# Future-Power-Networks/MAPDN

Hardware: AMD Instinct MI355X
Metric: env-steps/sec (whole node), case141 batch=4096, at 1/2/4/8 MI355X (higher is better)
Workload: dtype f64

## Files before the change

### include/mapdn.h

```cpp
#ifndef MAPDN_H
#define MAPDN_H

#include <stdint.h>

#ifdef __cplusplus
extern "C" {
#endif

#define MAPDN_OK 0
#define MAPDN_E_INVALID (-1)
#define MAPDN_E_TOPOLOGY (-2)
#define MAPDN_E_HIP (-3)
#define MAPDN_E_STATE (-4)
#define MAPDN_E_NOMEM (-5)
#define MAPDN_E_INTERNAL (-6)

#define MAPDN_N_INFO 11

enum { MAPDN_BARRIER_L1 = 0, MAPDN_BARRIER_L2 = 1, MAPDN_BARRIER_COURANT_BELTRAMI = 2,
       MAPDN_BARRIER_BOWL = 3, MAPDN_BARRIER_BUMP = 4 };

enum { MAPDN_SS_PV = 1, MAPDN_SS_DEMAND = 2, MAPDN_SS_REACTIVE = 4, MAPDN_SS_VM_PU = 8,
       MAPDN_SS_VA_DEGREE = 16, MAPDN_SS_ALL = 31 };

enum { MAPDN_F32 = 0, MAPDN_F64 = 1 };

typedef struct mapdn_netspec {
  int32_t n_bus;
  const double* bus_vn_kv;
  const int32_t* bus_zone;
  int32_t n_line;
  const int32_t* line_from_bus;
  const int32_t* line_to_bus;
  const double* line_r_ohm_per_km;
  const double* line_x_ohm_per_km;
  const double* line_c_nf_per_km;
  const double* line_g_us_per_km;
  const double* line_length_km;
  const int32_t* line_parallel;
  const uint8_t* line_in_service;
  int32_t n_branch_pu;
  const int32_t* br_from_bus;
  const int32_t* br_to_bus;
  const double* br_r_pu;
  const double* br_x_pu;
  const double* br_b_pu;
  const double* br_ratio;
  const double* br_shift_deg;
  int32_t n_shunt;
  const int32_t* shunt_bus;
  const double* shunt_p_mw;
  const double* shunt_q_mvar;
  int32_t n_load;
  const int32_t* load_bus;
  int32_t n_sgen;
  const int32_t* sgen_bus;
  const int32_t* sgen_zone;
  int32_t ext_grid_bus;
  double ext_grid_vm_pu;
  double sn_mva;
  double f_hz;
  const double* br_g_pu;
  const double* load_scaling;
  const double* sgen_scaling;
  const int32_t* bus_alias;
  const double* load_const_z;
  const double* load_const_i;
} mapdn_netspec;

typedef struct mapdn_env_config {
  int32_t barrier_type;
  double voltage_weight;
  double q_weight;
  double line_weight;
  int32_t use_line_weight;
  int32_t use_q_weight;
  double v_lower, v_upper;
  int32_t episode_limit;
  double action_low, action_high;
  int32_t reset_action;
  int32_t state_space;
  uint64_t seed;
  int64_t env_id_offset;
  int32_t auto_reset;
  int32_t nr_solver;
  int32_t nr_waves;
  int32_t nr_lanes;
  int32_t nr_lean;
  int32_t nr_h_lds, nr_g_lds, nr_rec_lds, nr_flat_lds, nr_line_lds;
  int32_t nr_mm_pass;
  int32_t sp_lanes;
  int32_t inject_full;
  double nr_check_dx;
  double nr_check_quad;
  int32_t debug_geometry;
  double tolerance_mva;
  int32_t tolerance_is_pu;
  int32_t nr_init;
  int32_t fuse_inject;
  int32_t overlap_advance;
  int32_t xcd_map;
} mapdn_env_config;

typedef struct mapdn_dims_t {
  int32_t n_envs, n_bus, n_line, n_load, n_sgen, n_agents, n_actions, obs_size, state_size, n_info;
  int32_t is_radial;
  int32_t max_zone_size;
} mapdn_dims_t;

typedef struct mapdn_handle mapdn_handle;

const char* mapdn_last_error(const mapdn_handle* h);

int mapdn_create(const mapdn_netspec* net, const mapdn_env_config* cfg, int32_t n_envs,
                 int32_t device, mapdn_handle** out);
void mapdn_destroy(mapdn_handle* h);
int mapdn_dims(const mapdn_handle* h, mapdn_dims_t* out);

int mapdn_set_profiles(mapdn_handle* h, const double* pv, const double* load_p, const double* load_q,
                       int64_t n_rows, int32_t time_delta_min, int32_t days);

int mapdn_get_profile_stats(const mapdn_handle* h, double* stdv, double* smax);

int mapdn_reset(mapdn_handle* h, const int64_t* start_rows, int32_t add_noise, int32_t max_tries,
                void* stream);

int mapdn_step(mapdn_handle* h, const void* actions, int32_t actions_dtype, int32_t add_noise,
               double* reward, uint8_t* terminated, double* info, void* stream);

int mapdn_step_obs(mapdn_handle* h, const void* actions, int32_t actions_dtype, int32_t add_noise,
                   double* reward, uint8_t* terminated, double* info, void* obs, int32_t obs_dtype, void* stream);

int mapdn_get_obs(mapdn_handle* h, void* obs, int32_t dtype, void* stream);
int mapdn_get_state(mapdn_handle* h, void* state, int32_t dtype, void* stream);

int mapdn_get_results(mapdn_handle* h, double* vm_pu, double* va_degree, double* p_mw, double* q_mvar,
                      double* pl_mw, double* sgen_p, double* sgen_q, void* stream);
int mapdn_get_loads(mapdn_handle* h, double* load_p, double* load_q, void* stream);

int mapdn_get_start_rows(mapdn_handle* h, int64_t* start_rows, void* stream);

int mapdn_get_auto_reset_mask(mapdn_handle* h, uint8_t* mask, void* stream);

int mapdn_get_returns(mapdn_handle* h, double* returns, void* stream);

int mapdn_solve_only(mapdn_handle* h, const double* p_load, const double* q_load, const double* p_sgen,
                     const double* q_sgen, double* vm_pu, double* va_degree, int32_t* iterations,
                     uint8_t* converged, void* stream);

int mapdn_get_ybus_dense(const mapdn_handle* h, double* ybus_re_im);
int mapdn_get_obs_index(const mapdn_handle* h, int32_t* kind, int32_t* index);

int mapdn_get_schedule(const mapdn_handle* h, int32_t n_waves, int32_t* n_rows, int32_t* rows, int32_t* parent);

int mapdn_get_nr_geometry(const mapdn_handle* h, int32_t* out20);

int mapdn_get_dc_angles(const mapdn_handle* h, const double* p_bus_demand_mw, double* va_rad);

int mapdn_get_flat_factors(const mapdn_handle* h, double* factors, int32_t* bus_of_pos);

int mapdn_get_sparse_program(const mapdn_handle* h, int32_t sub_lanes, int32_t* dims, int32_t* ops, int32_t* order, int32_t* slots_ij);

int mapdn_dense_solve(const double* a, const double* b, double* x, int32_t n, int32_t batch, void* stream);

int mapdn_policy_forward(const float* obs, const float* hid_in, const float* w1, const float* b1, const float* ln_g,
                         const float* ln_b, const float* w_ih, const float* w_hh, const float* b_ih, const float* b_hh,
                         const float* w2, const float* b2, float* means, float* hid_out, int32_t rows, int32_t n_agents,
                         int32_t obs_dim, int32_t id_dim, float ln_eps, void* stream);

int mapdn_policy_forward_train(const float* obs, const float* hid_in, const float* w1, const float* b1, const float* ln_g,
                               const float* ln_b, const float* w_ih, const float* w_hh, const float* b_ih, const float* b_hh,
                               const float* w2, const float* b2, float* means, float* hid_out, float* x1_out, int32_t rows,
                               int32_t n_agents, int32_t obs_dim, int32_t id_dim, float ln_eps, void* stream);
int64_t mapdn_policy_backward_scratch_floats(int64_t rows);
int mapdn_policy_backward(const float* dmeans, const float* x1, const float* hid_in, const float* ln_g, const float* ln_b, float ln_eps,
                          const float* w_ih, const float* w_hh, const float* b_ih, const float* b_hh, const float* w2, float* dx1,
                          float* dgates, float* xn, float* small, float* scratch, int64_t rows, void* stream);

int mapdn_policy_forward_fits(int32_t obs_dim, int32_t id_dim);
int mapdn_policy_forward_geometry(int32_t obs_dim, int32_t id_dim, int32_t* threads, int32_t* ids_lds, int32_t* lds_bytes);

int mapdn_layernorm64_forward(const float* x, const float* gamma, const float* beta, float* y, float* mean, float* rstd,
                              int64_t rows, float eps, int32_t relu, void* stream);
int mapdn_layernorm64_backward_blocks(int64_t rows);
int mapdn_layernorm64_backward(const float* dy, const float* x, const float* gamma, const float* beta, const float* mean,
                               const float* rstd, float* dx, float* dgamma, float* dbeta, float* partial, int64_t rows,
                               int32_t relu, void* stream);
int mapdn_layernorm64_bc_forward(const float* base, const float* per_n, int32_t n, const float* gamma, const float* beta, float* y,
                                 float* mean, float* rstd, int64_t rows, float eps, int32_t relu, void* stream);
int mapdn_layernorm64_bc_backward(const float* dy, const float* base, const float* per_n, int32_t n, const float* gamma, const float* beta,
                                  const float* mean, const float* rstd, float* dx, float* dgamma, float* dbeta, float* partial,
                                  int64_t rows, int32_t relu, void* stream);
int mapdn_relu_dot64_forward(const float* pre, const float* w, float bias, float* v, int64_t rows, void* stream);
int mapdn_relu_dot64_backward(const float* dv, const float* pre, const float* w, float* dpre, float* dw, float* db, float* partial,
                              int64_t rows, void* stream);

int mapdn_critic_head_forward(const float* x, const float* per_n, int32_t n, const float* gamma, const float* beta, float eps,
                              const float* w2, const float* b2, const float* w3, const float* b3, float* v, int64_t rows, void* stream);
int64_t mapdn_critic_head_scratch_floats(int64_t rows, int32_t n, int32_t formed);
int mapdn_critic_head_backward_geometry(int64_t rows, int32_t n, int32_t formed, int32_t mode, int32_t cus, int32_t* threads,
                                        int32_t* blocks, int32_t* lds_bytes);
int mapdn_critic_head_backward(const float* dv, const float* x, const float* per_n, int32_t n, const float* gamma, const float* beta,
                               float eps, const float* w2, const float* b2, const float* w3, const float* b3, float* dx, float* grads,
                               float* scratch, int64_t rows, int32_t param_grads, void* stream);
int mapdn_critic_head_mse(const float* ret, const float* wrow, const float* scale, const float* x, const float* per_n, int32_t n,
                          const float* gamma, const float* beta, float eps, const float* w2, const float* b2, const float* w3,
                          const float* b3, float* dx, float* grads, float* scratch, int64_t rows, void* stream);
int mapdn_critic_head_backward_dot(const float* dv, const float* x, const float* per_n, int32_t n, const float* gamma, const float* beta,
                                   float eps, const float* w2, const float* b2, const float* w3, const float* b3, const float* dot_w,
                                   float* dact, int64_t rows, void* stream);

int mapdn_critic_twin_forward(const float* base, const float* per_n, int32_t n, const float* flag_col, const float* gamma, const float* beta,
                              float eps, const float* w2, const float* b2, const float* w3, const float* b3, float* v1, float* v2,
                              float* vmin, int64_t rows, void* stream);
int64_t mapdn_critic_twin_scratch_floats(int64_t rows, int32_t n);
int mapdn_critic_twin_geometry(int64_t rows, int32_t n, int32_t cus, int32_t* threads, int32_t* blocks, int32_t* lds_bytes);
int mapdn_critic_twin_mse(const float* ret, const float* wrow, const float* scale, const float* base, const float* per_n, int32_t n,
                          const float* flag_col, const float* gamma, const float* beta, float eps, const float* w2, const float* b2,
                          const float* w3, const float* b3, float* dbase, float* grads, float* scratch, int64_t rows, void* stream);

int mapdn_explore_actions(const float* mean, const float* eps, const float* avail, float stdv, int32_t tanh_bound, double action_scale,
                          double action_bias, float* action, float* action_pol, float* actual, int64_t n, void* stream);
int mapdn_rollout_stats(const double* info, const double* reward, const uint8_t* alive, const uint8_t* done, uint8_t* alive_out, double* sums,
                        int32_t n_envs, void* stream);
int mapdn_copy_segments(const void* const* src, void* const* dst, const int64_t* nbytes, int32_t n_segments, void* stream);

int mapdn_debug_stream(const double* src, double* dst, int32_t rows, int32_t Bp, int32_t pattern, void* stream);

const char* mapdn_build_info(void);

int mapdn_stats(mapdn_handle* h, int64_t* reset_failures, double* mean_iters, int32_t* max_iters,
                void* stream);

int mapdn_nr_timing(mapdn_handle* h, int32_t enable);
int mapdn_nr_time_ms(mapdn_handle* h, double* total_ms, int64_t* launches);

int mapdn_get_nr_kernel(const mapdn_handle* h, int32_t* out8);

typedef struct mapdn_droop_config {
  double va, vb, vc, vd;
  double damping;
  int32_t max_iter;
  double v_tol;
  double reactive_ratio;
} mapdn_droop_config;

int mapdn_droop_actions(mapdn_handle* h, const mapdn_droop_config* cfg, double* actions, double* vm_pu, int32_t* iterations,
                        uint8_t* status, void* stream);

#ifdef __cplusplus
}
#endif
#endif
```

### mapdn_amd/_lib.py

```python
from __future__ import annotations

import ctypes as C
import os

import numpy as np

from .netspec import NetSpec

_HERE = os.path.dirname(os.path.abspath(__file__))
LIB_PATH = os.path.join(_HERE, "libmapdn_hip.so")

N_INFO = 11
INFO_KEYS = (
    "percentage_of_v_out_of_control", "percentage_of_lower_than_lower_v",
    "percentage_of_higher_than_upper_v", "totally_controllable_ratio",
    "average_voltage_deviation", "average_voltage", "max_voltage_drop_deviation",
    "max_voltage_rise_deviation", "total_line_loss", "q_loss", "destroy",
)
BARRIER_IDS = dict(l1=0, l2=1, courant_beltrami=2, bowl=3, bump=4)
SS_BITS = dict(pv=1, demand=2, reactive=4, vm_pu=8, va_degree=16)
F32, F64 = 0, 1

EXPORTS = (
    "mapdn_last_error", "mapdn_create", "mapdn_destroy", "mapdn_dims", "mapdn_set_profiles", "mapdn_reset",
    "mapdn_step", "mapdn_get_start_rows", "mapdn_get_returns", "mapdn_get_obs", "mapdn_get_state", "mapdn_get_results", "mapdn_get_loads",
    "mapdn_solve_only", "mapdn_get_ybus_dense", "mapdn_get_obs_index", "mapdn_get_schedule", "mapdn_get_flat_factors", "mapdn_stats", "mapdn_nr_timing",
    "mapdn_nr_time_ms", "mapdn_get_auto_reset_mask", "mapdn_dense_solve", "mapdn_step_obs", "mapdn_get_sparse_program", "mapdn_policy_forward",
    "mapdn_policy_forward_fits", "mapdn_layernorm64_forward", "mapdn_layernorm64_backward", "mapdn_layernorm64_backward_blocks",
    "mapdn_get_nr_geometry", "mapdn_debug_stream", "mapdn_build_info", "mapdn_layernorm64_bc_forward", "mapdn_layernorm64_bc_backward", "mapdn_relu_dot64_forward", "mapdn_relu_dot64_backward",
    "mapdn_critic_head_forward", "mapdn_critic_head_scratch_floats", "mapdn_critic_head_backward", "mapdn_critic_head_backward_dot", "mapdn_critic_head_mse", "mapdn_get_profile_stats",
    "mapdn_explore_actions", "mapdn_rollout_stats", "mapdn_copy_segments",
    "mapdn_policy_forward_train", "mapdn_policy_backward", "mapdn_policy_backward_scratch_floats", "mapdn_get_dc_angles",
    "mapdn_get_nr_kernel", "mapdn_droop_actions", "mapdn_policy_forward_geometry", "mapdn_critic_head_backward_geometry",
    "mapdn_critic_twin_forward", "mapdn_critic_twin_scratch_floats", "mapdn_critic_twin_geometry", "mapdn_critic_twin_mse",
)

_pd = C.POINTER(C.c_double)
_pi = C.POINTER(C.c_int32)
_pu8 = C.POINTER(C.c_uint8)


class CNetSpec(C.Structure):
    _fields_ = [
        ("n_bus", C.c_int32), ("bus_vn_kv", _pd), ("bus_zone", _pi),
        ("n_line", C.c_int32), ("line_from_bus", _pi), ("line_to_bus", _pi),
        ("line_r_ohm_per_km", _pd), ("line_x_ohm_per_km", _pd), ("line_c_nf_per_km", _pd),
        ("line_g_us_per_km", _pd), ("line_length_km", _pd), ("line_parallel", _pi), ("line_in_service", _pu8),
        ("n_branch_pu", C.c_int32), ("br_from_bus", _pi), ("br_to_bus", _pi), ("br_r_pu", _pd), ("br_x_pu", _pd),
        ("br_b_pu", _pd), ("br_ratio", _pd), ("br_shift_deg", _pd),
        ("n_shunt", C.c_int32), ("shunt_bus", _pi), ("shunt_p_mw", _pd), ("shunt_q_mvar", _pd),
        ("n_load", C.c_int32), ("load_bus", _pi),
        ("n_sgen", C.c_int32), ("sgen_bus", _pi), ("sgen_zone", _pi),
        ("ext_grid_bus", C.c_int32), ("ext_grid_vm_pu", C.c_double), ("sn_mva", C.c_double), ("f_hz", C.c_double),
        ("br_g_pu", _pd), ("load_scaling", _pd), ("sgen_scaling", _pd), ("bus_alias", _pi),
        ("load_const_z", _pd), ("load_const_i", _pd),
    ]


class CEnvConfig(C.Structure):
    _fields_ = [
        ("barrier_type", C.c_int32), ("voltage_weight", C.c_double), ("q_weight", C.c_double),
        ("line_weight", C.c_double), ("use_line_weight", C.c_int32), ("use_q_weight", C.c_int32),
        ("v_lower", C.c_double), ("v_upper", C.c_double), ("episode_limit", C.c_int32),
        ("action_low", C.c_double), ("action_high", C.c_double), ("reset_action", C.c_int32),
        ("state_space", C.c_int32), ("seed", C.c_uint64), ("env_id_offset", C.c_int64), ("auto_reset", C.c_int32),
        ("nr_solver", C.c_int32), ("nr_waves", C.c_int32), ("nr_lanes", C.c_int32), ("nr_lean", C.c_int32),
        ("nr_h_lds", C.c_int32), ("nr_g_lds", C.c_int32), ("nr_rec_lds", C.c_int32), ("nr_flat_lds", C.c_int32), ("nr_line_lds", C.c_int32),
        ("nr_mm_pass", C.c_int32), ("sp_lanes", C.c_int32), ("inject_full", C.c_int32),
        ("nr_check_dx", C.c_double), ("nr_check_quad", C.c_double), ("debug_geometry", C.c_int32),
        ("tolerance_mva", C.c_double), ("tolerance_is_pu", C.c_int32), ("nr_init", C.c_int32),
        ("fuse_inject", C.c_int32), ("overlap_advance", C.c_int32), ("xcd_map", C.c_int32),
    ]


TUNING_INT = ("nr_solver", "nr_waves", "nr_lanes", "nr_lean", "nr_h_lds", "nr_g_lds", "nr_rec_lds", "nr_flat_lds", "nr_line_lds",
              "nr_mm_pass", "sp_lanes", "inject_full", "debug_geometry", "tolerance_is_pu", "nr_init", "fuse_inject", "overlap_advance", "xcd_map")
TUNING_F64 = ("nr_check_dx", "nr_check_quad", "tolerance_mva")
NR_SOLVERS = dict(auto=0, tree=0, sparse=1, dense=2)
NR_INITS = dict(flat=0, dc=2)
GEOMETRY_KEYS = ("solver", "waves", "lanes", "lean", "rows", "h_lds", "g_lds", "rec_lds", "flat_lds", "line_lds", "mm_pass",
                 "lds_bytes", "workgroups", "resident_per_cu", "rounds", "model_ns", "fuse_inject", "n_fused_buses", "n_nodes", "nr_init")


class CDroopConfig(C.Structure):
    _fields_ = [("va", C.c_double), ("vb", C.c_double), ("vc", C.c_double), ("vd", C.c_double), ("damping", C.c_double),
                ("max_iter", C.c_int32), ("v_tol", C.c_double), ("reactive_ratio", C.c_double)]


DROOP_STATUS = ("converged", "max_iter", "pf_failed", "not_solved")


def make_droop_config(cfg=None) -> CDroopConfig:
    c = CDroopConfig()
    if cfg is None:
        return c
    get = cfg.get if isinstance(cfg, dict) else (lambda k, _d=None: getattr(cfg, k, _d))
    if isinstance(cfg, dict):
        unknown = set(cfg) - {f for f, _ in CDroopConfig._fields_}
        if unknown:
            raise KeyError(f"unknown droop config keys {sorted(unknown)}")
    for name, typ in CDroopConfig._fields_:
        v = get(name, None)
        if v is not None:
            setattr(c, name, int(v) if typ is C.c_int32 else float(v))
    return c


class CDims(C.Structure):
    _fields_ = [(k, C.c_int32) for k in (
        "n_envs", "n_bus", "n_line", "n_load", "n_sgen", "n_agents", "n_actions", "obs_size", "state_size",
        "n_info", "is_radial", "max_zone_size")]


class MapdnError(RuntimeError):
    def __init__(self, code, msg):
        super().__init__(f"libmapdn_hip error {code}: {msg}")
        self.code = code


_lib = None


def _safe_source_hash(b):
    try:
        return b.source_hash()
    except OSError:
        return "sources unreadable"


def load():
    global _lib
    if _lib is not None:
        return _lib
    import torch
    if "MAPDN_LIB_PATH" not in os.environ:
        from . import build as _build
        try:
            is_stale = _build.stale()
        except OSError:
            is_stale = not os.path.exists(LIB_PATH)
            if not is_stale:
                import warnings
                warnings.warn(f"mapdn_amd/csrc is not readable: {LIB_PATH} is loaded without the source-hash check", RuntimeWarning, stacklevel=2)
        if is_stale:
            try:
                _build.build_locked()
            except Exception as exc:
                raise ImportError(
                    f"{LIB_PATH} is missing or was built from other sources than mapdn_amd/csrc (hash {_build.library_hash()} vs "
                    f"{_safe_source_hash(_build)}) and could not be rebuilt ({exc}); build it with `python -m mapdn_amd.build` "
                    "(hipcc --offload-arch=gfx950); there is no CPU fallback") from exc
    lib = C.CDLL(os.environ.get("MAPDN_LIB_PATH", LIB_PATH))
    if "MAPDN_LIB_PATH" in os.environ:
        for name in EXPORTS:
            if not hasattr(lib, name):
                def _missing(*a, _n=name, **k):
                    raise AttributeError(f"{os.environ['MAPDN_LIB_PATH']} does not export {_n}")
                lib.__dict__[name] = _missing
    vp = C.c_void_p
    lib.mapdn_last_error.restype = C.c_char_p
    lib.mapdn_last_error.argtypes = [vp]
    lib.mapdn_build_info.restype = C.c_char_p
    lib.mapdn_build_info.argtypes = []
    lib.mapdn_create.argtypes = [C.POINTER(CNetSpec), C.POINTER(CEnvConfig), C.c_int32, C.c_int32, C.POINTER(vp)]
    lib.mapdn_destroy.argtypes = [vp]
    lib.mapdn_destroy.restype = None
    lib.mapdn_dims.argtypes = [vp, C.POINTER(CDims)]
    lib.mapdn_set_profiles.argtypes = [vp, _pd, _pd, _pd, C.c_int64, C.c_int32, C.c_int32]
    lib.mapdn_get_profile_stats.argtypes = [vp, _pd, _pd]
    lib.mapdn_reset.argtypes = [vp, vp, C.c_int32, C.c_int32, vp]
    lib.mapdn_step.argtypes = [vp, vp, C.c_int32, C.c_int32, vp, vp, vp, vp]
    lib.mapdn_step_obs.argtypes = [vp, vp, C.c_int32, C.c_int32, vp, vp, vp, vp, C.c_int32, vp]
    lib.mapdn_get_start_rows.argtypes = [vp, vp, vp]
    lib.mapdn_get_returns.argtypes = [vp, vp, vp]
    lib.mapdn_get_auto_reset_mask.argtypes = [vp, vp, vp]
    lib.mapdn_get_obs.argtypes = [vp, vp, C.c_int32, vp]
    lib.mapdn_get_state.argtypes = [vp, vp, C.c_int32, vp]
    lib.mapdn_get_results.argtypes = [vp] + [vp] * 7 + [vp]
    lib.mapdn_get_loads.argtypes = [vp, vp, vp, vp]
    lib.mapdn_solve_only.argtypes = [vp] + [vp] * 8 + [vp]
    lib.mapdn_get_ybus_dense.argtypes = [vp, _pd]
    lib.mapdn_get_obs_index.argtypes = [vp, _pi, _pi]
    lib.mapdn_get_schedule.argtypes = [vp, C.c_int32, _pi, _pi, _pi]
    lib.mapdn_get_flat_factors.argtypes = [vp, _pd, _pi]
    lib.mapdn_get_dc_angles.argtypes = [vp, _pd, _pd]
    lib.mapdn_get_nr_geometry.argtypes = [vp, _pi]
    lib.mapdn_get_nr_kernel.argtypes = [vp, _pi]
    lib.mapdn_debug_stream.argtypes = [vp, vp, C.c_int32, C.c_int32, C.c_int32, vp]
    lib.mapdn_get_sparse_program.argtypes = [vp, C.c_int32, _pi, _pi, _pi, _pi]
    lib.mapdn_policy_forward.argtypes = [vp] * 14 + [C.c_int32] * 4 + [C.c_float, vp]
    lib.mapdn_policy_forward_fits.argtypes = [C.c_int32, C.c_int32]
    lib.mapdn_policy_forward_geometry.argtypes = [C.c_int32, C.c_int32, _pi, _pi, _pi]
    lib.mapdn_critic_head_backward_geometry.argtypes = [C.c_int64, C.c_int32, C.c_int32, C.c_int32, C.c_int32, _pi, _pi, _pi]
    lib.mapdn_policy_forward_train.argtypes = [vp] * 15 + [C.c_int32] * 4 + [C.c_float, vp]
    lib.mapdn_policy_backward_scratch_floats.argtypes = [C.c_int64]
    lib.mapdn_policy_backward_scratch_floats.restype = C.c_int64
    lib.mapdn_policy_backward.argtypes = [vp] * 5 + [C.c_float] + [vp] * 10 + [C.c_int64, vp]
    lib.mapdn_layernorm64_forward.argtypes = [vp] * 6 + [C.c_int64, C.c_float, C.c_int32, vp]
    lib.mapdn_layernorm64_backward_blocks.argtypes = [C.c_int64]
    lib.mapdn_layernorm64_backward.argtypes = [vp] * 10 + [C.c_int64, C.c_int32, vp]
    lib.mapdn_layernorm64_bc_forward.argtypes = [vp, vp, C.c_int32] + [vp] * 5 + [C.c_int64, C.c_float, C.c_int32, vp]
    lib.mapdn_layernorm64_bc_backward.argtypes = [vp, vp, vp, C.c_int32] + [vp] * 8 + [C.c_int64, C.c_int32, vp]
    lib.mapdn_relu_dot64_forward.argtypes = [vp, vp, C.c_float, vp, C.c_int64, vp]
    lib.mapdn_relu_dot64_backward.argtypes = [vp] * 7 + [C.c_int64, vp]
    lib.mapdn_critic_head_forward.argtypes = [vp, vp, C.c_int32, vp, vp, C.c_float] + [vp] * 5 + [C.c_int64, vp]
    lib.mapdn_critic_head_scratch_floats.argtypes = [C.c_int64, C.c_int32, C.c_int32]
    lib.mapdn_critic_head_scratch_floats.restype = C.c_int64
    lib.mapdn_critic_head_backward.argtypes = [vp, vp, vp, C.c_int32, vp, vp, C.c_float] + [vp] * 7 + [C.c_int64, C.c_int32, vp]
    lib.mapdn_explore_actions.argtypes = [vp, vp, vp, C.c_float, C.c_int32, C.c_double, C.c_double, vp, vp, vp, C.c_int64, vp]
    lib.mapdn_rollout_stats.argtypes = [vp, vp, vp, vp, vp, vp, C.c_int32, vp]
    lib.mapdn_copy_segments.argtypes = [C.POINTER(vp), C.POINTER(vp), C.POINTER(C.c_int64), C.c_int32, vp]
    lib.mapdn_critic_head_mse.argtypes = [vp] * 5 + [C.c_int32, vp, vp, C.c_float] + [vp] * 7 + [C.c_int64, vp]
    lib.mapdn_critic_twin_forward.argtypes = [vp, vp, C.c_int32, vp, vp, vp, C.c_float] + [vp] * 7 + [C.c_int64, vp]
    lib.mapdn_critic_twin_scratch_floats.argtypes = [C.c_int64, C.c_int32]
    lib.mapdn_critic_twin_scratch_floats.restype = C.c_int64
    lib.mapdn_critic_twin_geometry.argtypes = [C.c_int64, C.c_int32, C.c_int32, _pi, _pi, _pi]
    lib.mapdn_critic_twin_mse.argtypes = [vp] * 5 + [C.c_int32, vp, vp, vp, C.c_float] + [vp] * 7 + [C.c_int64, vp]
    lib.mapdn_critic_head_backward_dot.argtypes = [vp, vp, vp, C.c_int32, vp, vp, C.c_float] + [vp] * 6 + [C.c_int64, vp]
    lib.mapdn_dense_solve.argtypes = [vp, vp, vp, C.c_int32, C.c_int32, vp]
    lib.mapdn_stats.argtypes = [vp, C.POINTER(C.c_int64), C.POINTER(C.c_double), C.POINTER(C.c_int32), vp]
    lib.mapdn_nr_timing.argtypes = [vp, C.c_int32]
    lib.mapdn_nr_time_ms.argtypes = [vp, C.POINTER(C.c_double), C.POINTER(C.c_int64)]
    lib.mapdn_droop_actions.argtypes = [vp, C.POINTER(CDroopConfig), vp, vp, vp, vp, vp]
    for name in EXPORTS:
        if name not in ("mapdn_last_error", "mapdn_destroy", "mapdn_build_info"):
            getattr(lib, name).restype = C.c_int
    _lib = lib
    return lib


def check(rc, handle=None):
    if rc != 0:
        msg = load().mapdn_last_error(handle)
        raise MapdnError(rc, msg.decode() if msg else "?")


def _p(a, typ):
    return a.ctypes.data_as(typ) if a.size else C.cast(None, typ)


def make_cnetspec(net: NetSpec):
    keep = net
    s = CNetSpec()
    s.n_bus = net.n_bus
    s.bus_vn_kv = _p(net.bus_vn_kv, _pd)
    s.bus_zone = _p(net.bus_zone, _pi)
    s.n_line = net.n_line
    s.line_from_bus = _p(net.line_from_bus, _pi)
    s.line_to_bus = _p(net.line_to_bus, _pi)
    s.line_r_ohm_per_km = _p(net.line_r_ohm_per_km, _pd)
    s.line_x_ohm_per_km = _p(net.line_x_ohm_per_km, _pd)
    s.line_c_nf_per_km = _p(net.line_c_nf_per_km, _pd)
    s.line_g_us_per_km = _p(net.line_g_us_per_km, _pd)
    s.line_length_km = _p(net.line_length_km, _pd)
    s.line_parallel = _p(net.line_parallel, _pi)
    s.line_in_service = _p(net.line_in_service, _pu8)
    s.n_branch_pu = net.n_branch_pu
    s.br_from_bus = _p(net.br_from_bus, _pi)
    s.br_to_bus = _p(net.br_to_bus, _pi)
    s.br_r_pu = _p(net.br_r_pu, _pd)
    s.br_x_pu = _p(net.br_x_pu, _pd)
    s.br_b_pu = _p(net.br_b_pu, _pd)
    s.br_ratio = _p(net.br_ratio, _pd)
    s.br_shift_deg = _p(net.br_shift_deg, _pd)
    s.n_shunt = int(net.shunt_bus.shape[0])
    s.shunt_bus = _p(net.shunt_bus, _pi)
    s.shunt_p_mw = _p(net.shunt_p_mw, _pd)
    s.shunt_q_mvar = _p(net.shunt_q_mvar, _pd)
    s.n_load = net.n_load
    s.load_bus = _p(net.load_bus, _pi)
    s.n_sgen = net.n_sgen
    s.sgen_bus = _p(net.sgen_bus, _pi)
    s.sgen_zone = _p(net.sgen_zone, _pi)
    s.ext_grid_bus = int(net.ext_grid_bus)
    s.ext_grid_vm_pu = float(net.ext_grid_vm_pu)
    s.sn_mva = float(net.sn_mva)
    s.f_hz = float(net.f_hz)
    s.br_g_pu = _p(net.br_g_pu, _pd)
    s.load_scaling = _p(net.load_scaling, _pd)
    s.sgen_scaling = _p(net.sgen_scaling, _pd)
    s.bus_alias = _p(net.bus_alias, _pi) if net.has_fused_buses else C.cast(None, _pi)
    zl = net.has_zip_loads
    s.load_const_z = _p(net.load_const_z, _pd) if zl else C.cast(None, _pd)
    s.load_const_i = _p(net.load_const_i, _pd) if zl else C.cast(None, _pd)
    return s, keep


def make_cconfig(args: dict, env_id_offset: int = 0, tuning: dict | None = None) -> CEnvConfig:
    c = CEnvConfig()
    for k, v in (tuning or {}).items():
        if k == "nr_solver" and isinstance(v, str):
            v = NR_SOLVERS[v]
        if k == "nr_init" and isinstance(v, str):
            if v not in NR_INITS:
                raise ValueError(f"nr_init must be one of {sorted(NR_INITS)} (or 0 / 2), got {v!r}")
            v = NR_INITS[v]
        if k in TUNING_INT:
            setattr(c, k, int(v))
        elif k in TUNING_F64:
            setattr(c, k, float(v))
        else:
            raise KeyError(f"unknown tuning key {k!r} (known: {TUNING_INT + TUNING_F64})")
    bt = args.get("voltage_barrier_type", "l1")
    if bt not in BARRIER_IDS:
        raise KeyError(bt)
    c.barrier_type = BARRIER_IDS[bt]
    c.voltage_weight = float(args.get("voltage_weight", 1.0))
    qw, lw = args.get("q_weight", 0.1), args.get("line_weight", None)
    c.q_weight = 0.0 if qw is None else float(qw)
    c.line_weight = 0.0 if lw is None else float(lw)
    c.use_q_weight = int(qw is not None)
    c.use_line_weight = int(lw is not None)
    c.v_lower = float(args.get("v_lower", 0.95))
    c.v_upper = float(args.get("v_upper", 1.05))
    c.episode_limit = int(args["episode_limit"])
    c.action_low = -float(args["action_scale"]) + float(args["action_bias"])
    c.action_high = float(args["action_scale"]) + float(args["action_bias"])
    c.reset_action = int(bool(args.get("reset_action", True)))
    ss = args.get("state_space", ["pv", "demand", "reactive", "vm_pu", "va_degree"])
    c.state_space = sum(SS_BITS[k] for k in set(ss) if k in SS_BITS)
    c.seed = int(args.get("seed", 0)) & 0xFFFFFFFFFFFFFFFF
    c.env_id_offset = int(env_id_offset)
    c.auto_reset = int(bool(args.get("auto_reset", False)))
    return c


def nr_geometry(handle) -> dict:
    out = (C.c_int32 * 20)()
    check(load().mapdn_get_nr_geometry(handle, out), handle)
    return dict(zip(GEOMETRY_KEYS, [int(x) for x in out]))


NR_KERNEL_KEYS = {0: ("W", "L", "HL", "GL", "RES", "DC", "ZIP"), 1: ("L", "DC", "ZIP"), 2: ("W", "GA")}


def nr_kernel(handle) -> dict:
    out = (C.c_int32 * 8)()
    check(load().mapdn_get_nr_kernel(handle, out), handle)
    solver = int(out[0])
    return dict(solver=solver, **{k: int(out[1 + i]) for i, k in enumerate(NR_KERNEL_KEYS[solver])})


def policy_forward_geometry(obs_dim: int, id_dim: int):
    t, il, lds = C.c_int32(), C.c_int32(), C.c_int32()
    ok = load().mapdn_policy_forward_geometry(int(obs_dim), int(id_dim), C.byref(t), C.byref(il), C.byref(lds))
    return (t.value, il.value, lds.value) if ok else None


def critic_head_backward_geometry(rows: int, n: int, formed: bool, mode: int, cus: int = 0):
    t, b, lds = C.c_int32(), C.c_int32(), C.c_int32()
    rc = load().mapdn_critic_head_backward_geometry(int(rows), int(n), int(bool(formed)), int(mode), int(cus), C.byref(t), C.byref(b), C.byref(lds))
    return (t.value, b.value, lds.value) if rc == 0 else None


def critic_twin_geometry(rows: int, n: int, cus: int = 0):
    t, b, lds = C.c_int32(), C.c_int32(), C.c_int32()
    rc = load().mapdn_critic_twin_geometry(int(rows), int(n), int(cus), C.byref(t), C.byref(b), C.byref(lds))
    return (t.value, b.value, lds.value) if rc == 0 else None
```

### mapdn_amd/csrc/capi.hip

```cpp
#include <hip/hip_runtime.h>

#include <algorithm>
#include <cmath>
#include <cstdio>
#include <cstdlib>
#include <cstring>
#include <string>
#include <type_traits>
#include <vector>

#include "kernels.hpp"
#include "nr_inst_list.hpp"
#include "colstats.hpp"
#include "plan.hpp"

using namespace mapdn;

static constexpr size_t CU_LDS = 160 * 1024;
static constexpr int DROOP_MAX_ITER_CAP = 10000;

struct Knobs {
  int solver;
  int waves, lanes;
  int lean, h_lds, g_lds, rec_lds, flat_lds, line_lds, mm_pass, fuse_inject;
  int sp_lanes;
  bool inject_full, debug_geometry;
  double check_dx, check_quad;
};

static Knobs resolve_knobs(const mapdn_env_config& c) {
  auto num = [](int v, const char* env) { const char* s = getenv(env); return s ? atoi(s) : v; };
  auto tri = [](int v, const char* env) { const char* s = getenv(env); return s ? (atoi(s) ? 1 : 2) : v; };
  auto f64 = [](double v, const char* env, double dflt) { const char* s = getenv(env); return s ? atof(s) : (v != 0.0 ? v : dflt); };
  Knobs k;
  k.solver = num(0, "MAPDN_NR_DENSE") ? 2 : (num(0, "MAPDN_NR_SPARSE") ? 1 : c.nr_solver);
  k.waves = num(c.nr_waves, "MAPDN_NR_WAVES"); k.lanes = num(c.nr_lanes, "MAPDN_NR_LANES"); k.lean = tri(c.nr_lean, "MAPDN_NR_LEAN");
  k.h_lds = tri(c.nr_h_lds, "MAPDN_NR_H_LDS"); k.g_lds = tri(c.nr_g_lds, "MAPDN_NR_G_LDS"); k.rec_lds = tri(c.nr_rec_lds, "MAPDN_NR_REC_LDS");
  k.flat_lds = tri(c.nr_flat_lds, "MAPDN_NR_FLAT_LDS"); k.line_lds = tri(c.nr_line_lds, "MAPDN_NR_LINE_LDS");
  k.mm_pass = tri(c.nr_mm_pass, "MAPDN_NR_MM_PASS");
  k.fuse_inject = tri(c.fuse_inject, "MAPDN_FUSE_INJECT");
  k.sp_lanes = num(c.sp_lanes, "MAPDN_SP_LANES");
  k.inject_full = num(c.inject_full, "MAPDN_INJECT_FULL") != 0;
  k.debug_geometry = num(c.debug_geometry, "MAPDN_DEBUG_GEOMETRY") != 0;
  k.check_dx = f64(c.nr_check_dx, "MAPDN_NR_CHECK_DX", 1e-7);
  k.check_quad = f64(c.nr_check_quad, "MAPDN_NR_CHECK_QUAD", 1.0);
  return k;
}

struct mapdn_handle {
  Plan plan;
  Schedule sched;
  SparseProg sprog;
  Knobs knobs;
  int solver = 0;
  int sp_lanes = 0;
  int nr_var = 0;
  mapdn_env_config cfg;
  Dev d;
  int device = 0;
  std::string err;
  std::vector<void*> allocs;
  bool have_profiles = false, was_reset = false, host_only = false;
  bool sbus_stale = true;
  bool fuse_inject = false;
  size_t lds_bytes = 0;
  struct Geo { int W = 0, L = 0, lean = 0, rows = 0, h_lds = 0, g_lds = 0, rec_lds = 0, flat_lds = 0, line_lds = 0, mm_pass = 0, ncl = 0;
               size_t lds = 0; long wgs = 0; int resident = 0, rounds = 0; double model_ns = 0.0; } geo;
  int32_t *obs_rows = nullptr, *state_rows = nullptr, *iota_idx = nullptr, *vm_row = nullptr, *va_row = nullptr;
  int32_t *obs_xptr = nullptr, *obs_xrow = nullptr;
  double *obs_scale = nullptr, *state_scale = nullptr;
  double *t_pl = nullptr, *t_ql = nullptr, *t_pv = nullptr, *t_q = nullptr;
  double* table = nullptr; double* stdv = nullptr; double* smax = nullptr;
  std::vector<double> stdv_host, smax_host;
  long long* stats_dev = nullptr;
  bool timing = false;
  std::vector<hipEvent_t> ev;
  size_t ev_used = 0;
  double acc_ms = 0.0;
  int64_t acc_launches = 0;
  DroopState droop{};
  bool droop_ready = false;
};

static std::string g_create_err;

static int api_fail(const mapdn_handle* h, int code, const char* what) noexcept {
  try { (h ? const_cast<mapdn_handle*>(h)->err : g_create_err) = what; } catch (...) {}
  return code;
}
#define MAPDN_CATCH(h)                                                                                       \
  catch (const std::bad_alloc&) { return api_fail((h), MAPDN_E_NOMEM, "out of host memory (std::bad_alloc)"); } \
  catch (const std::exception& e) { return api_fail((h), MAPDN_E_INTERNAL, e.what()); }                      \
  catch (...) { return api_fail((h), MAPDN_E_INTERNAL, "unknown C++ exception"); }

#define NEEDDEV(h) do { if ((h)->host_only) { (h)->err = "host-only handle (device == -1): no device entry points"; return MAPDN_E_STATE; } } while (0)
#define HIPCHK(h, call)                                                                         \
  do {                                                                                          \
    hipError_t _e = (call);                                                                     \
    if (_e != hipSuccess) {                                                                     \
      (h)->err = std::string(#call) + ": " + hipGetErrorString(_e);                             \
      return MAPDN_E_HIP;                                                                       \
    }                                                                                           \
  } while (0)

template <typename T>
static int dalloc(mapdn_handle* h, T** p, size_t count) {
  void* q = nullptr;
  size_t bytes = std::max<size_t>(count, 1) * sizeof(T);
  HIPCHK(h, hipMalloc(&q, bytes));
  h->allocs.push_back(q);
  HIPCHK(h, hipMemset(q, 0, bytes));
  *p = (T*)q;
  return MAPDN_OK;
}

template <typename Q, typename T>
static int dupload(mapdn_handle* h, Q** p, const std::vector<T>& v) {
  static_assert(std::is_same<std::remove_const_t<Q>, T>::value, "dupload: element type mismatch");
  T* q = nullptr;
  int rc = dalloc(h, &q, v.size());
  if (rc) return rc;
  if (!v.empty()) HIPCHK(h, hipMemcpy(q, v.data(), v.size() * sizeof(T), hipMemcpyHostToDevice));
  *p = q;
  return MAPDN_OK;
}

static double nr_model_ns(int W, int L, int n, int R, int h_lds, long wgs, int resident, int n_cu) {
  const double Wt = (double)W * (64 / L);
  const long per_round = (long)n_cu * std::max(resident, 1);
  const double rounds = (double)((wgs + per_round - 1) / per_round);
  const double row = W == 1 ? 2374.0 : (W == 2 ? 2903.0 : 3001.0);
  const double fill = (double)wgs / (double)n_cu;
  const double conc = std::min((double)std::max(resident, 1), std::max(1.0, fill));
  const double base = 26032.0 + 363.0 * (double)n / Wt + row * (double)R * (h_lds ? 1.0 : 1.023);
  const double load = 1.0 + (h_lds ? 0.0 : 0.21) * std::min(1.0, fill);
  const double share = 1.0 + 0.5 * std::max(0.0, conc * W / 4.0 - 1.0);
  return rounds * base * load * share;
}

static int settle_tree_geometry(mapdn_handle* h, int Bp, int n_cu) {
  const Plan& P = h->plan;
  const Knobs& k = h->knobs;
  if (P.n + 1 > 0xffff) { h->err = "networks with more than 65534 buses are not supported (16-bit node positions in the NR step records)"; return MAPDN_E_INVALID; }
  auto tri = [](int forced, bool dflt) { return forced == 1 ? 1 : (forced == 2 ? 0 : (dflt ? 1 : 0)); };
  auto settle = [&](int W, int L, int lean, Schedule& S, mapdn_handle::Geo& g) -> int {
    const int Wt = W * (64 / L);
    int min_rows = 0;
    for (int pass = 0; pass < 4; ++pass) {
      build_schedule(P, Wt, S, nr_min_cslots(W, L), 64 / L, min_rows);
      if (S.n_cslots > 1023 || S.n_xslots > 1023) { h->err = "NR schedule needs more than 1023 LDS slots"; return MAPDN_E_INVALID; }
      g.ncl = (int)S.clist.size();
      if (g.ncl > 4095) { h->err = "NR schedule: more than 4095 overflow children (junctions with > 3 non-chain children)"; return MAPDN_E_INVALID; }
      if ((long)S.R * Wt > 0xffff) { h->err = "NR schedule has more than 65535 steps"; return MAPDN_E_INVALID; }
      const int R_ = S.R;
      auto lds_for = [&](int hl, int gl, int ll, int rl, int fl) {
        return nr_lds_bytes(W, L, P.n, S.n_cslots, S.n_xslots, g.ncl, hl, gl, ll ? P.n_line : 0, rl ? R_ : 0, fl ? R_ : 0); };
      g.h_lds = tri(k.h_lds, !lean && lds_for(1, 0, 0, 0, 0) <= CU_LDS);
      g.rec_lds = tri(k.rec_lds, !lean && lds_for(g.h_lds, 0, 0, 1, 0) <= CU_LDS);
      g.flat_lds = tri(k.flat_lds, !lean && lds_for(g.h_lds, 0, 0, g.rec_lds, 1) <= CU_LDS);
      g.line_lds = (tri(k.line_lds, !lean && P.n_line > 0 && lds_for(g.h_lds, 0, 1, g.rec_lds, g.flat_lds) <= CU_LDS) && P.n_line > 0) ? 1 : 0;
      g.g_lds = (tri(k.g_lds, !lean && g.h_lds && lds_for(1, 1, g.line_lds, g.rec_lds, g.flat_lds) <= CU_LDS) && g.h_lds) ? 1 : 0;
      g.lds = lds_for(g.h_lds, g.g_lds, g.line_lds, g.rec_lds, g.flat_lds);
      if (g.lds > CU_LDS) return 1;
      const int need = g.g_lds ? 0 : (g.h_lds ? NR_G_REG_ROWS : NR_HG_REG_ROWS);
      if (R_ >= need) { min_rows = -1; break; }
      min_rows = need;
    }
    if (min_rows >= 0) { h->err = "NR schedule: could not settle the number of peeled rows"; return MAPDN_E_INVALID; }
    const int compiled = nr_geometry_compiled(W, L, g.h_lds, g.g_lds, g.rec_lds, g.flat_lds, h->nr_var);
    if (!compiled) return 1;
    g.W = W; g.L = L; g.lean = lean; g.rows = S.R;
    g.wgs = Bp / L;
    g.resident = (int)std::max<size_t>(1, std::min<size_t>(CU_LDS / std::max<size_t>(g.lds, 1), (size_t)std::max(4 / W, 1)));
    const long per_round = (long)n_cu * g.resident;
    g.rounds = (int)((g.wgs + per_round - 1) / per_round);
    g.model_ns = nr_model_ns(W, L, P.n, S.R, g.h_lds, g.wgs, g.resident, n_cu) * (compiled == 2 ? 1.0 : 1.05);
    return 0;
  };
  const int W = k.waves, L = k.lanes, lean_k = k.lean;
  if ((W != 0 && W != 1 && W != 2 && W != 4 && W != 8) || (L != 0 && L != 4 && L != 8 && L != 16 && L != 32)) {
    h->err = "nr_waves (MAPDN_NR_WAVES) must be 1/2/4/8 and nr_lanes (MAPDN_NR_LANES) 4/8/16/32 (0 = automatic)"; return MAPDN_E_INVALID; }
  mapdn_handle::Geo best; Schedule bestS; bool have = false;
  const bool forced = W != 0 && L != 0 && lean_k != 0;
  static const int cand[][2] = {{1, 16}, {2, 16}, {4, 16}, {4, 8}};
  for (const auto& wl : cand) {
    if ((W && wl[0] != W) || (L && wl[1] != L)) continue;
    for (int lean = 0; lean < 2; ++lean) {
      if ((lean_k == 1 && !lean) || (lean_k == 2 && lean)) continue;
      mapdn_handle::Geo g; Schedule S;
      const int r = settle(wl[0], wl[1], lean, S, g);
      if (r < 0) return r;
      if (r > 0) continue;
      if (!have || g.model_ns < best.model_ns) { best = g; bestS = std::move(S); have = true; }
    }
  }
  if (!have && W && L) {
    mapdn_handle::Geo g; Schedule S;
    const int r = settle(W, L, lean_k == 1 ? 1 : 0, S, g);
    if (r < 0) return r;
    if (r == 0) { best = g; bestS = std::move(S); have = true; }
    else if (g.lds > CU_LDS) { h->err = "NR schedule needs more LDS than one CU has (160 KB); use fewer envs per workgroup (nr_lanes / MAPDN_NR_LANES) or fewer waves"; return MAPDN_E_INVALID; }
  }
  if (!have) {
    h->err = (W || L) ? "this (nr_waves, nr_lanes) combination is not compiled in or does not fit the 160 KB LDS of a CU (csrc/nr_inst_list.hpp)"
                      : "no compiled k_nr_tree geometry fits this network into the 160 KB LDS of a CU";
    return MAPDN_E_INVALID; }
  if (forced) best.model_ns = 0.0;
  best.mm_pass = (best.h_lds && k.mm_pass != 2) ? 1 : 0;
  h->geo = best; h->sched = std::move(bestS); h->lds_bytes = best.lds;
  if (k.debug_geometry)
    fprintf(stderr, "[mapdn] k_nr_tree geometry: W %d L %d lean %d rows %d cslots %d | LDS: h %d rec %d flat %d line %d G %d = %zu B | "
                    "%ld workgroups, %d per CU, %d round(s), model %.1f us\n",
            best.W, best.L, best.lean, best.rows, h->sched.n_cslots, best.h_lds, best.rec_lds, best.flat_lds, best.line_lds, best.g_lds,
            best.lds, best.wgs, best.resident, best.rounds, best.model_ns * 1e-3);
  return MAPDN_OK;
}


static int choose_solver(mapdn_handle* h) {
  const Plan& P = h->plan;
  const int pick = h->knobs.solver;
  if (pick < 0 || pick > 2) { h->err = "nr_solver must be 0 (auto), 1 (sparse) or 2 (dense)"; return MAPDN_E_INVALID; }
  if (pick == 2) {
    if (2 * P.n > 1024) { h->err = "nr_solver = dense (MAPDN_NR_DENSE): the dense general-topology solver handles at most 513 buses (one thread per Jacobian row)"; return MAPDN_E_TOPOLOGY; }
    h->solver = 2;
  } else if (pick == 1 || !P.radial) {
    SparseProg g0;
    sparse_symbolic(P, g0);
    int Lc = 0;
    for (int l : {16, 8, 4, 2}) if (nr_sparse_lds_bytes(P.n, g0.n_blocks, l) <= CU_LDS) { Lc = l; break; }
    if (!Lc) {
      h->err = "topology: meshed network with " + std::to_string(P.nb) + " buses needs " + std::to_string(g0.n_blocks) +
               " Jacobian blocks after fill; two envs of it do not fit the 160 KB LDS of a CU";
      return MAPDN_E_TOPOLOGY; }
    h->solver = 1; h->sp_lanes = Lc;
  }
  return MAPDN_OK;
}

static int validate(mapdn_handle* h, const mapdn_env_config& c) {
  const Plan& P = h->plan;
  const Knobs& k = h->knobs;
  if (c.nr_init == 1)
    return api_fail(h, MAPDN_E_INVALID, "nr_init != 0 (warm start, runpp init=\"results\") is not built: tools/warm_start_study.py / "
                                        "profiles/r04_warm_start_study_*.json show no iteration saved per 16-env workgroup; every solve "
                                        "starts flat like the reference's");
  if (c.nr_init != 0 && c.nr_init != 2) return api_fail(h, MAPDN_E_INVALID, "nr_init must be 0 (flat start) or 2 (runpp init=\"dc\"); 1 (init=\"results\") is reserved");
  if (c.nr_init == 2 && !P.dc_ok)
    return api_fail(h, MAPDN_E_INVALID, !P.fused_obus.empty()
                        ? "nr_init = 2 (runpp init=\"dc\") on a net with fused buses (bus_alias) is not supported (the DC-angle start is defined on unfused nets only)"
                        : "nr_init = 2 (runpp init=\"dc\"): the DC power flow matrix Bbus of this net is singular or not finite (a branch with x = 0?)");
  if (h->solver == 2 && c.nr_init == 2)
    return api_fail(h, MAPDN_E_INVALID, "nr_init = 2 (runpp init=\"dc\") is not built for nr_solver = dense (k_nr_dense starts flat only): use the tree or the sparse solver");
  if (h->solver == 2 && P.zip)
    return api_fail(h, MAPDN_E_INVALID, "voltage-dependent loads (load_const_z / load_const_i) are not built for nr_solver = dense (k_nr_dense solves "
                                        "constant-power loads only): use the tree or the sparse solver");
  if (c.overlap_advance) return api_fail(h, MAPDN_E_INVALID, "overlap_advance was removed (measured slower than the single stream): it must be 0");
  if (c.xcd_map) return api_fail(h, MAPDN_E_INVALID, "xcd_map was removed (the XCD-aligned env order measured a wash): it must be 0");
  if (k.fuse_inject == 1 && h->solver != 0)
    return api_fail(h, MAPDN_E_INVALID, "fuse_inject = 1 exists on the tree solver only (this handle runs the general sparse / dense solver)");
  if (k.fuse_inject == 1 && (c.auto_reset || k.inject_full))
    return api_fail(h, MAPDN_E_INVALID, "fuse_inject = 1 needs a handle without auto_reset and without inject_full");
  if (h->solver == 1 && k.sp_lanes != 0 && k.sp_lanes != 16 && k.sp_lanes != 8 && k.sp_lanes != 4 && k.sp_lanes != 2)
    return api_fail(h, MAPDN_E_INVALID, "sp_lanes (MAPDN_SP_LANES) must be 16, 8, 4 or 2 (0 = automatic)");
  return MAPDN_OK;
}

static int settle_general_solver(mapdn_handle* h) {
  const Plan& P = h->plan;
  Dev& d = h->d;
  if (h->solver == 2) { d.dn_N = (2 * P.n + 15) / 16 * 16; d.dn_lda = d.dn_N + 2; return MAPDN_OK; }
  if (h->solver != 1) return MAPDN_OK;
  if (h->knobs.sp_lanes) h->sp_lanes = h->knobs.sp_lanes;
  else {
    double best = -1.0;
    for (int l : {16, 8, 4, 2}) {
      SparseProg g;
      sparse_program(P, 64 / l, g);
      const size_t lds = nr_sparse_lds_bytes(P.n, g.n_blocks, l);
      if (lds > CU_LDS) continue;
      const double waves = (double)std::min<size_t>(CU_LDS / lds, 8);
      const double score = waves * l / ((double)g.n_phases + 0.5 * g.rows_per_sub * g.max_nnz);
      if (score > best) { best = score; h->sp_lanes = l; }
    }
  }
  sparse_program(P, 64 / h->sp_lanes, h->sprog);
  h->lds_bytes = nr_sparse_lds_bytes(P.n, h->sprog.n_blocks, h->sp_lanes);
  if (h->lds_bytes > CU_LDS) { h->err = "sp_lanes (MAPDN_SP_LANES): does not fit in LDS"; return MAPDN_E_INVALID; }
  return MAPDN_OK;
}

#define UP(field, vec) do { if (const int rc_ = dupload(h, &d.field, vec)) return rc_; } while (0)
#define AL(field, rows) do { if (const int rc_ = dalloc(h, &d.field, (size_t)(rows) * d.Bp)) return rc_; } while (0)

static int upload_topology(mapdn_handle* h) {
  const Plan& P = h->plan;
  const mapdn_env_config& c = h->cfg;
  Dev& d = h->d;
  d.nb = P.nb; d.n = P.n; d.nl = P.nl; d.ns = P.ns; d.n_line = P.n_line;
  d.nbo = P.nbo;
  d.ncol = P.ns + 2 * P.nl;
  d.vroot = P.vroot; d.sn = P.sn_mva; d.tol = P.tol; d.max_it = 10;
  d.yrr0 = P.yrr[0]; d.yrr1 = P.yrr[1];
  d.barrier_type = c.barrier_type; d.use_line_weight = c.use_line_weight; d.episode_limit = c.episode_limit;
  d.reset_action = c.reset_action; d.auto_reset = c.auto_reset ? 1 : 0; d.voltage_weight = c.voltage_weight; d.q_weight = c.q_weight;
  d.line_weight = c.line_weight; d.v_lower = c.v_lower; d.v_upper = c.v_upper;
  d.action_low = c.action_low; d.action_high = c.action_high;
  d.seed_lo = (uint32_t)(c.seed & 0xffffffffull); d.seed_hi = (uint32_t)(c.seed >> 32);
  d.env_id_offset = c.env_id_offset;
  d.nr_init = c.nr_init;
  if (d.nr_init == 2) UP(dc_pc, P.dc_pc);
  d.zip = P.zip ? 1 : 0;
  if (d.zip) { UP(zip_c, P.zip_c); d.zip_c_bytes = (uint32_t)(P.zip_c.size() * sizeof(double)); }
  UP(bus_of_pos, P.bus_of_pos); UP(root_children, P.root_children); UP(root_y, P.root_y);
  UP(pos_of_obus, P.pos_of_obus); UP(cm_kind, P.cm_kind);
  d.n_fused = (int32_t)P.fused_obus.size(); d.n_alias = (int32_t)P.alias_pos.size(); d.n_slack_group = (int32_t)P.slack_group.size();
  if (d.n_fused) {
    UP(fused_obus, P.fused_obus); UP(ob_load_ptr, P.ob_load_ptr); UP(ob_load_idx, P.ob_load_idx); UP(ob_sgen_ptr, P.ob_sgen_ptr);
    UP(ob_sgen_idx, P.ob_sgen_idx); UP(ob_shunt_p, P.ob_shunt_p); UP(ob_shunt_q, P.ob_shunt_q);
    { std::vector<int32_t> sg(P.slack_group); if (sg.empty()) sg.push_back(0); UP(slack_group, sg); }
    { std::vector<int32_t> ap(P.alias_pos); if (ap.empty()) ap.push_back(0); UP(alias_pos, ap); }
  }
  d.n_root_children = (int32_t)P.root_children.size();
  UP(load_ptr, P.load_ptr); UP(load_idx, P.load_idx); UP(sgen_ptr, P.sgen_ptr); UP(sgen_idx, P.sgen_idx);
  UP(shunt_p, P.shunt_p); UP(shunt_q, P.shunt_q); UP(load_scale, P.load_scale); UP(sgen_scale, P.sgen_scale);
  std::vector<LineFlow> padded(P.lines);
  if (padded.size() % 2) padded.push_back(LineFlow{});
  UP(lines, padded);
  return MAPDN_OK;
}

static int setup_pv_buses(mapdn_handle* h) {
  const Plan& P = h->plan;
  Dev& d = h->d;
  std::vector<int32_t> sgb, sgb_of(P.nb, -1), lb, mlo;
  for (int k = 0; k < P.nb; ++k) {
    if (P.sgen_ptr[k + 1] > P.sgen_ptr[k]) { sgb_of[k] = (int32_t)sgb.size(); sgb.push_back(k); }
    else if (P.load_ptr[k + 1] > P.load_ptr[k]) {
      lb.push_back(k);
      if (P.load_ptr[k + 1] - P.load_ptr[k] > 1 && k < P.n) mlo.push_back(k);
    }
  }
  d.n_sgb = (int32_t)sgb.size(); d.n_lb = (int32_t)lb.size(); d.n_mlo = (int32_t)mlo.size();
  if (lb.empty()) lb.push_back(0);
  if (mlo.empty()) mlo.push_back(0);
  {
    std::vector<int32_t> rec;
    auto put = [&](int k, bool pv) {
      const int nsg = pv ? P.sgen_ptr[k + 1] - P.sgen_ptr[k] : 0, nld = P.load_ptr[k + 1] - P.load_ptr[k];
      rec.push_back(k < P.n ? k : -1);
      rec.push_back(k);
      rec.push_back(pv ? P.sgen_idx[P.sgen_ptr[k]] : -1);
      rec.push_back((nsg << 8) | std::min(nld, 2));
      rec.push_back(nld > 0 ? P.load_idx[P.load_ptr[k]] : -1);
      rec.push_back(nld > 1 ? P.load_idx[P.load_ptr[k] + 1] : -1);
      rec.push_back(0); rec.push_back(0);
    };
    for (int i = 0; i < d.n_sgb; ++i) put(sgb[i], true);
    for (int i = 0; i < d.n_mlo; ++i) put(mlo[i], false);
    UP(sgb_rec, rec);
  }
  UP(sgb_pos, sgb); UP(sgb_of_pos, sgb_of); UP(lb_pos, lb); UP(mlo_pos, mlo);
  std::vector<int32_t> ld_dest(std::max(P.nl, 1), 2);
  for (int k = 0; k < P.nb; ++k) {
    if (P.load_ptr[k + 1] - P.load_ptr[k] != 1) continue;
    const int li = P.load_idx[P.load_ptr[k]];
    if (sgb_of[k] >= 0) ld_dest[li] = (sgb_of[k] << 2) | 1;
    else if (k < P.n) ld_dest[li] = (k << 2) | 0;
  }
  UP(ld_dest, ld_dest);
  return dalloc(h, &d.bus_ld, (size_t)2 * d.n_sgb * d.Bp);
}

struct GbufRows { int pv, q, vm, va, rp, rq, n; };
static GbufRows gbuf_rows(const Dev& d) {
  const int vm = 2 * d.ns;
  return {0, d.ns, vm, vm + d.nbo, vm + 2 * d.nbo, vm + 3 * d.nbo, vm + 4 * d.nbo};
}

static int setup_env_state(mapdn_handle* h) {
  Dev& d = h->d;
  const size_t Bp = d.Bp;
  AL(q_new, d.ns); AL(cur_pl, d.nl); AL(cur_ql, d.nl); AL(pl, d.n_line);
  const GbufRows r = gbuf_rows(d);
  AL(gbuf, r.n);
  d.cur_pv = d.gbuf + (size_t)r.pv * Bp;
  d.cur_q = d.gbuf + (size_t)r.q * Bp; d.vm = d.gbuf + (size_t)r.vm * Bp; d.va = d.gbuf + (size_t)r.va * Bp;
  d.res_p = d.gbuf + (size_t)r.rp * Bp; d.res_q = d.gbuf + (size_t)r.rq * Bp;
  AL(sum_rewards, 1); AL(steps, 1); AL(start_row, 1); AL(draw, 1); AL(done, 1); AL(pending, 1);
  AL(active, 1); AL(commit, 1); AL(bad_start, 1); AL(resetting, 1); AL(adv_row, 1); AL(adv_draw, 1); AL(iters, 1); AL(conv, 1);
  std::vector<uint8_t> ones(Bp, 1);
  HIPCHK(h, hipMemcpy(d.done, ones.data(), Bp, hipMemcpyHostToDevice));
  int rc;
  if ((rc = dalloc(h, &h->t_pl, (size_t)d.nl * Bp)) || (rc = dalloc(h, &h->t_ql, (size_t)d.nl * Bp)) ||
      (rc = dalloc(h, &h->t_pv, (size_t)d.ns * Bp)) || (rc = dalloc(h, &h->t_q, (size_t)d.ns * Bp)))
    return rc;
  return dalloc(h, &h->stats_dev, 4);
}

static int setup_gather_tables(mapdn_handle* h) {
  const Plan& P = h->plan;
  const Dev& d = h->d;
  const GbufRows g = gbuf_rows(d);
  std::vector<std::vector<int>> sgens_at(P.nbo);
  for (int j = 0; j < P.ns; ++j) sgens_at[P.sgen_bus[j]].push_back(j);
  auto tables = [&](const std::vector<int32_t>& kind, const std::vector<int32_t>& idx, std::vector<int32_t>& rows,
                    std::vector<double>& scale, std::vector<int32_t>& xptr, std::vector<int32_t>& xrow) {
    rows.resize(kind.size()); scale.assign(kind.size(), 1.0); xptr.assign(kind.size() + 1, 0); xrow.clear();
    for (size_t c = 0; c < kind.size(); ++c) {
      switch (kind[c]) {
        case G_P_ADDBACK: rows[c] = g.rp + idx[c]; for (int j : sgens_at[idx[c]]) xrow.push_back(g.pv + j); break;
        case G_Q_ADDBACK: rows[c] = g.rq + idx[c]; for (int j : sgens_at[idx[c]]) xrow.push_back(g.q + j); break;
        case G_SGEN_P: rows[c] = g.pv + idx[c]; break;
        case G_SGEN_Q: rows[c] = g.q + idx[c]; break;
        case G_VM: rows[c] = g.vm + idx[c]; break;
        case G_VA_RAD: rows[c] = g.va + idx[c]; break;
        case G_P: rows[c] = g.rp + idx[c]; break;
        case G_Q: rows[c] = g.rq + idx[c]; break;
        case G_VA_DEG: rows[c] = g.va + idx[c]; scale[c] = 180.0 / M_PI; break;
        default: rows[c] = -1; break;
      }
      xptr[c + 1] = (int32_t)xrow.size();
      if (xptr[c + 1] > xptr[c]) rows[c] |= 0x40000000;
    }
    if (xrow.empty()) xrow.push_back(0);
  };
  std::vector<int32_t> rows, xptr, xrow; std::vector<double> scale;
  int rc;
  tables(P.obs_kind, P.obs_idx, rows, scale, xptr, xrow);
  if ((rc = dupload(h, &h->obs_rows, rows)) || (rc = dupload(h, &h->obs_scale, scale)) || (rc = dupload(h, &h->obs_xptr, xptr)) ||
      (rc = dupload(h, &h->obs_xrow, xrow)))
    return rc;
  tables(P.state_kind, P.state_idx, rows, scale, xptr, xrow);
  if ((rc = dupload(h, &h->state_rows, rows)) || (rc = dupload(h, &h->state_scale, scale))) return rc;
  std::vector<int32_t> io(std::max(std::max(d.nbo, d.n_line), std::max(d.nl, d.ns)));
  for (size_t i = 0; i < io.size(); ++i) io[i] = (int32_t)i;
  return dupload(h, &h->iota_idx, io);
}

static int alloc_nrbuf(mapdn_handle* h, size_t fb_rows, size_t nblk) {
  const Plan& P = h->plan;
  Dev& d = h->d;
  const size_t Bp = d.Bp;
  const size_t sb_off = fb_rows * Bp * 16;
  const size_t vout_off = sb_off + 2 * nblk * Bp * 16;
  const size_t bytes = vout_off + (size_t)VOF * (P.n + 1) * Bp * sizeof(double);
  if (bytes >= (size_t)0xFFFFFFFFu) { h->err = "env batch too large: NR scratch exceeds the 4 GiB one buffer resource addresses; use fewer envs per handle"; return MAPDN_E_INVALID; }
  if (const int rc = dalloc(h, &d.nrbuf, bytes / sizeof(double))) return rc;
  d.nrbuf_bytes = (uint32_t)bytes;
  d.sb_off = (uint32_t)sb_off; d.sb_off_alt = (uint32_t)(sb_off + nblk * Bp * 16);
  d.r_vout = (uint32_t)(vout_off / (Bp * sizeof(double)));
  std::vector<double> row(Bp, d.vroot);
  double* rootv = d.nrbuf + ((size_t)d.r_vout + (size_t)VOF * P.n) * Bp;
  HIPCHK(h, hipMemcpy(rootv + (size_t)VO_E * Bp, row.data(), Bp * sizeof(double), hipMemcpyHostToDevice));
  HIPCHK(h, hipMemcpy(rootv + (size_t)VO_VM * Bp, row.data(), Bp * sizeof(double), hipMemcpyHostToDevice));
  std::vector<int32_t> vmrow(P.nbo), varow(P.nbo);
  for (int b = 0; b < P.nbo; ++b) { const int k = P.pos_of_obus[b]; vmrow[b] = (int)d.r_vout + VOF * k + VO_VM; varow[b] = (int)d.r_vout + VOF * k + VO_VA; }
  int rc;
  if ((rc = dupload(h, &h->vm_row, vmrow)) || (rc = dupload(h, &h->va_row, varow))) return rc;
  return MAPDN_OK;
}

static int setup_dense(mapdn_handle* h) {
  const Plan& P = h->plan;
  Dev& d = h->d;
  d.dense = 1;
  if (nr_dense_ga(d.dn_N)) {
    const size_t per_env = (size_t)d.dn_N * d.dn_lda;
    if (const int rc = dalloc(h, &d.dn_A, per_env * d.Bp)) return rc;
  }
  UP(gy_ptr, P.gy_ptr); UP(gy_col, P.gy_col); UP(gy_val, P.gy_val);
  if (const int rc = alloc_nrbuf(h, 0, (size_t)P.n)) return rc;
  if (nr_dense_prepare(d) != 0) { (void)hipGetLastError(); h->err = "hipFuncSetAttribute(MaxDynamicSharedMemorySize) failed for k_nr_dense"; return MAPDN_E_HIP; }
  h->lds_bytes = nr_dense_lds_bytes(d);
  return MAPDN_OK;
}

static int setup_sparse(mapdn_handle* h) {
  const Plan& P = h->plan;
  Dev& d = h->d;
  const SparseProg& G = h->sprog;
  d.sparse = 1; d.sp_lanes = h->sp_lanes; d.sp_blocks = G.n_blocks; d.sp_fill = (int32_t)G.fill_slots.size();
  d.sp_phases = G.n_phases; d.sp_rows_per_sub = G.rows_per_sub; d.sp_max_nnz = G.max_nnz;
  UP(sp_ops, G.ops); d.sp_ops_bytes = (uint32_t)(G.ops.size() * sizeof(SpOp));
  UP(sp_nz, G.nz); d.sp_nz_bytes = (uint32_t)(G.nz.size() * sizeof(SpNz));
  { std::vector<int32_t> fs(G.fill_slots); if (fs.empty()) fs.push_back(G.n_blocks - 1); UP(sp_fill_slots, fs); }
  if (const int rc = alloc_nrbuf(h, 0, (size_t)P.n)) return rc;
  if (nr_sparse_prepare(h->sp_lanes) != 0) { (void)hipGetLastError(); h->err = "hipFuncSetAttribute(MaxDynamicSharedMemorySize) failed for k_nr_sparse"; return MAPDN_E_HIP; }
  return MAPDN_OK;
}

static int setup_tree(mapdn_handle* h) {
  const Plan& P = h->plan;
  Dev& d = h->d;
  hipDeviceProp_t prop;
  HIPCHK(h, hipGetDeviceProperties(&prop, h->device));
  if (const int rc = settle_tree_geometry(h, d.Bp, prop.multiProcessorCount)) return rc;
  const mapdn_handle::Geo& G_ = h->geo;
  const Schedule& S = h->sched;
  d.nr_waves = G_.W; d.nr_lanes = G_.L; d.nr_h_lds = G_.h_lds; d.nr_g_lds = G_.g_lds; d.nr_line_lds = G_.line_lds; d.nr_rec_lds = G_.rec_lds; d.nr_flat_lds = G_.flat_lds;
  d.nr_check_dx = h->knobs.check_dx; d.nr_check_quad = h->knobs.check_quad;
  d.nr_rows = S.R; d.nr_cslots = S.n_cslots; d.nr_xslots = S.n_xslots; d.nr_nclist = G_.ncl;
  {
    const int lr = nr_set_lds_limit(G_.W, G_.L, G_.h_lds, G_.g_lds, G_.rec_lds, G_.flat_lds, CU_LDS, h->nr_var);
    if (lr == -2) { h->err = "this (nr_waves, nr_lanes) combination is not compiled in (csrc/nr_inst_list.hpp)"; return MAPDN_E_INVALID; }
    if (lr != 0) { (void)hipGetLastError(); h->err = "hipFuncSetAttribute(MaxDynamicSharedMemorySize) failed"; return MAPDN_E_HIP; }
  }
  UP(sched, S.steps); d.sched_bytes = (uint32_t)(S.steps.size() * sizeof(StepRec));
  UP(clist, S.clist);
  UP(mm_ptr, S.mm_ptr); UP(mm_child, S.mm_child);
  UP(mm_recs, S.mm_recs); d.mm_recs_bytes = (uint32_t)(S.mm_recs.size() * sizeof(StepRec)); d.mm_np = S.mm_np;
  d.nr_mm_pass = G_.mm_pass;
  UP(flat, S.flat); d.flat_bytes = (uint32_t)(S.flat.size() * sizeof(double));
  if (d.nr_init == 2) { UP(dc_recs, S.dc_recs); d.dc_recs_bytes = (uint32_t)(S.dc_recs.size() * sizeof(DcRec)); }
  const size_t nblk = (size_t)P.n + 2;
  const size_t fb_rows = (G_.h_lds && G_.g_lds) ? 0 : (size_t)(P.n + 2) * NBP;
  return alloc_nrbuf(h, fb_rows, nblk);
}

#undef UP
#undef AL

static int create_impl(mapdn_handle* h, const mapdn_netspec* net, const mapdn_env_config* cfg, int32_t B, int32_t device) {
  if (!net || !cfg) { h->err = "null netspec/config"; return MAPDN_E_INVALID; }
  if (B < 1) { h->err = "n_envs must be >= 1"; return MAPDN_E_INVALID; }
  if (cfg->barrier_type < 0 || cfg->barrier_type > MAPDN_BARRIER_BUMP) { h->err = "unknown voltage_barrier_type"; return MAPDN_E_INVALID; }
  if (!cfg->use_line_weight && !cfg->use_q_weight) {
    h->err = "NotImplementedError: Please at least give one weight, either q_weight or line_weight."; return MAPDN_E_INVALID; }
  if (cfg->episode_limit < 2) { h->err = "episode_limit must be >= 2"; return MAPDN_E_INVALID; }
  h->cfg = *cfg;
  h->knobs = resolve_knobs(*cfg);
  int rc = build_plan(*net, *cfg, h->plan, h->err);
  if (!rc) rc = choose_solver(h);
  if (!rc) rc = validate(h, *cfg);
  if (rc) return rc;
  h->nr_var = (cfg->nr_init == 2 ? NR_VAR_DC : 0) | (h->plan.zip ? NR_VAR_ZIP : 0);
  h->fuse_inject = h->solver == 0 && !cfg->auto_reset && !h->knobs.inject_full && h->knobs.fuse_inject != 2;
  h->device = device;
  std::memset(&h->d, 0, sizeof(h->d));
  h->d.B = B; h->d.Bp = (B + 63) / 64 * 64;
  if ((rc = settle_general_solver(h))) return rc;
  if (device == -1) {
    h->host_only = true;
    return h->solver == 0 ? settle_tree_geometry(h, h->d.Bp, 256) : MAPDN_OK;
  }
  int ndev = 0;
  HIPCHK(h, hipGetDeviceCount(&ndev));
  if (device < 0 || device >= ndev) { h->err = "device index out of range"; return MAPDN_E_HIP; }
  HIPCHK(h, hipSetDevice(device));
  if ((rc = upload_topology(h)) || (rc = setup_pv_buses(h)) || (rc = setup_env_state(h)) || (rc = setup_gather_tables(h))) return rc;
  return h->solver == 2 ? setup_dense(h) : h->solver == 1 ? setup_sparse(h) : setup_tree(h);
}

extern "C" {

const char* mapdn_last_error(const mapdn_handle* h) { return h ? h->err.c_str() : g_create_err.c_str(); }

#ifndef MAPDN_SRC_HASH
#define MAPDN_SRC_HASH "unknown"
#endif
const char* mapdn_build_info(void) { return "MAPDN_SRC_HASH=" MAPDN_SRC_HASH; }

int mapdn_create(const mapdn_netspec* net, const mapdn_env_config* cfg, int32_t n_envs, int32_t device, mapdn_handle** out) {
  if (!out) { g_create_err = "null out pointer"; return MAPDN_E_INVALID; }
  *out = nullptr;
  mapdn_handle* h = nullptr;
  try {
    h = new mapdn_handle();
    const int rc = create_impl(h, net, cfg, n_envs, device);
    if (rc) { g_create_err = h->err; mapdn_destroy(h); return rc; }
    *out = h;
    return MAPDN_OK;
  } catch (...) {
    mapdn_destroy(h);
    try { throw; } MAPDN_CATCH(nullptr)
  }
}

void mapdn_destroy(mapdn_handle* h) {
  if (!h) return;
  for (void* p : h->allocs) (void)hipFree(p);
  for (hipEvent_t e : h->ev) (void)hipEventDestroy(e);
  delete h;
}

int mapdn_dims(const mapdn_handle* h, mapdn_dims_t* out) try {
  if (!h || !out) return MAPDN_E_INVALID;
  const Plan& P = h->plan;
  out->n_envs = h->d.B; out->n_bus = P.nbo; out->n_line = P.n_line; out->n_load = P.nl; out->n_sgen = P.ns;
  out->n_agents = P.n_agents; out->n_actions = 1; out->obs_size = P.obs_size; out->state_size = P.state_size;
  out->n_info = MAPDN_N_INFO; out->is_radial = P.radial ? 1 : 0; out->max_zone_size = P.max_zone;
  return MAPDN_OK;
} MAPDN_CATCH(h)

int mapdn_set_profiles(mapdn_handle* h, const double* pv, const double* load_p, const double* load_q,
                       int64_t T, int32_t time_delta_min, int32_t days) try {
  if (!h) return MAPDN_E_INVALID;
  if (!pv || !load_p || !load_q || T < 2) { h->err = "set_profiles: null table or too few rows"; return MAPDN_E_INVALID; }
  if (time_delta_min <= 0 || 60 % time_delta_min) { h->err = "set_profiles: time_delta_min must divide 60"; return MAPDN_E_INVALID; }
  NEEDDEV(h);
  HIPCHK(h, hipSetDevice(h->device));
  Dev& d = h->d;
  const int ns = d.ns, nl = d.nl, ncol = d.ncol;
  d.per_hour = 60 / time_delta_min; d.per_day = 24 * d.per_hour;
  const int episode_days = d.episode_limit / d.per_day + 1;
  d.n_start_days = days - episode_days;
  if (d.n_start_days < 1) { h->err = "set_profiles: table too short for one episode (pv_days - episode_days < 1)"; return MAPDN_E_INVALID; }
  const int64_t max_start = (d.per_hour - 1) + 23 * d.per_hour + (int64_t)(d.n_start_days - 1) * d.per_day;
  if (max_start + d.episode_limit + 1 >= T) { h->err = "set_profiles: sampled episodes could run past the end of the table"; return MAPDN_E_INVALID; }
  std::vector<double> tab((size_t)T * ncol), stdv(ncol), smax(ns);
  for (int64_t t = 0; t < T; ++t) {
    double* r = &tab[(size_t)t * ncol];
    std::memcpy(r, pv + (size_t)t * ns, ns * sizeof(double));
    std::memcpy(r + ns, load_p + (size_t)t * nl, nl * sizeof(double));
    std::memcpy(r + ns + nl, load_q + (size_t)t * nl, nl * sizeof(double));
  }
  column_std(tab.data(), T, ncol, 100.0, stdv);
  for (int j = 0; j < ns; ++j) smax[(size_t)j] = tab[(size_t)j];
  for (int64_t t = 1; t < T; ++t) {
    const double* r = &tab[(size_t)t * ncol];
    for (int j = 0; j < ns; ++j) smax[(size_t)j] = std::max(smax[(size_t)j], r[j]);
  }
  for (int j = 0; j < ns; ++j) smax[(size_t)j] *= 1.2;
  if (h->have_profiles) {
    for (double* p : {h->table, h->stdv, h->smax}) {
      auto it = std::find(h->allocs.begin(), h->allocs.end(), (void*)p);
      if (it != h->allocs.end()) { (void)hipFree(*it); h->allocs.erase(it); }
    }
  }
  int rc;
  if ((rc = dupload(h, &h->table, tab)) || (rc = dupload(h, &h->stdv, stdv)) || (rc = dupload(h, &h->smax, smax))) return rc;
  d.table = h->table; d.stdv = h->stdv; d.smax = h->smax; d.T = T;
  h->stdv_host = stdv; h->smax_host = smax;
  h->have_profiles = true;
  return MAPDN_OK;
} MAPDN_CATCH(h)

static void nr_launch(mapdn_handle* h, int mode, double* reward, uint8_t* term, double* info, hipStream_t st,
                      const void* fused_actions = nullptr, int fused_dtype = 0, const Dev* dv = nullptr) {
  const Dev& d = dv ? *dv : h->d;
  if (!h->timing) { launch_nr(d, mode, reward, term, info, st, fused_actions, fused_dtype); return; }
  if (h->ev_used + 2 > h->ev.size()) {
    if (h->ev.size() >= 2 * 8192) {
      double ms; int64_t n; mapdn_nr_time_ms(h, &ms, &n); h->acc_ms = ms; h->acc_launches = n;
    } else {
      hipEvent_t a, b;
      (void)hipEventCreate(&a); (void)hipEventCreate(&b);
      h->ev.push_back(a); h->ev.push_back(b);
    }
  }
  hipEvent_t a = h->ev[h->ev_used], b = h->ev[h->ev_used + 1];
  h->ev_used += 2;
  (void)hipEventRecord(a, st);
  launch_nr(d, mode, reward, term, info, st, fused_actions, fused_dtype);
  (void)hipEventRecord(b, st);
}

static void inject_launch(mapdn_handle* h, int mode, const void* actions, int dtype, int add_noise, hipStream_t st) {
  const Dev& d = h->d;
  if (h->sbus_stale || h->knobs.inject_full) {
    launch_inject(d, mode, actions, dtype, d.cur_pl, d.cur_ql, d.cur_pv, nullptr, add_noise, st);
    h->sbus_stale = false;
  } else launch_inject_sgen(d, mode, actions, dtype, add_noise, st);
}

static void step_launches(mapdn_handle* h, const void* actions, int32_t actions_dtype, int32_t add_noise, double* reward,
                          uint8_t* terminated, double* info, hipStream_t st) {
  const Dev& d = h->d;
  const bool fused = h->fuse_inject && !h->sbus_stale;
  if (!fused) inject_launch(h, MODE_STEP, actions, actions_dtype, add_noise, st);
  nr_launch(h, MODE_STEP, reward, terminated, info, st, fused ? actions : nullptr, actions_dtype);
  if (d.zip) {
    launch_advance(d, 0, 0, 1, d.sb_off_alt, st);
    launch_advance(d, add_noise, 1, 0, d.sb_off_alt, st);
  } else {
    launch_commit_fused(d, st);
    launch_advance(d, add_noise, 1, 1, d.sb_off_alt, st);
  }
  std::swap(h->d.sb_off, h->d.sb_off_alt);
}

int mapdn_reset(mapdn_handle* h, const int64_t* start_rows, int32_t add_noise, int32_t max_tries, void* stream) try {
  if (!h) return MAPDN_E_INVALID;
  if (!h->have_profiles) { h->err = "reset before set_profiles"; return MAPDN_E_STATE; }
  if (max_tries < 1) max_tries = 1;
  NEEDDEV(h);
  HIPCHK(h, hipSetDevice(h->device));
  hipStream_t st = (hipStream_t)stream;
  const Dev& d = h->d;
  for (int t = 0; t < max_tries; ++t) {
    launch_reset_begin(d, start_rows, t == 0, st);
    launch_advance(d, add_noise, 1, 0, d.sb_off, st);
    inject_launch(h, MODE_RESET, nullptr, MAPDN_F64, add_noise, st);
    nr_launch(h, MODE_RESET, nullptr, nullptr, nullptr, st);
    launch_commit_fused(d, st);
    launch_advance(d, 0, 0, 1, d.sb_off, st);
  }
  HIPCHK(h, hipGetLastError());
  h->was_reset = true;
  return MAPDN_OK;
} MAPDN_CATCH(h)

int mapdn_step(mapdn_handle* h, const void* actions, int32_t actions_dtype, int32_t add_noise, double* reward,
               uint8_t* terminated, double* info, void* stream) try {
  if (!h) return MAPDN_E_INVALID;
  if (!h->was_reset) { h->err = "step before reset"; return MAPDN_E_STATE; }
  if (!actions || !reward || !terminated || !info) { h->err = "step: null buffer"; return MAPDN_E_INVALID; }
  if (actions_dtype != MAPDN_F32 && actions_dtype != MAPDN_F64) { h->err = "step: bad actions dtype"; return MAPDN_E_INVALID; }
  NEEDDEV(h);
  HIPCHK(h, hipSetDevice(h->device));
  hipStream_t st = (hipStream_t)stream;
  step_launches(h, actions, actions_dtype, add_noise, reward, terminated, info, st);
  HIPCHK(h, hipGetLastError());
  return MAPDN_OK;
} MAPDN_CATCH(h)

int mapdn_step_obs(mapdn_handle* h, const void* actions, int32_t actions_dtype, int32_t add_noise, double* reward,
                   uint8_t* terminated, double* info, void* obs, int32_t obs_dtype, void* stream) try {
  if (!h) return MAPDN_E_INVALID;
  if (!h->was_reset) { h->err = "step before reset"; return MAPDN_E_STATE; }
  if (!actions || !reward || !terminated || !info || !obs) { h->err = "step_obs: null buffer"; return MAPDN_E_INVALID; }
  if (actions_dtype != MAPDN_F32 && actions_dtype != MAPDN_F64) { h->err = "step_obs: bad actions dtype"; return MAPDN_E_INVALID; }
  if (obs_dtype != MAPDN_F32 && obs_dtype != MAPDN_F64) { h->err = "step_obs: bad obs dtype"; return MAPDN_E_INVALID; }
  NEEDDEV(h);
  HIPCHK(h, hipSetDevice(h->device));
  hipStream_t st = (hipStream_t)stream;
  const Dev& d = h->d;
  const int C = h->plan.n_agents * h->plan.obs_size;
  step_launches(h, actions, actions_dtype, add_noise, reward, terminated, info, st);
  launch_gather(d, d.gbuf, h->obs_rows, h->obs_scale, 1.0, h->obs_xptr, h->obs_xrow, obs, obs_dtype, C, st);
  HIPCHK(h, hipGetLastError());
  return MAPDN_OK;
} MAPDN_CATCH(h)

int mapdn_get_obs(mapdn_handle* h, void* obs, int32_t dtype, void* stream) try {
  if (!h || !obs) return MAPDN_E_INVALID;
  if (!h->was_reset) { h->err = "get_obs before reset"; return MAPDN_E_STATE; }
  NEEDDEV(h);
  HIPCHK(h, hipSetDevice(h->device));
  hipStream_t st = (hipStream_t)stream;
  launch_gather(h->d, h->d.gbuf, h->obs_rows, h->obs_scale, 1.0, h->obs_xptr, h->obs_xrow, obs, dtype,
                h->plan.n_agents * h->plan.obs_size, st);
  HIPCHK(h, hipGetLastError());
  return MAPDN_OK;
} MAPDN_CATCH(h)

int mapdn_get_state(mapdn_handle* h, void* state, int32_t dtype, void* stream) try {
  if (!h || !state) return MAPDN_E_INVALID;
  if (!h->was_reset) { h->err = "get_state before reset"; return MAPDN_E_STATE; }
  NEEDDEV(h);
  HIPCHK(h, hipSetDevice(h->device));
  hipStream_t st = (hipStream_t)stream;
  launch_gather(h->d, h->d.gbuf, h->state_rows, h->state_scale, 1.0, nullptr, nullptr, state, dtype, h->plan.state_size, st);
  HIPCHK(h, hipGetLastError());
  return MAPDN_OK;
} MAPDN_CATCH(h)

static void transpose_out(mapdn_handle* h, const double* src, double scale, const int32_t* rows, double* out, int n, hipStream_t st) {
  launch_gather(h->d, src, rows, nullptr, scale, nullptr, nullptr, out, MAPDN_F64, n, st);
}

int mapdn_get_results(mapdn_handle* h, double* vm_pu, double* va_degree, double* p_mw, double* q_mvar, double* pl_mw,
                      double* sgen_p, double* sgen_q, void* stream) try {
  if (!h) return MAPDN_E_INVALID;
  if (!h->was_reset) { h->err = "get_results before reset"; return MAPDN_E_STATE; }
  NEEDDEV(h);
  HIPCHK(h, hipSetDevice(h->device));
  hipStream_t st = (hipStream_t)stream;
  const Dev& d = h->d;
  if (vm_pu) transpose_out(h, d.vm, 1.0, h->iota_idx, vm_pu, d.nbo, st);
  if (va_degree) transpose_out(h, d.va, 180.0 / M_PI, h->iota_idx, va_degree, d.nbo, st);
  if (p_mw) transpose_out(h, d.res_p, 1.0, h->iota_idx, p_mw, d.nbo, st);
  if (q_mvar) transpose_out(h, d.res_q, 1.0, h->iota_idx, q_mvar, d.nbo, st);
  if (pl_mw) transpose_out(h, d.pl, 1.0, h->iota_idx, pl_mw, d.n_line, st);
  if (sgen_p) transpose_out(h, d.cur_pv, 1.0, h->iota_idx, sgen_p, d.ns, st);
  if (sgen_q) transpose_out(h, d.cur_q, 1.0, h->iota_idx, sgen_q, d.ns, st);
  HIPCHK(h, hipGetLastError());
  return MAPDN_OK;
} MAPDN_CATCH(h)

int mapdn_get_loads(mapdn_handle* h, double* load_p, double* load_q, void* stream) try {
  if (!h) return MAPDN_E_INVALID;
  NEEDDEV(h);
  HIPCHK(h, hipSetDevice(h->device));
  hipStream_t st = (hipStream_t)stream;
  if (load_p) transpose_out(h, h->d.cur_pl, 1.0, h->iota_idx, load_p, h->d.nl, st);
  if (load_q) transpose_out(h, h->d.cur_ql, 1.0, h->iota_idx, load_q, h->d.nl, st);
  HIPCHK(h, hipGetLastError());
  return MAPDN_OK;
} MAPDN_CATCH(h)

int mapdn_get_start_rows(mapdn_handle* h, int64_t* start_rows, void* stream) try {
  if (!h || !start_rows) return MAPDN_E_INVALID;
  NEEDDEV(h);
  HIPCHK(h, hipSetDevice(h->device));
  HIPCHK(h, hipMemcpyAsync(start_rows, h->d.start_row, (size_t)h->d.B * sizeof(int64_t), hipMemcpyDeviceToDevice, (hipStream_t)stream));
  return MAPDN_OK;
} MAPDN_CATCH(h)

int mapdn_get_auto_reset_mask(mapdn_handle* h, uint8_t* mask, void* stream) try {
  if (!h || !mask) return MAPDN_E_INVALID;
  NEEDDEV(h);
  HIPCHK(h, hipSetDevice(h->device));
  HIPCHK(h, hipMemcpyAsync(mask, h->d.resetting, (size_t)h->d.B, hipMemcpyDeviceToDevice, (hipStream_t)stream));
  return MAPDN_OK;
} MAPDN_CATCH(h)

int mapdn_get_returns(mapdn_handle* h, double* returns, void* stream) try {
  if (!h || !returns) return MAPDN_E_INVALID;
  NEEDDEV(h);
  HIPCHK(h, hipSetDevice(h->device));
  HIPCHK(h, hipMemcpyAsync(returns, h->d.sum_rewards, (size_t)h->d.B * sizeof(double), hipMemcpyDeviceToDevice, (hipStream_t)stream));
  return MAPDN_OK;
} MAPDN_CATCH(h)

int mapdn_solve_only(mapdn_handle* h, const double* p_load, const double* q_load, const double* p_sgen, const double* q_sgen,
                     double* vm_pu, double* va_degree, int32_t* iterations, uint8_t* converged, void* stream) try {
  if (!h) return MAPDN_E_INVALID;
  if (!p_load || !q_load || !p_sgen || !q_sgen) { h->err = "solve_only: null input"; return MAPDN_E_INVALID; }
  NEEDDEV(h);
  HIPCHK(h, hipSetDevice(h->device));
  hipStream_t st = (hipStream_t)stream;
  const Dev& d = h->d;
  launch_to_envminor(d, p_load, h->t_pl, d.nl, st);
  launch_to_envminor(d, q_load, h->t_ql, d.nl, st);
  launch_to_envminor(d, p_sgen, h->t_pv, d.ns, st);
  launch_to_envminor(d, q_sgen, h->t_q, d.ns, st);
  HIPCHK(h, hipMemsetAsync(d.active, 1, d.B, st));
  if (d.Bp > d.B) HIPCHK(h, hipMemsetAsync(d.active + d.B, 0, d.Bp - d.B, st));
  launch_inject(d, MODE_SOLVE, nullptr, MAPDN_F64, h->t_pl, h->t_ql, h->t_pv, h->t_q, 0, st);
  h->sbus_stale = true;
  nr_launch(h, MODE_SOLVE, nullptr, nullptr, nullptr, st);
  if (vm_pu) transpose_out(h, d.nrbuf, 1.0, h->vm_row, vm_pu, d.nbo, st);
  if (va_degree) transpose_out(h, d.nrbuf, 180.0 / M_PI, h->va_row, va_degree, d.nbo, st);
  if (iterations) launch_copy_i32(d.iters, iterations, d.B, st);
  if (converged) launch_copy_u8(d.conv, converged, d.B, st);
  HIPCHK(h, hipGetLastError());
  return MAPDN_OK;
} MAPDN_CATCH(h)

int mapdn_get_profile_stats(const mapdn_handle* h, double* stdv, double* smax) try {
  if (!h) return MAPDN_E_INVALID;
  if (!h->have_profiles) { const_cast<mapdn_handle*>(h)->err = "get_profile_stats before set_profiles"; return MAPDN_E_STATE; }
  if (stdv) std::memcpy(stdv, h->stdv_host.data(), h->stdv_host.size() * sizeof(double));
  if (smax) std::memcpy(smax, h->smax_host.data(), h->smax_host.size() * sizeof(double));
  return MAPDN_OK;
} MAPDN_CATCH(h)

int mapdn_get_ybus_dense(const mapdn_handle* h, double* out) try {
  if (!h || !out) return MAPDN_E_INVALID;
  const Plan& P = h->plan;
  for (size_t i = 0; i < P.ybus.size(); ++i) { out[2 * i] = P.ybus[i].real(); out[2 * i + 1] = P.ybus[i].imag(); }
  return MAPDN_OK;
} MAPDN_CATCH(h)

int mapdn_get_obs_index(const mapdn_handle* h, int32_t* kind, int32_t* index) try {
  if (!h || !kind || !index) return MAPDN_E_INVALID;
  std::memcpy(kind, h->plan.obs_kind.data(), h->plan.obs_kind.size() * sizeof(int32_t));
  std::memcpy(index, h->plan.obs_idx.data(), h->plan.obs_idx.size() * sizeof(int32_t));
  return MAPDN_OK;
} MAPDN_CATCH(h)

int mapdn_get_nr_geometry(const mapdn_handle* h, int32_t* out) try {
  if (!h || !out) return MAPDN_E_INVALID;
  const mapdn_handle::Geo& g = h->geo;
  const int32_t v[20] = {h->solver, g.W, g.L, g.lean, g.rows, g.h_lds, g.g_lds, g.rec_lds, g.flat_lds, g.line_lds, g.mm_pass,
                         (int32_t)h->lds_bytes, (int32_t)g.wgs, g.resident, g.rounds, (int32_t)std::min(g.model_ns, 2.0e9),
                         h->fuse_inject ? 1 : 0, (int32_t)h->plan.fused_obus.size(), h->plan.nb, h->cfg.nr_init};
  std::memcpy(out, v, sizeof(v));
  if (h->solver == 1) out[2] = h->sp_lanes;
  return MAPDN_OK;
} MAPDN_CATCH(h)

int mapdn_get_nr_kernel(const mapdn_handle* h, int32_t* out) try {
  if (!h || !out) return MAPDN_E_INVALID;
  const int dc = h->cfg.nr_init == 2 ? 1 : 0, zip = h->plan.zip ? 1 : 0;
  int32_t v[8] = {h->solver, 0, 0, 0, 0, 0, 0, 0};
  if (h->solver == 0) {
    const mapdn_handle::Geo& g = h->geo;
    const NrInst* I = nr_inst_of(g.W, g.L, g.h_lds, g.g_lds, g.rec_lds, g.flat_lds, h->nr_var);
    if (!I) return api_fail(h, MAPDN_E_INTERNAL, "mapdn_get_nr_kernel: the handle's geometry has no k_nr_tree instantiation");
    const int32_t t[7] = {I->W, I->L, I->HL, I->GL, I->RES, (I->VAR & NR_VAR_DC) ? 1 : 0, (I->VAR & NR_VAR_ZIP) ? 1 : 0};
    std::memcpy(v + 1, t, sizeof(t));
  } else if (h->solver == 1) {
    v[1] = h->sp_lanes; v[2] = dc; v[3] = zip;
  } else {
    const bool ga = nr_dense_ga(h->d.dn_N);
    v[1] = nr_dense_waves(h->d.dn_N, ga); v[2] = ga ? 1 : 0;
  }
  std::memcpy(out, v, sizeof(v));
  return MAPDN_OK;
} MAPDN_CATCH(h)

int mapdn_get_dc_angles(const mapdn_handle* h, const double* p_bus_demand_mw, double* va_rad) try {
  if (!h || !p_bus_demand_mw || !va_rad) return MAPDN_E_INVALID;
  const Plan& P = h->plan;
  if (!P.dc_ok) return api_fail(h, MAPDN_E_INVALID, P.fused_obus.empty() ? "the DC power flow matrix Bbus of this net is singular or not finite"
                                                                          : "the DC-angle start is not defined on a net with fused buses (bus_alias)");
  const int n = P.n;
  std::vector<double> pbus(n);
  for (int k = 0; k < n; ++k) pbus[k] = -p_bus_demand_mw[P.bus_of_pos[k]] / P.sn_mva + P.dc_pc[k];
  std::vector<double> th(n + 1, 0.0);
  if (h->solver == 0) {
    Schedule S;
    build_schedule(P, 1, S);
    std::vector<double> c(n, 0.0), hh(n, 0.0);
    for (int k = 0; k < n; ++k) {
      double y = pbus[k];
      for (int j = S.mm_ptr[k]; j < S.mm_ptr[k + 1]; ++j) y -= c[S.mm_child[j]];
      hh[k] = y * P.dc_id[k];
      c[k] = P.dc_bpk[k] * hh[k];
    }
    for (int k = n - 1; k >= 0; --k) th[k] = std::fma(-P.dc_g[k], th[P.par[k]], hh[k]);
  } else {
    SparseProg G;
    const int S = h->sp_lanes ? 64 / h->sp_lanes : 4;
    sparse_program(P, S, G);
    std::vector<double> B((size_t)G.n_blocks * 4, 0.0);
    for (size_t r = 0; r < G.rows.size(); ++r) {
      const SpRow& R = G.rows[r];
      if (!R.live) continue;
      const int i = (int)R.node;
      for (int q = 0; q < G.max_nnz; ++q) {
        const SpNz& z = G.nz[r * G.max_nnz + q];
        if ((int)z.col == i) B[(size_t)i * 4] = z.bdc;
        else if (z.slot >= 0) { double* o = &B[(size_t)z.slot * 4]; o[0] = z.bdc; o[1] = o[2] = o[3] = 0.0; }
      }
      B[(size_t)i * 4 + 3] = 1.0;
      B[(size_t)(n + i) * 4] = pbus[i];
    }
    for (int p = 0; p < G.n_phases; ++p)
      for (int s = 0; s < S; ++s) {
        const SpOp& op = G.ops[(size_t)p * S + s];
        const unsigned type = op.type & 255u;
        if (type == 0u) continue;
        const double* a = &B[(size_t)op.a * 4]; const double* b = &B[(size_t)op.b * 4];
        double r[4];
        if (type == 1u) { const double id = 1.0 / (a[0] * a[3] - a[1] * a[2]); r[0] = a[3] * id; r[1] = -a[1] * id; r[2] = -a[2] * id; r[3] = a[0] * id; }
        else {
          const double m[4] = {a[0] * b[0] + a[1] * b[2], a[0] * b[1] + a[1] * b[3], a[2] * b[0] + a[3] * b[2], a[2] * b[1] + a[3] * b[3]};
          const double* c0 = &B[(size_t)op.c * 4];
          for (int j = 0; j < 4; ++j) r[j] = type == 2u ? m[j] : c0[j] - m[j];
        }
        std::memcpy(&B[(size_t)op.c * 4], r, sizeof(r));
      }
    for (int i = 0; i < n; ++i) th[i] = B[(size_t)(n + i) * 4];
  }
  for (int b = 0; b < P.nbo; ++b) va_rad[b] = th[P.pos_of_obus[b]];
  return MAPDN_OK;
} MAPDN_CATCH(h)

int mapdn_get_flat_factors(const mapdn_handle* h, double* factors, int32_t* bus_of_pos) try {
  if (!h || !factors) return MAPDN_E_INVALID;
  if (!h->plan.radial) return MAPDN_E_TOPOLOGY;
  Schedule S;
  build_schedule(h->plan, 1, S);
  const int n = h->plan.n;
  for (int r = 0; r < S.R; ++r) {
    const StepRec& T = S.steps[(size_t)r];
    if (T.flags & S_LIVE) std::memcpy(factors + (size_t)(T.kp & 0xffffu) * FLAT_N, &S.flat[(size_t)r * FLAT_N], FLAT_N * sizeof(double));
  }
  if (bus_of_pos) std::memcpy(bus_of_pos, h->plan.bus_of_pos.data(), (size_t)(n + 1) * sizeof(int32_t));
  return MAPDN_OK;
} MAPDN_CATCH(h)

int mapdn_get_schedule(const mapdn_handle* h, int32_t W, int32_t* n_rows, int32_t* rows, int32_t* parent) try {
  if (!h || !n_rows || W < 1 || W > 16) return MAPDN_E_INVALID;
  if (!h->plan.radial) return MAPDN_E_TOPOLOGY;
  Schedule S;
  build_schedule(h->plan, W, S);
  *n_rows = S.R;
  if (rows) for (size_t i = 0; i < S.steps.size(); ++i) rows[i] = (S.steps[i].flags & S_LIVE) ? (int32_t)(S.steps[i].kp & 0xffffu) : -1;
  if (parent) std::memcpy(parent, h->plan.par.data(), h->plan.par.size() * sizeof(int32_t));
  return MAPDN_OK;
} MAPDN_CATCH(h)

int mapdn_get_sparse_program(const mapdn_handle* h, int32_t S, int32_t* dims, int32_t* ops, int32_t* order, int32_t* slots_ij) try {
  if (!h || !dims || S < 1 || S > 64) return MAPDN_E_INVALID;
  SparseProg G;
  sparse_program(h->plan, S, G);
  dims[0] = G.n_blocks; dims[1] = G.n_fill; dims[2] = G.n_phases; dims[3] = G.rows_per_sub; dims[4] = G.max_nnz;
  dims[5] = (int32_t)(G.slots_ij.size() / 3);
  if (ops) std::memcpy(ops, G.ops.data(), G.ops.size() * sizeof(SpOp));
  if (order) std::memcpy(order, G.order.data(), G.order.size() * sizeof(int32_t));
  if (slots_ij) std::memcpy(slots_ij, G.slots_ij.data(), G.slots_ij.size() * sizeof(int32_t));
  return MAPDN_OK;
} MAPDN_CATCH(h)

int mapdn_dense_solve(const double* a, const double* b, double* x, int32_t n, int32_t batch, void* stream) try {
  if (!a || !b || !x) return MAPDN_E_INVALID;
  const int rc = dense_solve_debug(a, b, x, n, batch, (hipStream_t)stream);
  return rc == 0 ? MAPDN_OK : (rc == -1 ? MAPDN_E_INVALID : MAPDN_E_HIP);
} MAPDN_CATCH(nullptr)

int mapdn_stats(mapdn_handle* h, int64_t* reset_failures, double* mean_iters, int32_t* max_iters, void* stream) try {
  if (!h) return MAPDN_E_INVALID;
  NEEDDEV(h);
  HIPCHK(h, hipSetDevice(h->device));
  hipStream_t st = (hipStream_t)stream;
  launch_stats(h->d, h->stats_dev, st);
  long long host[4];
  HIPCHK(h, hipMemcpyAsync(host, h->stats_dev, sizeof(host), hipMemcpyDeviceToHost, st));
  HIPCHK(h, hipStreamSynchronize(st));
  if (reset_failures) *reset_failures = host[0];
  if (mean_iters) *mean_iters = host[2] ? (double)host[1] / (double)host[2] : 0.0;
  if (max_iters) *max_iters = (int32_t)host[3];
  return MAPDN_OK;
} MAPDN_CATCH(h)

int mapdn_nr_timing(mapdn_handle* h, int32_t enable) try {
  if (!h) return MAPDN_E_INVALID;
  h->timing = enable != 0;
  return MAPDN_OK;
} MAPDN_CATCH(h)

int mapdn_nr_time_ms(mapdn_handle* h, double* total_ms, int64_t* launches) try {
  if (!h) return MAPDN_E_INVALID;
  NEEDDEV(h);
  HIPCHK(h, hipSetDevice(h->device));
  double ms = h->acc_ms; int64_t n = h->acc_launches;
  for (size_t i = 0; i + 1 < h->ev_used; i += 2) {
    HIPCHK(h, hipEventSynchronize(h->ev[i + 1]));
    float t = 0.f;
    HIPCHK(h, hipEventElapsedTime(&t, h->ev[i], h->ev[i + 1]));
    ms += t; n += 1;
  }
  h->ev_used = 0; h->acc_ms = 0.0; h->acc_launches = 0;
  if (total_ms) *total_ms = ms;
  if (launches) *launches = n;
  return MAPDN_OK;
} MAPDN_CATCH(h)

static const char* droop_resolve(const mapdn_droop_config* in, mapdn_droop_config& c) {
  if (in) c = *in; else std::memset(&c, 0, sizeof(c));
  if (c.va == 0.0) c.va = 0.95;
  if (c.vb == 0.0) c.vb = 1.0;
  if (c.vc == 0.0) c.vc = 1.0;
  if (c.vd == 0.0) c.vd = 1.05;
  if (c.damping == 0.0) c.damping = 0.1;
  if (c.max_iter == 0) c.max_iter = 100;
  if (c.v_tol == 0.0) c.v_tol = 1e-4;
  if (c.reactive_ratio == 0.0) c.reactive_ratio = 1.0;
  if (!(c.va < c.vb && c.vb <= c.vc && c.vc < c.vd)) return "droop: the breakpoints must satisfy va < vb <= vc < vd";
  if (!(c.damping > 0.0 && c.damping <= 1.0)) return "droop: damping must lie in (0, 1]";
  if (c.max_iter < 1 || c.max_iter > DROOP_MAX_ITER_CAP) return "droop: max_iter must lie in 1 ... 10000";
  if (!(c.v_tol > 0.0)) return "droop: v_tol must be > 0";
  if (!(c.reactive_ratio > 0.0)) return "droop: reactive_ratio must be > 0";
  return nullptr;
}

static int droop_prepare(mapdn_handle* h) {
  if (h->droop_ready) return MAPDN_OK;
  const Plan& P = h->plan;
  DroopState& s = h->droop;
  const size_t Bp = h->d.Bp, ns = (size_t)P.ns;
  int32_t *iters = nullptr, *nr_iters = nullptr, *n_active = nullptr; uint8_t *status = nullptr, *act = nullptr, *nr_conv = nullptr;
  int rc;
  if ((rc = dalloc(h, &s.a, ns * Bp)) || (rc = dalloc(h, &s.a_sol, ns * Bp)) || (rc = dalloc(h, &s.v_last, ns * Bp)) ||
      (rc = dalloc(h, &s.dv2, ns * Bp)) ||
      (rc = dalloc(h, &iters, Bp)) || (rc = dalloc(h, &nr_iters, Bp)) || (rc = dalloc(h, &status, Bp)) || (rc = dalloc(h, &act, Bp)) ||
      (rc = dalloc(h, &nr_conv, Bp)) || (rc = dalloc(h, &n_active, (size_t)DROOP_MAX_ITER_CAP + 1)))
    return rc;
  s.iters = iters; s.nr_iters = nr_iters; s.status = status; s.act = act; s.nr_conv = nr_conv; s.n_active = n_active;
  std::vector<int32_t> vrow(std::max<size_t>(ns, 1), 0);
  for (size_t j = 0; j < ns; ++j) vrow[j] = (int32_t)h->d.r_vout + VOF * P.pos_of_obus[P.sgen_bus[j]] + VO_VM;
  const int32_t* vr = nullptr;
  if ((rc = dupload(h, &vr, vrow))) return rc;
  s.sg_vrow = vr; s.vm_row = h->vm_row;
  h->droop_ready = true;
  return MAPDN_OK;
}

static int droop_run(mapdn_handle* h, const mapdn_droop_config& c, double* actions, double* vm_pu, int32_t* iterations,
                     uint8_t* status, hipStream_t st) {
  constexpr int DROOP_POLL = 4;
  if (const int rc = droop_prepare(h)) return rc;
  const Dev& d = h->d;
  DroopState s = h->droop;
  s.va = c.va; s.vb = c.vb; s.vc = c.vc; s.vd = c.vd; s.damping = c.damping; s.v_tol = c.v_tol; s.ratio = c.reactive_ratio;
  s.max_iter = c.max_iter; s.vm_out = vm_pu;
  HIPCHK(h, hipMemsetAsync(s.n_active, 0, ((size_t)c.max_iter + 1) * sizeof(int32_t), st));
  if (h->sbus_stale) {
    HIPCHK(h, hipMemsetAsync(s.a, 0, (size_t)d.ns * d.Bp * sizeof(double), st));
    launch_inject(d, MODE_SOLVE, nullptr, MAPDN_F64, d.cur_pl, d.cur_ql, d.cur_pv, s.a, 0, st);
  }
  launch_droop_update(d, s, 0, st);
  Dev dd = d;
  dd.active = s.act; dd.iters = const_cast<int32_t*>(s.nr_iters); dd.conv = const_cast<uint8_t*>(s.nr_conv);
  for (int i = 0; i < c.max_iter; ++i) {
    if (i % DROOP_POLL == 0) {
      int32_t left = 0;
      HIPCHK(h, hipMemcpyAsync(&left, s.n_active + i, sizeof(left), hipMemcpyDeviceToHost, st));
      HIPCHK(h, hipStreamSynchronize(st));
      if (left == 0) break;
    }
    nr_launch(h, MODE_SOLVE, nullptr, nullptr, nullptr, st, nullptr, 0, &dd);
    launch_droop_update(d, s, i + 1, st);
  }
  transpose_out(h, s.a_sol, 1.0, h->iota_idx, actions, d.ns, st);
  launch_copy_i32(s.iters, iterations, d.B, st);
  launch_copy_u8(s.status, status, d.B, st);
  HIPCHK(h, hipGetLastError());
  return MAPDN_OK;
}

int mapdn_droop_actions(mapdn_handle* h, const mapdn_droop_config* cfg, double* actions, double* vm_pu, int32_t* iterations,
                        uint8_t* status, void* stream) try {
  if (!h) return MAPDN_E_INVALID;
  mapdn_droop_config c;
  if (const char* why = droop_resolve(cfg, c)) return api_fail(h, MAPDN_E_INVALID, why);
  if (!actions || !iterations || !status) { h->err = "droop_actions: null buffer"; return MAPDN_E_INVALID; }
  NEEDDEV(h);
  if (!h->was_reset) { h->err = "droop_actions before reset"; return MAPDN_E_STATE; }
  HIPCHK(h, hipSetDevice(h->device));
  return droop_run(h, c, actions, vm_pu, iterations, status, (hipStream_t)stream);
} MAPDN_CATCH(h)

}
```

### mapdn_amd/csrc/kernels.hip

```cpp
#include <hip/hip_runtime.h>
#include <stdint.h>

#include <type_traits>

#include "kernels.hpp"
#include "philox.hpp"
#include "nr_common.hpp"
#include "nr_inst_list.hpp"

namespace mapdn {

__device__ __forceinline__ int64_t sample_start_row(const Dev& d, int e, uint32_t draw) {
  uint32_t x[4];
  philox4x32_10((uint32_t)(d.env_id_offset + e), draw, STREAM_START, 0u, d.seed_lo, d.seed_hi, x);
  const int64_t hour = (int64_t)(((uint64_t)x[0] * 24u) >> 32);
  const int64_t day = (int64_t)(((uint64_t)x[1] * (uint64_t)d.n_start_days) >> 32);
  const int64_t interval = (int64_t)(((uint64_t)x[2] * (uint64_t)d.per_hour) >> 32);
  return interval + hour * d.per_hour + day * d.per_day;
}
__device__ __forceinline__ double profile_value(const Dev& d, int e, int64_t row, uint32_t draw, int stream, int j, int col0, int add_noise) {
  double v = d.table[(size_t)row * d.ncol + col0 + j];
  if (add_noise) {
    uint32_t x[4];
    philox4x32_10((uint32_t)(d.env_id_offset + e), draw, (uint32_t)stream, (uint32_t)(j >> 1), d.seed_lo, d.seed_hi, x);
// ... 58 lines not shown
    double p;
    if (ar) { p = profile_value(d, e, ar_row, draw, STREAM_PV, j, 0, add_noise); d.cur_pv[o] = p; d.cur_q[o] = 0.0; }
    else p = pv[o];
    double q;
    if (mode == MODE_SOLVE) q = qin[o];
    else if (!act) q = d.q_new[o];
    else {
      const double sm = d.smax[j];
      const double lim = sqrt(sm * sm - p * p);
      if (mode == MODE_STEP && !ar) q = lim * (double)actions[(size_t)e * d.ns + j];
      else if (d.reset_action) {
        uint32_t x[4];
        philox4x32_10((uint32_t)(d.env_id_offset + e), draw, STREAM_ACTION, (uint32_t)(j >> 1), d.seed_lo, d.seed_hi, x);
        const double u = ((j & 1) ? u53(x[2], x[3]) : u53(x[0], x[1])) * (1.0 / 9007199254740992.0);
        q = lim * (d.action_low + (d.action_high - d.action_low) * u);
      } else q = 0.0;
      d.q_new[o] = q;
    }
    P -= p * d.sgen_scale[j]; Q -= q * d.sgen_scale[j];
  }
  if (k < d.n) {
    const size_t o = (size_t)k * d.Bp + e;
    const double2 v = make_double2(-P / d.sn, -Q / d.sn);
    ((double2*)((char*)d.nrbuf + d.sb_off))[o] = v;
    if (mode != MODE_SOLVE) ((double2*)((char*)d.nrbuf + d.sb_off_alt))[o] = v;
  }
}

template <typename AT>
__global__ void __launch_bounds__(256)
k_inject_sgen(Dev d, int mode, const AT* __restrict__ actions, int add_noise) {
  const int e = blockIdx.x * blockDim.x + threadIdx.x;
  const int jb = blockIdx.y;
  if (e >= d.B) return;
  const bool mlo_row = jb >= d.n_sgb;
  const int k = mlo_row ? d.mlo_pos[jb - d.n_sgb] : d.sgb_pos[jb];
  bool act, ar = false;
  if (mode == MODE_STEP) {
    const bool dn = d.done[e] != 0;
    ar = dn && d.auto_reset;
    act = !dn || ar;
  } else act = d.pending[e] != 0;
  const uint32_t draw = mode == MODE_STEP ? d.draw[e] : d.adv_draw[e];
  int64_t ar_row = 0;
  if (ar) {
    const int64_t start = sample_start_row(d, e, draw);
    ar_row = start + 1;
    if (jb == 0) d.start_row[e] = start;
  }
  if (jb == 0) {
    d.active[e] = act ? 1 : 0;
    if (mode == MODE_STEP) {
      d.resetting[e] = ar ? 1 : 0;
      d.adv_row[e] = (act && !ar) ? d.start_row[e] + d.steps[e] : -1; d.adv_draw[e] = draw;
    }
  }
  if (!act) return;
  double2* const sbp = (double2*)((char*)d.nrbuf + d.sb_off) + e;
  auto stored_load_sum = [&](int kk, double& Ps, double& Qs) {
    Ps = 0.0; Qs = 0.0;
    for (int i = d.load_ptr[kk]; i < d.load_ptr[kk + 1]; ++i) {
      const int li = d.load_idx[i];
      Ps += d.cur_pl[(size_t)li * d.Bp + e] * d.load_scale[li]; Qs += d.cur_ql[(size_t)li * d.Bp + e] * d.load_scale[li];
    }
  };
  if (mlo_row) {
    if (ar || k >= d.n) return;
    double Ps, Qs;
    stored_load_sum(k, Ps, Qs);
    sbp[(size_t)k * d.Bp] = make_double2(-Ps / d.sn, -Qs / d.sn);
    return;
  }
  double2* const bl = (double2*)d.bus_ld + (size_t)jb * d.Bp + e;
  double P, Q;
  if (ar) {
    auto load_sum = [&](int kk, double& Ps, double& Qs) {
      Ps = 0.0; Qs = 0.0;
      for (int i = d.load_ptr[kk]; i < d.load_ptr[kk + 1]; ++i) {
        const int li = d.load_idx[i];
        const size_t o = (size_t)li * d.Bp + e;
        const double p = profile_value(d, e, ar_row, draw, STREAM_LOAD_P, li, d.ns, add_noise);
        const double q = profile_value(d, e, ar_row, draw, STREAM_LOAD_Q, li, d.ns + d.nl, add_noise);
        d.cur_pl[o] = p; d.cur_ql[o] = q;
        Ps += p * d.load_scale[li]; Qs += q * d.load_scale[li];
      }
    };
    load_sum(k, P, Q);
    *bl = make_double2(P, Q);
    for (int i = jb; i < d.n_lb; i += d.n_sgb) {
      const int kk = d.lb_pos[i];
      double Ps, Qs;
      load_sum(kk, Ps, Qs);
      if (kk < d.n) {
        const double2 v = make_double2(-Ps / d.sn, -Qs / d.sn);
        sbp[(size_t)kk * d.Bp] = v;
        ((double2*)((char*)d.nrbuf + d.sb_off_alt))[(size_t)kk * d.Bp + e] = v;
      }
    }
  } else if (d.load_ptr[k + 1] - d.load_ptr[k] > 1) stored_load_sum(k, P, Q);
  else { const double2 v = *bl; P = v.x; Q = v.y; }
  for (int i = d.sgen_ptr[k]; i < d.sgen_ptr[k + 1]; ++i) {
    const int j = d.sgen_idx[i];
    const size_t o = (size_t)j * d.Bp + e;
    double p;
    if (ar) { p = profile_value(d, e, ar_row, draw, STREAM_PV, j, 0, add_noise); d.cur_pv[o] = p; d.cur_q[o] = 0.0; }
    else p = d.cur_pv[o];
    const double sm = d.smax[j];
    const double lim = sqrt(sm * sm - p * p);
    double q;
    if (mode == MODE_STEP && !ar) q = lim * (double)actions[(size_t)e * d.ns + j];
    else if (d.reset_action) {
      uint32_t x[4];
      philox4x32_10((uint32_t)(d.env_id_offset + e), draw, STREAM_ACTION, (uint32_t)(j >> 1), d.seed_lo, d.seed_hi, x);
      const double u = ((j & 1) ? u53(x[2], x[3]) : u53(x[0], x[1])) * (1.0 / 9007199254740992.0);
      q = lim * (d.action_low + (d.action_high - d.action_low) * u);
    } else q = 0.0;
    d.q_new[o] = q;
    P -= p * d.sgen_scale[j]; Q -= q * d.sgen_scale[j];
  }
  if (k < d.n) sbp[(size_t)k * d.Bp] = make_double2(-P / d.sn, -Q / d.sn);
}

__global__ void __launch_bounds__(256) k_reset_begin(Dev d, const int64_t* __restrict__ start_rows, int first_try) {
  const int e = blockIdx.x * blockDim.x + threadIdx.x;
  if (e >= d.B) return;
  if (first_try) d.pending[e] = 1;
  d.adv_row[e] = -1;
  if (!d.pending[e]) return;
  d.steps[e] = 1; d.sum_rewards[e] = 0.0; d.done[e] = 1;
  const uint32_t dr = d.draw[e];
  d.draw[e] = dr + 1;
  int64_t start;
  if (start_rows) start = start_rows[e];
  else start = sample_start_row(d, e, dr);
  const bool bad = start < 0 || start + (int64_t)d.episode_limit + 1 >= d.T;
  d.bad_start[e] = bad ? 1 : 0;
  if (bad) { d.pending[e] = 0; d.start_row[e] = 0; return; }
  d.start_row[e] = start;
  d.adv_row[e] = start + 1;
  d.adv_draw[e] = dr;
  for (int j = 0; j < d.ns; ++j) d.cur_q[(size_t)j * d.Bp + e] = 0.0;
}

__device__ __forceinline__ void noise_pair(const Dev& d, int e, uint32_t draw, int stream, int b, double& n0, double& n1) {
  uint32_t x[4];
  philox4x32_10((uint32_t)(d.env_id_offset + e), draw, (uint32_t)stream, (uint32_t)b, d.seed_lo, d.seed_hi, x);
  const double u1 = (u53(x[0], x[1]) + 0.5) * (1.0 / 9007199254740992.0);
  const double u2 = u53(x[2], x[3]) * (1.0 / 9007199254740992.0);
  const double r = sqrt(-2.0 * log(u1));
  double sn_, cs_;
  sincos(2.0 * M_PI * u2, &sn_, &cs_);
  n0 = fabs(r * cs_); n1 = fabs(r * sn_);
}
template <bool WANT>
__device__ __forceinline__ void commit_bus(const Dev& d, int b_, int e, size_t S, double& v, double& va, double& P, double& Q) {
  const size_t o = (size_t)b_ * S + e;
  if (!d.commit[e]) {
    if (WANT) { v = d.vm[o]; va = d.va[o]; P = d.res_p[o]; Q = d.res_q[o]; }
    return;
  }
  const int k = d.pos_of_obus[b_];
  if (k < d.n) {
    const double* vo = d.nrbuf + ((size_t)d.r_vout + (size_t)VOF * k) * S + e;
    const double2 sb = ((const double2*)((const char*)d.nrbuf + d.sb_off))[(size_t)k * S + e];
    const double ek = vo[(size_t)VO_E * S], fk = vo[(size_t)VO_F * S];
    v = sqrt(ek * ek + fk * fk);
    va = atan2(fk, ek);
    P = -sb.x * d.sn; Q = -sb.y * d.sn;
    if (d.zip) {
      const double ci = d.zip_c[2 * k], cz = d.zip_c[2 * k + 1];
      if (ci != 0.0 || cz != 0.0) {
        double Pl = 0.0, Ql = 0.0;
        for (int i = d.load_ptr[k]; i < d.load_ptr[k + 1]; ++i) {
          const int li = d.load_idx[i];
          Pl += d.cur_pl[(size_t)li * S + e] * d.load_scale[li]; Ql += d.cur_ql[(size_t)li * S + e] * d.load_scale[li];
        }
        const double vd1 = fma(cz, v * v, fma(ci, v, 1.0 - (ci + cz))) - 1.0;
        P = fma(Pl, vd1, P); Q = fma(Ql, vd1, Q);
      }
    }
  } else {
    v = d.vroot; va = 0.0;
    double ir = d.yrr0 * d.vroot, ii = d.yrr1 * d.vroot;
    for (int j = 0; j < d.n_root_children; ++j) {
      const double* cb = d.nrbuf + ((size_t)d.r_vout + (size_t)VOF * d.root_children[j]) * S + e;
      const double g = d.root_y[2 * j], b = d.root_y[2 * j + 1], ec = cb[(size_t)VO_E * S], fc = cb[(size_t)VO_F * S];
      ir += g * ec - b * fc; ii += g * fc + b * ec;
    }
    P = -(d.vroot * ir) * d.sn; Q = (d.vroot * ii) * d.sn;
  }
  d.va[o] = va;
  d.vm[o] = v;
  if (d.cm_kind[b_] == 0) { P = P + d.shunt_p[k] * v * v; Q = Q + d.shunt_q[k] * v * v; d.res_p[o] = P; d.res_q[o] = Q; }
  else if (WANT) { P = d.res_p[o]; Q = d.res_q[o]; }
}
template <bool WANT>
__device__ __forceinline__ void advance_pv_pair(const Dev& d, int e, int b, int add_noise, size_t S, double& v0, double& v1) {
  const int j0 = 2 * b, j1 = 2 * b + 1;
  const int64_t row = d.adv_row[e];
  if (row < 0 || row >= d.T) {
    if (WANT) { v0 = d.cur_pv[(size_t)j0 * S + e]; v1 = (j1 < d.ns) ? d.cur_pv[(size_t)j1 * S + e] : 0.0; }
    return;
  }
  const double* trow = d.table + (size_t)row * d.ncol;
  v0 = trow[j0]; v1 = (j1 < d.ns) ? trow[j1] : 0.0;
  if (add_noise) {
    double n0, n1;
    noise_pair(d, e, d.adv_draw[e], STREAM_PV, b, n0, n1);
    v0 += d.stdv[j0] * n0;
    if (j1 < d.ns) v1 += d.stdv[j1] * n1;
  }
  d.cur_pv[(size_t)j0 * S + e] = v0;
  if (j1 < d.ns) d.cur_pv[(size_t)j1 * S + e] = v1;
}
__device__ __forceinline__ void advance_load_pair(const Dev& d, int e, int b, int add_noise, size_t S, uint32_t sb_write_off) {
  const int64_t row = d.adv_row[e];
  if (row < 0 || row >= d.T) return;
  double2* const sbw = (double2*)((char*)d.nrbuf + sb_write_off) + e;
  const int j0 = 2 * b, j1 = 2 * b + 1;
  const bool has1 = j1 < d.nl;
  const double* trp = d.table + (size_t)row * d.ncol + d.ns;
  const double* trq = trp + d.nl;
  double p0 = trp[j0], q0 = trq[j0], p1 = has1 ? trp[j1] : 0.0, q1 = has1 ? trq[j1] : 0.0;
  if (add_noise) {
    const uint32_t draw = d.adv_draw[e];
    double n0, n1, m0, m1;
    noise_pair(d, e, draw, STREAM_LOAD_P, b, n0, n1);
    noise_pair(d, e, draw, STREAM_LOAD_Q, b, m0, m1);
    p0 += d.stdv[d.ns + j0] * n0; q0 += d.stdv[d.ns + d.nl + j0] * m0;
    if (has1) { p1 += d.stdv[d.ns + j1] * n1; q1 += d.stdv[d.ns + d.nl + j1] * m1; }
  }
  auto put = [&](int li, double p, double q) {
    d.cur_pl[(size_t)li * S + e] = p; d.cur_ql[(size_t)li * S + e] = q;
    const int dd = d.ld_dest[li];
    const double sc = d.load_scale[li];
    const double ps = p * sc, qs = q * sc;
    if ((dd & 3) == 0) sbw[(size_t)(dd >> 2) * S] = make_double2(-ps / d.sn, -qs / d.sn);
    else if ((dd & 3) == 1) ((double2*)d.bus_ld)[(size_t)(dd >> 2) * S + e] = make_double2(ps, qs);
  };
  put(j0, p0, q0);
  if (has1) put(j1, p1, q1);
}

__device__ __forceinline__ void advance_body(const Dev& d, int add_noise, int do_profiles, int do_commit, uint32_t sb_write_off,
                                             unsigned blk_x, unsigned blk_y) {
  const int e = (int)(blk_x * 256u + threadIdx.x);
  if (e >= d.B) return;
  const int npv = (d.ns + 1) >> 1, npl = (d.nl + 1) >> 1;
  const int npairs = do_profiles ? npv + npl : 0;
  const size_t S = (size_t)d.Bp;
  if ((int)blk_y >= npairs) {
    double v, va, P, Q;
    commit_bus<false>(d, (int)blk_y - npairs, e, S, v, va, P, Q);
    return;
  }
  if ((int)blk_y < npv) { double v0, v1; advance_pv_pair<false>(d, e, (int)blk_y, add_noise, S, v0, v1); }
  else advance_load_pair(d, e, (int)blk_y - npv, add_noise, S, sb_write_off);
}

__global__ void __launch_bounds__(256) k_advance(Dev d, int add_noise, int do_profiles, int do_commit, uint32_t sb_write_off) {
  advance_body(d, add_noise, do_profiles, do_commit, sb_write_off, blockIdx.x, blockIdx.y);
}

__global__ void __launch_bounds__(256) k_commit_fused(Dev d) {
  const int e = blockIdx.x * blockDim.x + threadIdx.x;
  if (e >= d.B || !d.commit[e]) return;
  const size_t S = (size_t)d.Bp;
  auto own = [&](int i, double& P, double& Q) {
    P = 0.0; Q = 0.0;
    for (int q = d.ob_load_ptr[i]; q < d.ob_load_ptr[i + 1]; ++q) {
      const int li = d.ob_load_idx[q];
      P += d.cur_pl[(size_t)li * S + e] * d.load_scale[li]; Q += d.cur_ql[(size_t)li * S + e] * d.load_scale[li];
    }
    for (int q = d.ob_sgen_ptr[i]; q < d.ob_sgen_ptr[i + 1]; ++q) {
      const int j = d.ob_sgen_idx[q];
      P -= d.cur_pv[(size_t)j * S + e] * d.sgen_scale[j]; Q -= d.cur_q[(size_t)j * S + e] * d.sgen_scale[j];
    }
  };
  const int i = blockIdx.y;
  const int b_ = d.fused_obus[i], k = d.pos_of_obus[b_];
  double v = d.vroot;
  if (k < d.n) {
    const double* vo = d.nrbuf + ((size_t)d.r_vout + (size_t)VOF * k) * S + e;
    const double ek = vo[(size_t)VO_E * S], fk = vo[(size_t)VO_F * S];
    v = sqrt(ek * ek + fk * fk);
  }
  double P, Q;
  own(i, P, Q);
  P += d.ob_shunt_p[i] * v * v; Q += d.ob_shunt_q[i] * v * v;
  if (d.cm_kind[b_] == 2) {
    double Dp = 0.0, Dq = 0.0;
    for (int m = 0; m < d.n_slack_group; ++m) { double p_, q_; own(d.slack_group[m], p_, q_); Dp += p_; Dq += q_; }
    double ir = d.yrr0 * d.vroot, ii = d.yrr1 * d.vroot;
    for (int j = 0; j < d.n_root_children; ++j) {
      const double* cb = d.nrbuf + ((size_t)d.r_vout + (size_t)VOF * d.root_children[j]) * S + e;
      const double g = d.root_y[2 * j], b = d.root_y[2 * j + 1], ec = cb[(size_t)VO_E * S], fc = cb[(size_t)VO_F * S];
      ir += g * ec - b * fc; ii += g * fc + b * ec;
    }
    P -= Dp + (d.vroot * ir) * d.sn; Q -= Dq - (d.vroot * ii) * d.sn;
  }
  d.res_p[(size_t)b_ * S + e] = P; d.res_q[(size_t)b_ * S + e] = Q;
}

#define GATHER_HAS_EXTRA 0x40000000
template <typename T>
__device__ __forceinline__ void gather_body(const double* __restrict__ base, const int32_t* rows_g, const double* scales_g,
                                            double scale_all, const int32_t* x_ptr_g, const int32_t* x_row_g,
                                            T* __restrict__ out, int C, int B, int Bp, unsigned blk_x, unsigned blk_y, unsigned grd_x, unsigned grd_y) {
  __shared__ T tile[64][65];
  typedef const __attribute__((address_space(4))) int32_t* c_i32;
  typedef const __attribute__((address_space(4))) double* c_f64;
  const c_i32 rows = (c_i32)(unsigned long long)rows_g, x_ptr = (c_i32)(unsigned long long)x_ptr_g, x_row = (c_i32)(unsigned long long)x_row_g;
  const c_f64 scales = (c_f64)(unsigned long long)scales_g;
  unsigned bx = blk_x, by = blk_y;
  if ((grd_y & 7u) == 0u) {
    const unsigned lin = blk_y * grd_x + blk_x, xcd = lin & 7u, slot = lin >> 3;
    by = (slot / grd_x) * 8u + xcd; bx = slot % grd_x;
  }
  const int c0 = (int)bx * 64, e0 = (int)by * 64;
  const int tx = threadIdx.x & 63, ty = __builtin_amdgcn_readfirstlane(threadIdx.x >> 6);
  const int etx = e0 + tx;
  int rw[16]; double sc[16];
#pragma unroll
  for (int i = 0; i < 16; ++i) {
    const int c = c0 + ty + 4 * i;
    rw[i] = (c < C) ? rows[c] : -1;
    sc[i] = (scales_g && c < C) ? scales[c] : scale_all;
  }
  double v[16];
#pragma unroll
  for (int i = 0; i < 16; ++i)
    v[i] = (rw[i] >= 0) ? base[(size_t)(rw[i] & ~GATHER_HAS_EXTRA) * Bp + etx] * sc[i] : 0.0;
#pragma unroll
  for (int i = 0; i < 16; ++i) {
    if (rw[i] >= 0 && (rw[i] & GATHER_HAS_EXTRA)) {
      const int c = c0 + ty + 4 * i;
      for (int q = x_ptr[c]; q < x_ptr[c + 1]; ++q) v[i] += base[(size_t)x_row[q] * Bp + etx];
    }
    tile[ty + 4 * i][tx] = (T)v[i];
  }
  __syncthreads();
  const int q4 = (threadIdx.x & 15) * 4, er = threadIdx.x >> 4;
  const bool vec = (C % 4) == 0 && ((unsigned long long)out % (sizeof(T) * 4)) == 0;
#pragma unroll
  for (int pass = 0; pass < 4; ++pass) {
    const int r = er + 16 * pass, e = e0 + r, c = c0 + q4;
    if (e >= B || c >= C) continue;
    T* o = out + (size_t)e * C + c;
    if (vec) {
      struct alignas(sizeof(T) * 4) V4 { T a, b, c, d; };
      *reinterpret_cast<V4*>(o) = V4{tile[q4][r], tile[q4 + 1][r], tile[q4 + 2][r], tile[q4 + 3][r]};
    } else {
#pragma unroll
      for (int u = 0; u < 4; ++u) if (c + u < C) o[u] = tile[q4 + u][r];
    }
  }
}

template <typename T>
__global__ void __launch_bounds__(256)
k_gather(const double* __restrict__ base, const int32_t* rows_g, const double* scales_g,
         double scale_all, const int32_t* x_ptr_g, const int32_t* x_row_g,
         T* __restrict__ out, int C, int B, int Bp) {
  gather_body<T>(base, rows_g, scales_g, scale_all, x_ptr_g, x_row_g, out, C, B, Bp, blockIdx.x, blockIdx.y, gridDim.x, gridDim.y);
}

__global__ void __launch_bounds__(256)
k_to_envminor(const double* __restrict__ src, double* __restrict__ dst, int n, int B, int Bp) {
  __shared__ double tile[64][65];
  const int c0 = blockIdx.x * 64, e0 = blockIdx.y * 64;
  const int tx = threadIdx.x & 63, ty = threadIdx.x >> 6;
  for (int r = ty; r < 64; r += 4) {
    const int e = e0 + r, c = c0 + tx;
    tile[r][tx] = (e < B && c < n) ? src[(size_t)e * n + c] : 0.0;
  }
  __syncthreads();
  for (int r = ty; r < 64; r += 4) {
    const int c = c0 + r;
    if (c < n) dst[(size_t)c * Bp + e0 + tx] = tile[tx][r];
  }
}

__global__ void k_copy_i32(const int32_t* s, int32_t* dd, int B) { int e = blockIdx.x * blockDim.x + threadIdx.x; if (e < B) dd[e] = s[e]; }
__global__ void k_copy_u8(const uint8_t* s, uint8_t* dd, int B) { int e = blockIdx.x * blockDim.x + threadIdx.x; if (e < B) dd[e] = s[e]; }

__global__ void __launch_bounds__(256) k_stats(Dev d, long long* out) {
  __shared__ long long s_pend[256], s_sum[256], s_cnt[256];
  __shared__ int s_max[256];
  long long pend = 0, sum = 0, cnt = 0; int mx = 0;
  for (int e = threadIdx.x; e < d.B; e += 256) {
    pend += (d.pending[e] || d.bad_start[e]) ? 1 : 0;
    if (d.active[e]) { sum += d.iters[e]; cnt += 1; mx = max(mx, d.iters[e]); }
  }
  s_pend[threadIdx.x] = pend; s_sum[threadIdx.x] = sum; s_cnt[threadIdx.x] = cnt; s_max[threadIdx.x] = mx;
  __syncthreads();
  for (int w = 128; w > 0; w >>= 1) {
    if (threadIdx.x < w) {
      s_pend[threadIdx.x] += s_pend[threadIdx.x + w]; s_sum[threadIdx.x] += s_sum[threadIdx.x + w];
      s_cnt[threadIdx.x] += s_cnt[threadIdx.x + w]; s_max[threadIdx.x] = max(s_max[threadIdx.x], s_max[threadIdx.x + w]);
    }
    __syncthreads();
  }
  if (threadIdx.x == 0) { out[0] = s_pend[0]; out[1] = s_sum[0]; out[2] = s_cnt[0]; out[3] = s_max[0]; }
}

__global__ void __launch_bounds__(256) k_calib_stream(const double* __restrict__ src, double* __restrict__ dst, int rows, int Bp, int pattern) {
  const unsigned pb = (unsigned)Bp * 16u;
  const __amdgpu_buffer_rsrc_t rs = __builtin_amdgcn_make_buffer_rsrc(const_cast<double*>(src), 0, (unsigned)rows * pb, 0x00020000);
  const __amdgpu_buffer_rsrc_t rd = __builtin_amdgcn_make_buffer_rsrc(dst, 0, (unsigned)rows * pb, 0x00020000);
  typedef unsigned int u4 __attribute__((ext_vector_type(4)));
  if (pattern == 0) {
    const unsigned el = threadIdx.x & 15u, w = threadIdx.x >> 4, e = blockIdx.x * 16u + el;
    for (unsigned r = w; r < (unsigned)rows; r += 16u) {
      const u4 v = __builtin_amdgcn_raw_buffer_load_b128(rs, e * 16u, r * pb, 0);
      __builtin_amdgcn_raw_buffer_store_b128(v, rd, e * 16u, r * pb, 0);
    }
  } else {
    const unsigned e = blockIdx.x * 256u + threadIdx.x;
    for (unsigned r = blockIdx.y; r < (unsigned)rows; r += gridDim.y) {
      const u4 v = __builtin_amdgcn_raw_buffer_load_b128(rs, e * 16u, r * pb, 0);
      __builtin_amdgcn_raw_buffer_store_b128(v, rd, e * 16u, r * pb, 0);
    }
  }
}
}
extern "C" int mapdn_debug_stream(const double* src, double* dst, int32_t rows, int32_t Bp, int32_t pattern, void* stream) {
  if (!src || !dst || rows < 1 || Bp < 256 || (Bp & 255) || (size_t)rows * Bp * 16 >= 0xffffffffull) return MAPDN_E_INVALID;
  if (pattern == 0) hipLaunchKernelGGL(mapdn::k_calib_stream, dim3(Bp / 16), dim3(256), 0, (hipStream_t)stream, src, dst, rows, Bp, 0);
  else hipLaunchKernelGGL(mapdn::k_calib_stream, dim3(Bp / 256, 64), dim3(256), 0, (hipStream_t)stream, src, dst, rows, Bp, 1);
  return hipGetLastError() == hipSuccess ? MAPDN_OK : MAPDN_E_HIP;
}
namespace mapdn {


void launch_inject(const Dev& d, int mode, const void* actions, int dtype, const double* pl, const double* ql,
                   const double* pv, const double* q, int add_noise, hipStream_t st) {
  const dim3 grid((d.Bp + 255) / 256, d.nb);
  if (dtype == MAPDN_F32) hipLaunchKernelGGL(k_inject<float>, grid, dim3(256), 0, st, d, mode, (const float*)actions, pl, ql, pv, q, add_noise);
  else hipLaunchKernelGGL(k_inject<double>, grid, dim3(256), 0, st, d, mode, (const double*)actions, pl, ql, pv, q, add_noise);
}
#define NR_TABLES \
  const NrInst* tabs[NR_INST_PARTS] = {nr_insts_0, nr_insts_1, nr_insts_2, nr_insts_3}; \
  const int cnt[NR_INST_PARTS] = {nr_n_insts_0, nr_n_insts_1, nr_n_insts_2, nr_n_insts_3};
static const NrInst* nr_find(int W, int L, bool hl, bool gl, int res, int var) {
  NR_TABLES
  for (int p = 0; p < NR_INST_PARTS; ++p)
    for (int i = 0; i < cnt[p]; ++i) {
      const NrInst& I = tabs[p][i];
      if (I.W == W && I.L == L && (I.HL != 0) == hl && (I.GL != 0) == gl && I.RES == res && I.VAR == var) return &I;
    }
  return nullptr;
}
static int nr_res_of(int rec_lds, int flat_lds) { return (rec_lds && flat_lds) ? 1 : (!rec_lds && !flat_lds) ? 2 : (rec_lds && !flat_lds) ? 3 : 0; }
static const NrInst* nr_pick(int W, int L, int h_lds, int g_lds, int rec_lds, int flat_lds, int var) {
  const bool hl = h_lds != 0, gl = hl && g_lds != 0;
  const int res = nr_res_of(rec_lds, flat_lds);
  const NrInst* I = res ? nr_find(W, L, hl, gl, res, var) : nullptr;
  return I ? I : nr_find(W, L, hl, gl, 0, var);
}
#ifdef MAPDN_NR_STAMPS
int nr_debug_stamps_0(unsigned long long*, int); int nr_debug_stamps_1(unsigned long long*, int);
int nr_debug_stamps_2(unsigned long long*, int); int nr_debug_stamps_3(unsigned long long*, int);
static int g_last_part = 0;
}
extern "C" int mapdn_debug_stamps(unsigned long long* out, int n) {
  using namespace mapdn;
  switch (g_last_part) { case 0: return nr_debug_stamps_0(out, n); case 1: return nr_debug_stamps_1(out, n);
                         case 2: return nr_debug_stamps_2(out, n); default: return nr_debug_stamps_3(out, n); }
}
namespace mapdn {
#endif
void launch_nr(const Dev& d, int mode, double* reward, uint8_t* term, double* info, hipStream_t st, const void* fused_actions, int fused_dtype) {
  if (d.dense) { launch_nr_dense(d, mode, reward, term, info, st); return; }
  if (d.sparse) { launch_nr_sparse(d, mode, reward, term, info, st); return; }
  const size_t lds = nr_lds_bytes(d.nr_waves, d.nr_lanes, d.n, d.nr_cslots, d.nr_xslots, d.nr_nclist, d.nr_h_lds, d.nr_g_lds,
                                  d.nr_line_lds ? d.n_line : 0, d.nr_rec_lds ? d.nr_rows : 0, d.nr_flat_lds ? d.nr_rows : 0);
  const NrInst* I = nr_pick(d.nr_waves, d.nr_lanes, d.nr_h_lds, d.nr_g_lds, d.nr_rec_lds, d.nr_flat_lds,
                            (d.nr_init == 2 ? NR_VAR_DC : 0) | (d.zip ? NR_VAR_ZIP : 0));
  if (!I) return;
#ifdef MAPDN_NR_STAMPS
  { NR_TABLES
    for (int p = 0; p < NR_INST_PARTS; ++p) if (I >= tabs[p] && I < tabs[p] + cnt[p]) g_last_part = p; }
#endif
  Dev dd = d;
  dd.fi_actions = (mode == MODE_STEP) ? fused_actions : nullptr; dd.fi_dtype = fused_dtype;
  void* args[] = {(void*)&dd, (void*)&mode, (void*)&reward, (void*)&term, (void*)&info};
  (void)hipLaunchKernel(I->fn, dim3(d.Bp / d.nr_lanes), dim3(64 * d.nr_waves), args, lds, st);
}
int nr_set_lds_limit(int waves, int lanes, int h_lds, int g_lds, int rec_lds, int flat_lds, size_t bytes, int var) {
  const NrInst* I = nr_pick(waves, lanes, h_lds, g_lds, rec_lds, flat_lds, var);
  if (!I) return -2;
  return hipFuncSetAttribute(I->fn, hipFuncAttributeMaxDynamicSharedMemorySize, (int)bytes) == hipSuccess ? 0 : -1;
}
int nr_geometry_compiled(int waves, int lanes, int h_lds, int g_lds, int rec_lds, int flat_lds, int var) {
  const NrInst* I = nr_pick(waves, lanes, h_lds, g_lds, rec_lds, flat_lds, var);
  return I ? (I->RES ? 2 : 1) : 0;
}
const NrInst* nr_inst_of(int waves, int lanes, int h_lds, int g_lds, int rec_lds, int flat_lds, int var) {
  return nr_pick(waves, lanes, h_lds, g_lds, rec_lds, flat_lds, var);
}
void launch_reset_begin(const Dev& d, const int64_t* start_rows, int first_try, hipStream_t st) {
  hipLaunchKernelGGL(k_reset_begin, dim3((d.B + 255) / 256), dim3(256), 0, st, d, start_rows, first_try);
}
void launch_advance(const Dev& d, int add_noise, int do_profiles, int do_commit, uint32_t sb_write_off, hipStream_t st) {
  const int rows = (do_profiles ? ((d.ns + 1) >> 1) + ((d.nl + 1) >> 1) : 0) + (do_commit ? d.nbo : 0);
  if (rows == 0) return;
  hipLaunchKernelGGL(k_advance, dim3((d.B + 255) / 256, rows), dim3(256), 0, st, d, add_noise, do_profiles, do_commit, sb_write_off);
}
void launch_commit_fused(const Dev& d, hipStream_t st) {
  if (d.n_fused > 0) hipLaunchKernelGGL(k_commit_fused, dim3((d.B + 255) / 256, d.n_fused), dim3(256), 0, st, d);
}
void launch_inject_sgen(const Dev& d, int mode, const void* actions, int dtype, int add_noise, hipStream_t st) {
  const dim3 grid((d.B + 255) / 256, d.n_sgb + d.n_mlo);
  if (dtype == MAPDN_F32) hipLaunchKernelGGL(k_inject_sgen<float>, grid, dim3(256), 0, st, d, mode, (const float*)actions, add_noise);
  else hipLaunchKernelGGL(k_inject_sgen<double>, grid, dim3(256), 0, st, d, mode, (const double*)actions, add_noise);
}
void launch_gather(const Dev& d, const double* base, const int32_t* rows, const double* scales, double scale_all,
                   const int32_t* x_ptr, const int32_t* x_row, void* out, int dtype, int C, hipStream_t st) {
  const dim3 grid((C + 63) / 64, d.Bp / 64);
  if (dtype == MAPDN_F32) hipLaunchKernelGGL(k_gather<float>, grid, dim3(256), 0, st, base, rows, scales, scale_all, x_ptr, x_row, (float*)out, C, d.B, d.Bp);
  else hipLaunchKernelGGL(k_gather<double>, grid, dim3(256), 0, st, base, rows, scales, scale_all, x_ptr, x_row, (double*)out, C, d.B, d.Bp);
}
void launch_to_envminor(const Dev& d, const double* src, double* dst, int n, hipStream_t st) {
  hipLaunchKernelGGL(k_to_envminor, dim3((n + 63) / 64, d.Bp / 64), dim3(256), 0, st, src, dst, n, d.B, d.Bp);
}
void launch_copy_i32(const int32_t* s, int32_t* dd, int B, hipStream_t st) { hipLaunchKernelGGL(k_copy_i32, dim3((B + 255) / 256), dim3(256), 0, st, s, dd, B); }
void launch_copy_u8(const uint8_t* s, uint8_t* dd, int B, hipStream_t st) { hipLaunchKernelGGL(k_copy_u8, dim3((B + 255) / 256), dim3(256), 0, st, s, dd, B); }
void launch_stats(const Dev& d, long long* out, hipStream_t st) { hipLaunchKernelGGL(k_stats, dim3(1), dim3(256), 0, st, d, out); }

}

#include "droop.hip"
```

### mapdn_amd/csrc/kernels.hpp

```cpp
#pragma once
#include <hip/hip_runtime.h>
#include <stdint.h>

#include "plan.hpp"

namespace mapdn {

enum { MODE_STEP = 0, MODE_RESET = 1, MODE_SOLVE = 2 };
enum { STREAM_PV = 0, STREAM_LOAD_P = 1, STREAM_LOAD_Q = 2, STREAM_ACTION = 3, STREAM_START = 4 };

enum { NB_G01 = 0, NB_G23, NB_H, NBP };
enum { VO_E = 0, VO_F, VO_VM, VO_VA, VOF };

struct Dev {
  int32_t B, Bp, nb, n, nl, ns, n_line, ncol;
  double vroot, sn, tol;
  int32_t max_it;
  const int32_t* bus_of_pos;
  const int32_t *load_ptr, *load_idx, *sgen_ptr, *sgen_idx;
  const double *shunt_p, *shunt_q;
  const double *load_scale, *sgen_scale;
  const int32_t *sgb_pos, *sgb_of_pos, *lb_pos, *mlo_pos, *ld_dest; int32_t n_sgb, n_lb, n_mlo;
  double* bus_ld;
  const LineFlow* lines;
  const int32_t* root_children; const double* root_y; int32_t n_root_children;
  double yrr0, yrr1;
  const double* table; const double* stdv; const double* smax;
  int64_t T; int32_t n_start_days, per_hour, per_day;
  int32_t barrier_type, use_line_weight, episode_limit, reset_action, auto_reset;
  double voltage_weight, q_weight, line_weight, v_lower, v_upper, action_low, action_high;
  uint32_t seed_lo, seed_hi; int64_t env_id_offset;
  double *cur_pv, *cur_q, *cur_pl, *cur_ql, *q_new;
  double* gbuf;
  double *vm, *va, *res_p, *res_q;
  double *pl;
  double *sum_rewards;
  int32_t* steps; int64_t* start_row; uint32_t* draw;
  uint8_t *done, *pending, *active, *commit, *bad_start, *resetting;
  int64_t* adv_row; uint32_t* adv_draw;
  double* nrbuf; uint32_t nrbuf_bytes; uint32_t sb_off, r_vout;
  uint32_t sb_off_alt;
  int32_t* iters; uint8_t* conv;
  int32_t nr_waves, nr_lanes, nr_rows, nr_cslots, nr_xslots, nr_nclist, nr_h_lds, nr_g_lds, nr_line_lds, nr_rec_lds, nr_flat_lds;
  const StepRec* sched; uint32_t sched_bytes; const int32_t* clist;
  const double* flat; uint32_t flat_bytes;
  const int32_t *mm_ptr, *mm_child; int32_t nr_mm_pass, mm_np;
  const StepRec* mm_recs; uint32_t mm_recs_bytes;
  double nr_check_dx;
  double nr_check_quad;
  int32_t sparse, sp_lanes, sp_blocks, sp_fill, sp_phases, sp_rows_per_sub, sp_max_nnz;
  const SpOp* sp_ops; uint32_t sp_ops_bytes; const SpNz* sp_nz; uint32_t sp_nz_bytes; const int32_t* sp_fill_slots;
  int32_t dense, dn_N, dn_lda;
  double* dn_A;
  const int32_t *gy_ptr, *gy_col; const double* gy_val;
  int32_t nbo, n_fused, n_alias, n_slack_group;
  const int32_t *pos_of_obus, *cm_kind, *fused_obus, *ob_load_ptr, *ob_load_idx, *ob_sgen_ptr, *ob_sgen_idx, *slack_group, *alias_pos;
  const double *ob_shunt_p, *ob_shunt_q;
  const int32_t* sgb_rec;
  const void* fi_actions; int32_t fi_dtype;
  int32_t nr_init;
  const DcRec* dc_recs; uint32_t dc_recs_bytes;
  const double* dc_pc;
  int32_t zip;
  const double* zip_c; uint32_t zip_c_bytes;
};

void launch_inject(const Dev& d, int mode, const void* actions, int dtype, const double* pl, const double* ql,
                   const double* pv, const double* q, int add_noise, hipStream_t st);
void launch_inject_sgen(const Dev& d, int mode, const void* actions, int dtype, int add_noise, hipStream_t st);
void launch_nr(const Dev& d, int mode, double* reward, uint8_t* term, double* info, hipStream_t st,
               const void* fused_actions = nullptr, int fused_dtype = 0);
enum { NR_VAR_DC = 1, NR_VAR_ZIP = 2 };
int nr_set_lds_limit(int waves, int lanes, int h_lds, int g_lds, int rec_lds, int flat_lds, size_t bytes, int var = 0);
int nr_geometry_compiled(int waves, int lanes, int h_lds, int g_lds, int rec_lds, int flat_lds, int var = 0);
struct NrInst;
const NrInst* nr_inst_of(int waves, int lanes, int h_lds, int g_lds, int rec_lds, int flat_lds, int var);
__host__ __device__ static inline size_t nr_line_bytes(int n_line) { return ((size_t)n_line * sizeof(LineFlow) + 15) & ~(size_t)15; }
static inline int nr_min_cslots(int W, int L) { return (10 * 64 * W + 8 * L - 1) / (8 * L); }
static inline size_t nr_lds_bytes(int W, int L, int n, int cslots, int xslots, int nclist, int h_lds, int g_lds, int n_line_lds,
                                  int rec_rows, int flat_rows) {
  const size_t rows = (size_t)(n + 2) * (1 + (h_lds ? 1 : 0) + (g_lds ? 2 : 0)) + (size_t)cslots * 4 + (size_t)xslots;
  const size_t Wt = (size_t)W * (64 / L);
  return rows * (size_t)L * 16 + (size_t)W * 64 + (size_t)64 * W * sizeof(double) + (size_t)((nclist + 3) & ~3) * sizeof(int32_t) +
         nr_line_bytes(n_line_lds) + Wt * rec_rows * sizeof(StepRec) + Wt * flat_rows * FLAT_N * sizeof(double);
}
size_t nr_sparse_lds_bytes(int n, int n_blocks, int L);
int nr_sparse_prepare(int L);
void launch_nr_sparse(const Dev& d, int mode, double* reward, uint8_t* term, double* info, hipStream_t st);
static inline bool nr_dense_ga(int N) { return N > 128; }
int nr_dense_waves(int N, bool ga);
size_t nr_dense_lds_bytes(const Dev& d);
int nr_dense_prepare(const Dev& d);
void launch_nr_dense(const Dev& d, int mode, double* reward, uint8_t* term, double* info, hipStream_t st);
int dense_solve_debug(const double* A, const double* b, double* x, int n, int batch, hipStream_t st);
void launch_reset_begin(const Dev& d, const int64_t* start_rows, int first_try, hipStream_t st);
void launch_advance(const Dev& d, int add_noise, int do_profiles, int do_commit, uint32_t sb_write_off, hipStream_t st);
void launch_commit_fused(const Dev& d, hipStream_t st);
void launch_gather(const Dev& d, const double* base, const int32_t* rows, const double* scales, double scale_all,
                   const int32_t* x_ptr, const int32_t* x_row, void* out, int dtype, int C, hipStream_t st);
void launch_to_envminor(const Dev& d, const double* src, double* dst, int n, hipStream_t st);
void launch_copy_i32(const int32_t* s, int32_t* dd, int B, hipStream_t st);
void launch_copy_u8(const uint8_t* s, uint8_t* dd, int B, hipStream_t st);
void launch_stats(const Dev& d, long long* out, hipStream_t st);

enum { DROOP_CONVERGED = 0, DROOP_MAX_ITER = 1, DROOP_PF_FAILED = 2, DROOP_STOPPED = 3, DROOP_RUNNING = 255 };
struct DroopState {
  double va, vb, vc, vd, damping, v_tol, ratio;
  int32_t max_iter;
  double *a, *a_sol, *v_last, *dv2;
  int32_t* iters;
  uint8_t* status;
  uint8_t* act;
  const int32_t* nr_iters; const uint8_t* nr_conv;
  const int32_t* sg_vrow;
  const int32_t* vm_row;
  int32_t* n_active;
  double* vm_out;
};
void launch_droop_update(const Dev& d, const DroopState& s, int iter, hipStream_t st);

}
```

### mapdn_amd/csrc/nr_common.hpp

```cpp
#pragma once
#include <hip/hip_runtime.h>
#include <stdint.h>

#include <type_traits>

#include "kernels.hpp"
#include "nrmath.hpp"

namespace mapdn {

typedef double d2 __attribute__((ext_vector_type(2)));
typedef unsigned int u32x2 __attribute__((ext_vector_type(2)));
typedef unsigned int u32x4 __attribute__((ext_vector_type(4)));

__device__ __forceinline__ double barrier(int type, double v) {
  switch (type) {
    case MAPDN_BARRIER_L1: return fabs(v - 1.0);
    case MAPDN_BARRIER_L2: return 2.0 * (v - 1.0) * (v - 1.0);
    case MAPDN_BARRIER_COURANT_BELTRAMI: {
      const double a = fmax(0.0, v - 1.05), b = fmax(0.0, 0.95 - v);
      return a * a + b * b;
    }
    case MAPDN_BARRIER_BOWL: {
      const double dv = fabs(v - 1.0);
      const double inside = bowl_inside(v);
      return (dv > 0.05) ? 2.0 * dv - 0.095 : inside;
    }
    default: {
      if (fabs(v) < 1.0) return exp(-1.0 / (1.0 - v * v * v * v));
      if (v > 1.0 && v < 3.0) { const double w = v - 2.0; return exp(-1.0 / (1.0 - w * w * w * w)); }
      return 0.0;
    }
  }
}

__device__ __forceinline__ double rcp_nr(double x) {
  double r = __builtin_amdgcn_rcp(x);
  double t = fma(-x, r, 1.0);
  r = fma(r, t, r);
  t = fma(-x, r, 1.0);
  return fma(r, t, r);
}

__device__ __forceinline__ d2 nr_rotate(d2 v, double s, double c, double y1) {
  const double sc = 1.0 - y1;
  return d2{sc * fma(v.x, c, -(v.y * s)), sc * fma(v.x, s, v.y * c)};
}

template <unsigned L, unsigned Wt, typename Stamp>
__device__ __forceinline__ void nr_epilogue(const Dev& d, int mode, double* __restrict__ reward, uint8_t* __restrict__ terminated,
                                            double* __restrict__ info, const d2* sV, unsigned t, unsigned e, bool act, bool conv,
                                            int bk_steps, uint32_t bk_draw, double bk_sum, double* s_epi, const double* s_lines,
                                            Stamp stamp) {
  const unsigned n = (unsigned)d.n;
  const double vroot = d.vroot;
  const size_t SB = (size_t)d.Bp;
  if (mode == MODE_SOLVE) {
    double* gV = d.nrbuf + (size_t)d.r_vout * SB + e;
    for (unsigned k = t; k < n; k += Wt) {
      const d2 vv = sV[(size_t)k * L];
      const double ek = vv.x, fk = vv.y;
      double* o = gV + (size_t)(VOF * k) * SB;
      o[(size_t)VO_E * SB] = ek; o[(size_t)VO_F * SB] = fk;
      o[(size_t)VO_VM * SB] = sqrt(ek * ek + fk * fk);
      o[(size_t)VO_VA * SB] = atan2(fk, ek);
    }
    return;
  }
  const bool commitf = act && conv;
  const bool valid = e < (unsigned)d.B;
  const double vlo = d.v_lower, vhi = d.v_upper, vref = 0.5 * (vlo + vhi);
  double n_lo = 0, n_hi = 0, dev = 0.0, vsum = 0.0, mdrop = 0.0, mrise = 0.0, bar = 0.0, line_loss = 0.0, q_loss = 0.0, q_fail = 0.0;
  typedef const __attribute__((address_space(4))) double* c_f64;
  const c_f64 linec = (c_f64)(unsigned long long)d.lines;
  double* gV = d.nrbuf + (size_t)d.r_vout * SB + e;
  constexpr int QPRE = 3;
  double q_pre[QPRE];
#pragma unroll
  for (int i = 0; i < QPRE; ++i) { const unsigned j = t + (unsigned)i * Wt; q_pre[i] = (j < (unsigned)d.ns) ? d.q_new[(size_t)j * SB + e] : 0.0; }
  auto bus_loop = [&](auto type_tag) {
    constexpr int BT = decltype(type_tag)::value;
#pragma unroll 4
    for (unsigned k = t; k < n; k += Wt) {
      const d2 vv = sV[(size_t)k * L];
      const double ek = vv.x, fk = vv.y;
      const double v = sqrt(ek * ek + fk * fk);
      if (commitf) { gV[((size_t)VOF * k + VO_E) * SB] = ek; gV[((size_t)VOF * k + VO_F) * SB] = fk; }
      n_lo += (v < vlo) ? 1.0 : 0.0; n_hi += (v > vhi) ? 1.0 : 0.0;
      dev += fabs(v - vref); vsum += v;
      mdrop = fmax(mdrop, (v < vlo) ? (vlo - v) : 0.0);
      mrise = fmax(mrise, (v > vhi) ? (v - vhi) : 0.0);
      bar += barrier(BT, v);
    }
  };
  switch (d.barrier_type) {
    case MAPDN_BARRIER_L1: bus_loop(std::integral_constant<int, MAPDN_BARRIER_L1>{}); break;
    case MAPDN_BARRIER_L2: bus_loop(std::integral_constant<int, MAPDN_BARRIER_L2>{}); break;
    case MAPDN_BARRIER_COURANT_BELTRAMI: bus_loop(std::integral_constant<int, MAPDN_BARRIER_COURANT_BELTRAMI>{}); break;
    case MAPDN_BARRIER_BOWL: bus_loop(std::integral_constant<int, MAPDN_BARRIER_BOWL>{}); break;
    default: bus_loop(std::integral_constant<int, MAPDN_BARRIER_BUMP>{}); break;
  }
  if (t == n % Wt) {
    const double v = vroot;
    n_lo += (v < vlo) ? 1.0 : 0.0; n_hi += (v > vhi) ? 1.0 : 0.0;
    dev += fabs(v - vref); vsum += v;
    mdrop = fmax(mdrop, (v < vlo) ? (vlo - v) : 0.0);
    mrise = fmax(mrise, (v > vhi) ? (v - vhi) : 0.0);
    bar += barrier(d.barrier_type, v);
  }
  if (d.n_alias) {
    for (unsigned a = t; a < (unsigned)d.n_alias; a += Wt) {
      const unsigned k = (unsigned)d.alias_pos[a];
      double v = vroot;
      if (k < n) { const d2 vv = sV[(size_t)k * L]; v = sqrt(vv.x * vv.x + vv.y * vv.y); }
      n_lo += (v < vlo) ? 1.0 : 0.0; n_hi += (v > vhi) ? 1.0 : 0.0;
      dev += fabs(v - vref); vsum += v;
      mdrop = fmax(mdrop, (v < vlo) ? (vlo - v) : 0.0);
      mrise = fmax(mrise, (v > vhi) ? (v - vhi) : 0.0);
      bar += barrier(d.barrier_type, v);
    }
  }
  stamp(22);
  if (t == 0 && valid) d.commit[e] = commitf ? 1 : 0;
  auto line_loop = [&](auto Lbase) {
#pragma unroll 4
    for (unsigned l = t; l < (unsigned)d.n_line; l += Wt) {
      const auto Lc = Lbase + (size_t)l * 5;
      const double ab = Lc[0];
      const unsigned a = (unsigned)__double2loint(ab), b = (unsigned)__double2hiint(ab);
      const double gff = Lc[1], gtt = Lc[2], gs = Lc[3], bd = Lc[4];
      const d2 vf = sV[(size_t)a * L], vt = sV[(size_t)b * L];
      const double ef = vf.x, ff = vf.y, et = vt.x, ft = vt.y;
      const double wr = ef * et + ff * ft, wi = ff * et - ef * ft;
      const double pl = ((gff * (ef * ef + ff * ff) + gtt * (et * et + ft * ft)) + (gs * wr + bd * wi)) * d.sn;
      if (commitf) d.pl[(size_t)l * SB + e] = pl;
      line_loss += pl;
    }
  };
  if (d.nr_line_lds) line_loop((const double*)s_lines); else line_loop(linec);
  stamp(23);
  {
    int i = 0;
    for (unsigned j = t; j < (unsigned)d.ns; j += Wt, ++i) {
      const size_t o = (size_t)j * SB + e;
      const double qn = i < QPRE ? (i == 0 ? q_pre[0] : i == 1 ? q_pre[1] : q_pre[2]) : d.q_new[o];
      if (commitf) d.cur_q[o] = qn;
      q_loss += fabs(qn * d.sgen_scale[j]); q_fail += fabs(qn);
    }
  }
  if (mode == MODE_STEP && __any(act && !conv)) {
    double a_lo = 0, a_hi = 0, a_dev = 0, a_sum = 0, a_drop = 0, a_rise = 0, a_bar = 0, a_ll = 0, a_ql = 0;
    for (unsigned k = t; k < (unsigned)d.nbo; k += Wt) {
      const double v = valid ? d.vm[(size_t)k * SB + e] : 1.0;
      a_lo += (v < vlo) ? 1.0 : 0.0; a_hi += (v > vhi) ? 1.0 : 0.0;
      a_dev += fabs(v - vref); a_sum += v;
      a_drop = fmax(a_drop, (v < vlo) ? (vlo - v) : 0.0);
      a_rise = fmax(a_rise, (v > vhi) ? (v - vhi) : 0.0);
      a_bar += barrier(d.barrier_type, v);
    }
    for (unsigned l = t; l < (unsigned)d.n_line; l += Wt) a_ll += valid ? d.pl[(size_t)l * SB + e] : 0.0;
    for (unsigned j = t; j < (unsigned)d.ns; j += Wt) a_ql += fabs(d.cur_q[(size_t)j * SB + e] * d.sgen_scale[j]);
    if (!commitf) { n_lo = a_lo; n_hi = a_hi; dev = a_dev; vsum = a_sum; mdrop = a_drop; mrise = a_rise; bar = a_bar; line_loss = a_ll; q_loss = a_ql; }
  }
  if (mode == MODE_RESET) {
    if (t == 0 && valid) {
      d.adv_row[e] = -1;
      if (act && conv) { d.pending[e] = 0; d.done[e] = 0; }
    }
    return;
  }
  stamp(21);
  double* sm = s_epi;
  const double part[10] = {n_lo, n_hi, dev, vsum, mdrop, mrise, bar, line_loss, q_loss, q_fail};
#pragma unroll
  for (int q = 0; q < 10; ++q) sm[(size_t)(q * Wt + t) * L] = part[q];
  __syncthreads();
  constexpr unsigned UNR = Wt <= 16 ? Wt : 8;
  for (unsigned q = t; q < 10u; q += Wt) {
    double a = sm[(size_t)(q * Wt) * L];
#pragma unroll UNR
    for (unsigned ww = 1; ww < Wt; ++ww) { const double b = sm[(size_t)(q * Wt + ww) * L]; a = (q == 4u || q == 5u) ? fmax(a, b) : a + b; }
    sm[(size_t)(q * Wt) * L] = a;
  }
  __syncthreads();
  if (t != 0 || !valid) return;
  if (!act) {
    reward[e] = 0.0; terminated[e] = 1;
    for (int c = 0; c < MAPDN_N_INFO; ++c) info[(size_t)e * MAPDN_N_INFO + c] = 0.0;
    return;
  }
  if (d.resetting[e]) {
    reward[e] = 0.0;
    for (int c = 0; c < MAPDN_N_INFO; ++c) info[(size_t)e * MAPDN_N_INFO + c] = 0.0;
    d.draw[e] = bk_draw + 1;
    if (conv) { terminated[e] = 0; d.steps[e] = 1; d.sum_rewards[e] = 0.0; d.done[e] = 0; }
    else { terminated[e] = 1; d.resetting[e] = 0; }
    return;
  }
  double tot[10];
#pragma unroll
  for (int q = 0; q < 10; ++q) tot[q] = sm[(size_t)(q * Wt) * L];
  {
    const bool ok = conv;
    const double inv_nb = 1.0 / (double)d.nbo;
    const double out = (tot[0] + tot[1]) * inv_nb;
    const double ql = tot[8] / (double)d.ns, qf = tot[9] / (double)d.ns;
    const double v_loss = tot[6] * inv_nb * d.voltage_weight;
    double loss;
    if (d.use_line_weight) loss = tot[7] / (double)d.n_line * d.line_weight + v_loss;
    else loss = ql * d.q_weight + v_loss;
    double rew = -loss;
    double* inf = info + (size_t)e * MAPDN_N_INFO;
    inf[0] = out; inf[1] = tot[0] * inv_nb; inf[2] = tot[1] * inv_nb;
    inf[3] = (out > 1e-3) ? 0.0 : 1.0;
    inf[4] = tot[2] * inv_nb; inf[5] = tot[3] * inv_nb; inf[6] = tot[4]; inf[7] = tot[5];
    inf[8] = tot[7]; inf[9] = ql; inf[10] = 0.0;
    if (!ok) { rew -= 200.0; inf[10] = 1.0; inf[3] = 0.0; inf[9] = qf; }
    const int st = bk_steps;
    d.draw[e] = bk_draw + 1;
    d.steps[e] = st + 1;
    d.sum_rewards[e] = bk_sum + rew;
    const bool term = (st + 1 >= d.episode_limit) || !ok;
    d.done[e] = term ? 1 : 0;
    reward[e] = rew; terminated[e] = term ? 1 : 0;
  }
  stamp(24);
}

}
```

### mapdn_amd/env.py

```python
from __future__ import annotations

import os
from collections import namedtuple

import numpy as np
import torch

from . import _lib
from ._lib import INFO_KEYS, N_INFO
from .marl_env_api import MultiAgentEnv
from .netspec import NetSpec, Profiles, make_case


def convert(dictionary):
    return namedtuple('GenericDict', dictionary.keys())(**dictionary)


class ActionSpace(object):

    def __init__(self, low, high):
        self.low = low
        self.high = high


# ... 151 lines not shown

    def step(self, actions, add_noise=True):
        a = actions
        if not torch.is_tensor(a):
            a = torch.as_tensor(np.asarray(a), device=self.device)
        if a.device != self.device:
            a = a.to(self.device)
        if a.dtype not in (torch.float32, torch.float64):
            a = a.to(torch.float64)
        a = a.reshape(self.n_envs, self.n_sgen).contiguous()
        if not self.fused_step:
            with torch.cuda.device(self.device):
                _lib.check(self._lib.mapdn_step(self._h, a.data_ptr(), self._code(a.dtype), int(add_noise),
                                                self._reward.data_ptr(), self._term.data_ptr(), self._info.data_ptr(),
                                                self._stream()), self._h)
            self._stepped = True
            self._obs_fresh = None
            return self._out(self._reward), self._out(self._term), self._out(self._info)
        buf = self._obs_buf(self.obs_dtype)
        with torch.cuda.device(self.device):
            _lib.check(self._lib.mapdn_step_obs(self._h, a.data_ptr(), self._code(a.dtype), int(add_noise),
                                                self._reward.data_ptr(), self._term.data_ptr(), self._info.data_ptr(),
                                                buf.data_ptr(), self._code(self.obs_dtype), self._stream()), self._h)
        self._stepped = True
        self._obs_fresh = self.obs_dtype
        return self._out(self._reward), self._out(self._term), self._out(self._info)

    def _obs_buf(self, dtype):
        buf = self._obs.get(dtype)
        if buf is None:
            buf = self._obs[dtype] = torch.empty(self.n_envs, self.n_agents, self._obs_size1, dtype=dtype, device=self.device)
        return buf

    def get_obs(self, dtype=None):
        dtype = dtype or self.obs_dtype
        buf = self._obs_buf(dtype)
        if self._obs_fresh != dtype:
            with torch.cuda.device(self.device):
                _lib.check(self._lib.mapdn_get_obs(self._h, buf.data_ptr(), self._code(dtype), self._stream()), self._h)
        if self.history > 1:
            o1, key = self._obs_size1, (dtype, "hist")
            pair = self._obs.get(key)
            if pair is None:
                pair = self._obs[key] = [torch.zeros(self.n_envs, self.n_agents, o1 * self.history, dtype=dtype, device=self.device)
                                         for _ in range(2)]
            if self._obs_hist is None:
                pair[0].zero_()
                self._obs_hist = 0
            cur, new = pair[self._obs_hist], pair[1 - self._obs_hist]
            new[..., :-o1].copy_(cur[..., o1:])
            new[..., -o1:].copy_(buf)
            if self.args.get("auto_reset") and self._stepped:
                new[..., :-o1].masked_fill_(self.auto_reset_mask().view(-1, 1, 1), 0)
            self._obs_hist = 1 - self._obs_hist
            return self._out(new)
        return self._out(buf)

    def get_state(self, dtype=None):
        dtype = dtype or self.obs_dtype
        buf = self._state.get(dtype)
        if buf is None:
            buf = self._state[dtype] = torch.empty(self.n_envs, self.state_size, dtype=dtype, device=self.device)
        with torch.cuda.device(self.device):
            _lib.check(self._lib.mapdn_get_state(self._h, buf.data_ptr(), self._code(dtype), self._stream()), self._h)
        return self._out(buf)

    def get_avail_actions(self):
        return torch.ones(self.n_envs, self.n_agents, self.n_actions, device=self.device)

    def get_obs_size(self):
        return self.obs_size

    def get_state_size(self):
        return self.state_size

    def get_total_actions(self):
        return self.n_actions

    def get_num_of_agents(self):
        return self.n_agents

    def get_env_info(self):
        return {"state_shape": self.get_state_size(), "obs_shape": self.get_obs_size(),
                "n_actions": self.get_total_actions(), "n_agents": self.n_agents,
                "episode_limit": self.episode_limit}

    _RESULT_KEYS = ("vm_pu", "va_degree", "p_mw", "q_mvar", "pl_mw", "sgen_p", "sgen_q")

    def results(self, keys=None):
        keys = self._RESULT_KEYS if keys is None else tuple(keys)
        B, dv, f64 = self.n_envs, self.device, torch.float64
        width = dict(vm_pu=self.n_bus, va_degree=self.n_bus, p_mw=self.n_bus, q_mvar=self.n_bus, pl_mw=self.n_line,
                     sgen_p=self.n_sgen, sgen_q=self.n_sgen)
        out = {k: (torch.empty(B, width[k], dtype=f64, device=dv) if self.copy or B > 1 else self._res_buf(k, width[k])) for k in keys}
        with torch.cuda.device(self.device):
            _lib.check(self._lib.mapdn_get_results(self._h, *[(out[k].data_ptr() if k in out else None) for k in self._RESULT_KEYS],
                                                   self._stream()), self._h)
        return out

    def _res_buf(self, k, w):
        b = self._obs.get(("res", k))
        if b is None:
            b = self._obs[("res", k)] = torch.empty(self.n_envs, w, dtype=torch.float64, device=self.device)
        return b

    def loads(self):
        lp = torch.empty(self.n_envs, self.n_load, dtype=torch.float64, device=self.device)
        lq = torch.empty_like(lp)
        with torch.cuda.device(self.device):
            _lib.check(self._lib.mapdn_get_loads(self._h, lp.data_ptr(), lq.data_ptr(), self._stream()), self._h)
        return lp, lq

    def solve(self, p_load, q_load, p_sgen, q_sgen):
        f64, dv, B = torch.float64, self.device, self.n_envs
        ins = [torch.as_tensor(x, dtype=f64, device=dv).contiguous() for x in (p_load, q_load, p_sgen, q_sgen)]
        assert ins[0].shape == (B, self.n_load) and ins[2].shape == (B, self.n_sgen)
        vm = torch.empty(B, self.n_bus, dtype=f64, device=dv)
        va = torch.empty_like(vm)
        it = torch.empty(B, dtype=torch.int32, device=dv)
        cv = torch.empty(B, dtype=torch.uint8, device=dv)
        with torch.cuda.device(self.device):
            _lib.check(self._lib.mapdn_solve_only(self._h, *[t.data_ptr() for t in ins], vm.data_ptr(), va.data_ptr(),
                                                  it.data_ptr(), cv.data_ptr(), self._stream()), self._h)
        return vm, va, it, cv.bool()

    def droop_actions(self, config=None, vm_pu=False):
        cc = _lib.make_droop_config(config)
        B, dv = self.n_envs, self.device
        act = torch.empty(B, self.n_sgen, dtype=torch.float64, device=dv)
        it = torch.empty(B, dtype=torch.int32, device=dv)
        st = torch.empty(B, dtype=torch.uint8, device=dv)
        vm = torch.empty(B, self.n_bus, dtype=torch.float64, device=dv) if vm_pu else None
        with torch.cuda.device(self.device):
            _lib.check(self._lib.mapdn_droop_actions(self._h, _lib.C.byref(cc), act.data_ptr(), vm.data_ptr() if vm_pu else None,
                                                     it.data_ptr(), st.data_ptr(), self._stream()), self._h)
        return (act, it, st, vm) if vm_pu else (act, it, st)

    def ybus_dense(self):
        nn = self.geometry()["n_nodes"]
        out = np.zeros((nn, nn, 2))
        _lib.check(self._lib.mapdn_get_ybus_dense(self._h, _lib._p(out, _lib._pd)), self._h)
        return out[..., 0] + 1j * out[..., 1]

    def obs_index(self):
        n = self.n_agents * self._obs_size1
        kind = np.zeros(n, np.int32)
        idx = np.zeros(n, np.int32)
        _lib.check(self._lib.mapdn_get_obs_index(self._h, _lib._p(kind, _lib._pi), _lib._p(idx, _lib._pi)), self._h)
        return kind.reshape(self.n_agents, -1), idx.reshape(self.n_agents, -1)

    def geometry(self):
        return _lib.nr_geometry(self._h)

    def nr_kernel(self):
        return _lib.nr_kernel(self._h)

    def stats(self):
        rf, mi, mx = _lib.C.c_int64(), _lib.C.c_double(), _lib.C.c_int32()
        with torch.cuda.device(self.device):
            _lib.check(self._lib.mapdn_stats(self._h, _lib.C.byref(rf), _lib.C.byref(mi), _lib.C.byref(mx), self._stream()), self._h)
        return dict(reset_failures=rf.value, mean_nr_iters=mi.value, max_nr_iters=mx.value)

    def profile_stats(self):
        sd, sm = np.empty(self.n_sgen + 2 * self.n_load), np.empty(self.n_sgen)
        _lib.check(self._lib.mapdn_get_profile_stats(self._h, _lib._p(sd, _lib._pd), _lib._p(sm, _lib._pd)), self._h)
        return sd, sm

    def nr_timing(self, enable=True):
        _lib.check(self._lib.mapdn_nr_timing(self._h, int(enable)), self._h)

    def nr_time_ms(self):
        ms, n = _lib.C.c_double(), _lib.C.c_int64()
        _lib.check(self._lib.mapdn_nr_time_ms(self._h, _lib.C.byref(ms), _lib.C.byref(n)), self._h)
        return ms.value, n.value


def _resolve_data(args):
    if args.get("net") is not None and args.get("profiles") is not None:
        return args["net"], args["profiles"]
    dp = str(args.get("data_path", ""))
    ps, ds = float(args.get("pv_scale", 1.0)), float(args.get("demand_scale", 1.0))
    if os.path.isdir(dp) and (os.path.exists(os.path.join(dp, "netspec.npz")) or os.path.exists(os.path.join(dp, "model.p"))):
        from .data import load_scenario
        return load_scenario(dp, ps, ds, hv_init=args.get("hv_init"),
                             zip_loads=args.get("zip_loads"))
    name = os.path.basename(os.path.normpath(dp))
    if name not in _SCENARIOS:
        raise FileNotFoundError(f"unknown scenario {name!r}: pass net=/profiles=, a directory with netspec.npz + the three "
                                f"CSV tables, or a data_path ending in one of {sorted(_SCENARIOS)}")
    import warnings
    warnings.warn(f"data_path {dp!r} holds no netspec.npz / model.p: using the SYNTHETIC {_SCENARIOS[name]} feeder of the same shape "
                  f"(mapdn_amd.netspec.make_case) — results are NOT comparable with runs on the real MAPDN data; pass "
                  f"net=/profiles= or a scenario directory to silence this", RuntimeWarning, stacklevel=3)
    net, prof = make_case(_SCENARIOS[name], seed=0)
    if ps != 1.0 or ds != 1.0:
        prof = Profiles(pv=prof.pv * ps, load_p=prof.load_p * ds, load_q=prof.load_q * ds,
                        time_delta_min=prof.time_delta_min, days=prof.days)
    return net, prof


class VoltageControl(MultiAgentEnv):

    def __init__(self, kwargs, device=None):
        args = _as_dict(kwargs)
        self.args = convert({k: v for k, v in args.items() if k not in ("net", "profiles")})
        net, prof = _resolve_data(args)
        self.data_path = args.get("data_path")
        self._b = VoltageControlBatch(net, prof, {k: v for k, v in args.items() if k in DEFAULT_ARGS}, n_envs=1,
                                      device=device, copy=False, obs_dtype=torch.float64)
        b = self._b
        self.episode_limit = b.episode_limit
        self.voltage_barrier_type = b.args["voltage_barrier_type"]
        self.voltage_weight, self.q_weight, self.line_weight = b.args["voltage_weight"], b.args["q_weight"], b.args["line_weight"]
        self.v_upper, self.v_lower = b.args["v_upper"], b.args["v_lower"]
        self.action_space = b.action_space
        self.history = b.history
        self.state_space = b.args["state_space"]
        self.n_actions = 1
        self.n_agents = b.n_agents
        self.s_max = prof.s_max(1.2)
        print(f"This is the s_max: \n{self.s_max}")
        n, o1 = b.n_agents, b._obs_size1
        off_info = 32
        off_term = off_info + 8 * N_INFO
        off_obs = (off_term + 8 + 63) // 64 * 64
        self._pk_off = dict(reward=0, info=off_info, term=off_term, obs=off_obs)
        nbytes = self._pk_off["obs"] + 8 * n * o1
        self._pk_dev = torch.zeros(nbytes, dtype=torch.uint8, device=b.device)
        self._pk_host = torch.zeros(nbytes, dtype=torch.uint8).pin_memory()
        self._pk_np = self._pk_host.numpy()
        assert self._pk_dev.data_ptr() % 64 == 0 and self._pk_host.data_ptr() % 64 == 0, "packed step buffers must be 64-byte aligned"
        po = self._pk_off
        b._reward = self._pk_dev[po["reward"]:po["reward"] + 8].view(torch.float64)
        b._info = self._pk_dev[po["info"]:po["info"] + 8 * N_INFO].view(torch.float64).view(1, N_INFO)
        b._term = self._pk_dev[po["term"]:po["term"] + 1].view(torch.bool)
        b._obs[torch.float64] = self._pk_dev[po["obs"]:].view(torch.float64).view(1, n, o1)
        self._act_host = torch.zeros(1, b.n_sgen, dtype=torch.float64).pin_memory()
        self._act_dev = torch.zeros(1, b.n_sgen, dtype=torch.float64, device=b.device)
        self._packed = b.fused_step and os.environ.get("MAPDN_DROPIN_PACKED", "1") != "0"
        self._zero_copy = self._packed and self.history == 1 and os.environ.get("MAPDN_DROPIN_ZEROCOPY", "1") != "0"
        if self._zero_copy:
            po, hp = self._pk_off, self._pk_host.data_ptr()
            self._zc = dict(reward=hp + po["reward"], info=hp + po["info"], term=hp + po["term"], obs=hp + po["obs"],
                            act=self._act_host.data_ptr())
        self._host_obs_valid = False
        agents_obs, state = self.reset()
        self.obs_size = agents_obs[0].shape[0]
        self.state_size = state.shape[0]
        self.steps = 1
        self.sum_rewards = 0

    def reset(self, reset_time=True):
        self._host_obs_valid = False
        self.steps = 1
        self.sum_rewards = 0
        for _ in range(100):
            obs, state = self._b.reset(reset_time=reset_time)
            if self._b.stats()["reset_failures"] == 0:
                return self._obs_list(obs), state[0].cpu().numpy()
        raise RuntimeError("reset(): no solvable start found (the reference would keep looping at voltage_control_env.py:108)")

    def manual_reset(self, day, hour, interval):
        self._host_obs_valid = False
        self.steps = 1
        self.sum_rewards = 0
        obs, state = self._b.manual_reset(day, hour, interval)
        if self._b.stats()["reset_failures"]:
            raise RuntimeError("manual_reset(): the power flow of this start is not solvable")
        return self._obs_list(obs), state[0].cpu().numpy()

    def step(self, actions, add_noise=True):
        if self._packed:
            self._act_host.numpy()[0, :] = np.asarray(actions, dtype=np.float64).reshape(-1)
            if self._zero_copy:
                b, z = self._b, self._zc
                with torch.cuda.device(b.device):
                    _lib.check(b._lib.mapdn_step_obs(b._h, z["act"], _lib.F64, int(add_noise), z["reward"], z["term"], z["info"],
                                                     z["obs"], _lib.F64, b._stream()), b._h)
                b._stepped = True
                b._obs_fresh = None
            else:
                self._act_dev.copy_(self._act_host, non_blocking=True)
                self._b.step(self._act_dev, add_noise=add_noise)
                self._pk_host.copy_(self._pk_dev, non_blocking=True)
            torch.cuda.current_stream(self._b.device).synchronize()
            po, h = self._pk_off, self._pk_np
            reward = float(h[po["reward"]:po["reward"] + 8].view(np.float64)[0])
            terminated = bool(h[po["term"]])
            vals = h[po["info"]:po["info"] + 8 * N_INFO].view(np.float64).copy()
            self._host_obs_valid = self.history == 1
        else:
            a = torch.as_tensor(np.asarray(actions, dtype=np.float64).reshape(1, -1))
            r, t, info = self._b.step(a, add_noise=add_noise)
            reward = float(r[0].item())
            terminated = bool(t[0].item())
            vals = info[0].cpu().numpy()
        self.steps += 1
        self.sum_rewards += reward
        if terminated:
            print(f"Episode terminated at time: {self.steps} with return: {self.sum_rewards:2.4f}.")
        return reward, terminated, {k: float(v) for k, v in zip(INFO_KEYS, vals)}

    def droop_action(self, config=None, vm_pu=False):
        out = self._b.droop_actions(config, vm_pu=vm_pu)
        a, it, st = out[0][0].cpu().numpy(), int(out[1][0].item()), int(out[2][0].item())
        return (a, it, st, out[3][0].cpu().numpy()) if vm_pu else (a, it, st)
# ... 69 lines not shown
```

Before: 39.99 million.

## Defer per-bus result commit and gather observations directly from NR voltages

Adds a lazy-commit mode, on by default for the tree solver without ZIP loads or fused buses. The step no longer writes per-bus vm/va/P/Q for envs that accepted the new solution. Instead it records a lazy flag and rotates among three Sbus buffers, and the observation/state gather computes vm, va, P and Q on the fly from the NR voltage output and the previous Sbus. A catch-up commit runs before any API that reads the committed arrays (reset, get_results, solve_only, droop). The aim is to remove the full-bus commit pass and its global memory traffic from the step path, at the cost of a third Sbus buffer, a heavier gather kernel, and more complex state handling.

```diff
diff --git a/include/mapdn.h b/include/mapdn.h
--- a/include/mapdn.h
+++ b/include/mapdn.h
@@ -100,6 +100,7 @@
   int32_t fuse_inject;
   int32_t overlap_advance;
   int32_t xcd_map;
+  int32_t lazy_commit;
 } mapdn_env_config;
 
 typedef struct mapdn_dims_t {
@@ -154,6 +155,8 @@
 int mapdn_get_schedule(const mapdn_handle* h, int32_t n_waves, int32_t* n_rows, int32_t* rows, int32_t* parent);
 
 int mapdn_get_nr_geometry(const mapdn_handle* h, int32_t* out20);
+
+int mapdn_get_lazy_commit(const mapdn_handle* h, int32_t* out);
 
 int mapdn_get_dc_angles(const mapdn_handle* h, const double* p_bus_demand_mw, double* va_rad);
 
diff --git a/mapdn_amd/_lib.py b/mapdn_amd/_lib.py
--- a/mapdn_amd/_lib.py
+++ b/mapdn_amd/_lib.py
@@ -33,6 +33,7 @@
     "mapdn_policy_forward_train", "mapdn_policy_backward", "mapdn_policy_backward_scratch_floats", "mapdn_get_dc_angles",
     "mapdn_get_nr_kernel", "mapdn_droop_actions", "mapdn_policy_forward_geometry", "mapdn_critic_head_backward_geometry",
     "mapdn_critic_twin_forward", "mapdn_critic_twin_scratch_floats", "mapdn_critic_twin_geometry", "mapdn_critic_twin_mse",
+    "mapdn_get_lazy_commit",
 )
 
 _pd = C.POINTER(C.c_double)
@@ -69,12 +70,13 @@
         ("nr_mm_pass", C.c_int32), ("sp_lanes", C.c_int32), ("inject_full", C.c_int32),
         ("nr_check_dx", C.c_double), ("nr_check_quad", C.c_double), ("debug_geometry", C.c_int32),
         ("tolerance_mva", C.c_double), ("tolerance_is_pu", C.c_int32), ("nr_init", C.c_int32),
-        ("fuse_inject", C.c_int32), ("overlap_advance", C.c_int32), ("xcd_map", C.c_int32),
+        ("fuse_inject", C.c_int32), ("overlap_advance", C.c_int32), ("xcd_map", C.c_int32), ("lazy_commit", C.c_int32),
     ]
 
 
 TUNING_INT = ("nr_solver", "nr_waves", "nr_lanes", "nr_lean", "nr_h_lds", "nr_g_lds", "nr_rec_lds", "nr_flat_lds", "nr_line_lds",
-              "nr_mm_pass", "sp_lanes", "inject_full", "debug_geometry", "tolerance_is_pu", "nr_init", "fuse_inject", "overlap_advance", "xcd_map")
+              "nr_mm_pass", "sp_lanes", "inject_full", "debug_geometry", "tolerance_is_pu", "nr_init", "fuse_inject", "overlap_advance", "xcd_map",
+              "lazy_commit")
 TUNING_F64 = ("nr_check_dx", "nr_check_quad", "tolerance_mva")
 NR_SOLVERS = dict(auto=0, tree=0, sparse=1, dense=2)
 NR_INITS = dict(flat=0, dc=2)
@@ -186,6 +188,7 @@
     lib.mapdn_get_dc_angles.argtypes = [vp, _pd, _pd]
     lib.mapdn_get_nr_geometry.argtypes = [vp, _pi]
     lib.mapdn_get_nr_kernel.argtypes = [vp, _pi]
+    lib.mapdn_get_lazy_commit.argtypes = [vp, _pi]
     lib.mapdn_debug_stream.argtypes = [vp, vp, C.c_int32, C.c_int32, C.c_int32, vp]
     lib.mapdn_get_sparse_program.argtypes = [vp, C.c_int32, _pi, _pi, _pi, _pi]
     lib.mapdn_policy_forward.argtypes = [vp] * 14 + [C.c_int32] * 4 + [C.c_float, vp]
@@ -331,6 +334,12 @@
     return dict(zip(GEOMETRY_KEYS, [int(x) for x in out]))
 
 
+def lazy_commit(handle) -> bool:
+    out = C.c_int32()
+    check(load().mapdn_get_lazy_commit(handle, C.byref(out)), handle)
+    return bool(out.value)
+
+
 NR_KERNEL_KEYS = {0: ("W", "L", "HL", "GL", "RES", "DC", "ZIP"), 1: ("L", "DC", "ZIP"), 2: ("W", "GA")}
 
 
diff --git a/mapdn_amd/csrc/capi.hip b/mapdn_amd/csrc/capi.hip
--- a/mapdn_amd/csrc/capi.hip
+++ b/mapdn_amd/csrc/capi.hip
@@ -22,7 +22,7 @@
 struct Knobs {
   int solver;
   int waves, lanes;
-  int lean, h_lds, g_lds, rec_lds, flat_lds, line_lds, mm_pass, fuse_inject;
+  int lean, h_lds, g_lds, rec_lds, flat_lds, line_lds, mm_pass, fuse_inject, lazy_commit;
   int sp_lanes;
   bool inject_full, debug_geometry;
   double check_dx, check_quad;
@@ -39,6 +39,7 @@
   k.flat_lds = tri(c.nr_flat_lds, "MAPDN_NR_FLAT_LDS"); k.line_lds = tri(c.nr_line_lds, "MAPDN_NR_LINE_LDS");
   k.mm_pass = tri(c.nr_mm_pass, "MAPDN_NR_MM_PASS");
   k.fuse_inject = tri(c.fuse_inject, "MAPDN_FUSE_INJECT");
+  k.lazy_commit = tri(c.lazy_commit, "MAPDN_LAZY_COMMIT");
   k.sp_lanes = num(c.sp_lanes, "MAPDN_SP_LANES");
   k.inject_full = num(c.inject_full, "MAPDN_INJECT_FULL") != 0;
   k.debug_geometry = num(c.debug_geometry, "MAPDN_DEBUG_GEOMETRY") != 0;
@@ -63,6 +64,8 @@
   bool have_profiles = false, was_reset = false, host_only = false;
   bool sbus_stale = true;
   bool fuse_inject = false;
+  bool lazy_commit = false, res_behind = false;
+  int32_t *obs_kpos = nullptr, *state_kpos = nullptr;
   size_t lds_bytes = 0;
   struct Geo { int W = 0, L = 0, lean = 0, rows = 0, h_lds = 0, g_lds = 0, rec_lds = 0, flat_lds = 0, line_lds = 0, mm_pass = 0, ncl = 0;
                size_t lds = 0; long wgs = 0; int resident = 0, rounds = 0; double model_ns = 0.0; } geo;
@@ -261,6 +264,12 @@
     return api_fail(h, MAPDN_E_INVALID, "fuse_inject = 1 exists on the tree solver only (this handle runs the general sparse / dense solver)");
   if (k.fuse_inject == 1 && (c.auto_reset || k.inject_full))
     return api_fail(h, MAPDN_E_INVALID, "fuse_inject = 1 needs a handle without auto_reset and without inject_full");
+  if (k.lazy_commit == 1 && h->solver != 0)
+    return api_fail(h, MAPDN_E_INVALID, "lazy_commit = 1 exists on the tree solver only (this handle runs the general sparse / dense solver)");
+  if (k.lazy_commit == 1 && P.zip)
+    return api_fail(h, MAPDN_E_INVALID, "lazy_commit = 1 is not built for voltage-dependent (ZIP) loads (the commit of a ZIP bus sums the bus's loads)");
+  if (k.lazy_commit == 1 && !P.fused_obus.empty())
+    return api_fail(h, MAPDN_E_INVALID, "lazy_commit = 1 is not built for nets with fused buses (bus_alias: k_commit_fused)");
   if (h->solver == 1 && k.sp_lanes != 0 && k.sp_lanes != 16 && k.sp_lanes != 8 && k.sp_lanes != 4 && k.sp_lanes != 2)
     return api_fail(h, MAPDN_E_INVALID, "sp_lanes (MAPDN_SP_LANES) must be 16, 8, 4 or 2 (0 = automatic)");
   return MAPDN_OK;
@@ -389,6 +398,7 @@
   d.res_p = d.gbuf + (size_t)r.rp * Bp; d.res_q = d.gbuf + (size_t)r.rq * Bp;
   AL(sum_rewards, 1); AL(steps, 1); AL(start_row, 1); AL(draw, 1); AL(done, 1); AL(pending, 1);
   AL(active, 1); AL(commit, 1); AL(bad_start, 1); AL(resetting, 1); AL(adv_row, 1); AL(adv_draw, 1); AL(iters, 1); AL(conv, 1);
+  if (h->lazy_commit) { AL(lazy, 1); AL(lazy_next, 1); }
   std::vector<uint8_t> ones(Bp, 1);
   HIPCHK(h, hipMemcpy(d.done, ones.data(), Bp, hipMemcpyHostToDevice));
   int rc;
@@ -404,35 +414,44 @@
   const GbufRows g = gbuf_rows(d);
   std::vector<std::vector<int>> sgens_at(P.nbo);
   for (int j = 0; j < P.ns; ++j) sgens_at[P.sgen_bus[j]].push_back(j);
+  auto plus_zero = [](double x) { return x == 0.0 && !std::signbit(x); };
   auto tables = [&](const std::vector<int32_t>& kind, const std::vector<int32_t>& idx, std::vector<int32_t>& rows,
-                    std::vector<double>& scale, std::vector<int32_t>& xptr, std::vector<int32_t>& xrow) {
-    rows.resize(kind.size()); scale.assign(kind.size(), 1.0); xptr.assign(kind.size() + 1, 0); xrow.clear();
+                    std::vector<double>& scale, std::vector<int32_t>& xptr, std::vector<int32_t>& xrow, std::vector<int32_t>& kpos) {
+    rows.resize(kind.size()); scale.assign(kind.size(), 1.0); xptr.assign(kind.size() + 1, 0); xrow.clear(); kpos.assign(kind.size(), 0);
+    auto bus = [&](size_t c, int q) {
+      if (!h->lazy_commit) return;
+      const int k = P.pos_of_obus[idx[c]];
+      kpos[c] = k;
+      rows[c] |= GATHER_BUS | (q << GATHER_Q_SHIFT);
+      if (q >= 2 && (k >= P.n || !plus_zero(q == 2 ? P.shunt_p[k] : P.shunt_q[k]))) rows[c] |= GATHER_SLOW;
+    };
     for (size_t c = 0; c < kind.size(); ++c) {
       switch (kind[c]) {
-        case G_P_ADDBACK: rows[c] = g.rp + idx[c]; for (int j : sgens_at[idx[c]]) xrow.push_back(g.pv + j); break;
-        case G_Q_ADDBACK: rows[c] = g.rq + idx[c]; for (int j : sgens_at[idx[c]]) xrow.push_back(g.q + j); break;
+        case G_P_ADDBACK: rows[c] = g.rp + idx[c]; bus(c, 2); for (int j : sgens_at[idx[c]]) xrow.push_back(g.pv + j); break;
+        case G_Q_ADDBACK: rows[c] = g.rq + idx[c]; bus(c, 3); for (int j : sgens_at[idx[c]]) xrow.push_back(g.q + j); break;
         case G_SGEN_P: rows[c] = g.pv + idx[c]; break;
         case G_SGEN_Q: rows[c] = g.q + idx[c]; break;
-        case G_VM: rows[c] = g.vm + idx[c]; break;
-        case G_VA_RAD: rows[c] = g.va + idx[c]; break;
-        case G_P: rows[c] = g.rp + idx[c]; break;
-        case G_Q: rows[c] = g.rq + idx[c]; break;
-        case G_VA_DEG: rows[c] = g.va + idx[c]; scale[c] = 180.0 / M_PI; break;
+        case G_VM: rows[c] = g.vm + idx[c]; bus(c, 0); break;
+        case G_VA_RAD: rows[c] = g.va + idx[c]; bus(c, 1); break;
+        case G_P: rows[c] = g.rp + idx[c]; bus(c, 2); break;
+        case G_Q: rows[c] = g.rq + idx[c]; bus(c, 3); break;
+        case G_VA_DEG: rows[c] = g.va + idx[c]; bus(c, 1); scale[c] = 180.0 / M_PI; break;
         default: rows[c] = -1; break;
       }
       xptr[c + 1] = (int32_t)xrow.size();
-      if (xptr[c + 1] > xptr[c]) rows[c] |= 0x40000000;
+      if (xptr[c + 1] > xptr[c]) rows[c] |= GATHER_HAS_EXTRA;
     }
     if (xrow.empty()) xrow.push_back(0);
   };
-  std::vector<int32_t> rows, xptr, xrow; std::vector<double> scale;
+  if ((size_t)g.n > (size_t)GATHER_ROW_MASK) { h->err = "too many rows in the gatherable state block"; return MAPDN_E_INVALID; }
+  std::vector<int32_t> rows, xptr, xrow, kpos; std::vector<double> scale;
   int rc;
-  tables(P.obs_kind, P.obs_idx, rows, scale, xptr, xrow);
+  tables(P.obs_kind, P.obs_idx, rows, scale, xptr, xrow, kpos);
   if ((rc = dupload(h, &h->obs_rows, rows)) || (rc = dupload(h, &h->obs_scale, scale)) || (rc = dupload(h, &h->obs_xptr, xptr)) ||
-      (rc = dupload(h, &h->obs_xrow, xrow)))
+      (rc = dupload(h, &h->obs_xrow, xrow)) || (rc = dupload(h, &h->obs_kpos, kpos)))
     return rc;
-  tables(P.state_kind, P.state_idx, rows, scale, xptr, xrow);
-  if ((rc = dupload(h, &h->state_rows, rows)) || (rc = dupload(h, &h->state_scale, scale))) return rc;
+  tables(P.state_kind, P.state_idx, rows, scale, xptr, xrow, kpos);
+  if ((rc = dupload(h, &h->state_rows, rows)) || (rc = dupload(h, &h->state_scale, scale)) || (rc = dupload(h, &h->state_kpos, kpos))) return rc;
   std::vector<int32_t> io(std::max(std::max(d.nbo, d.n_line), std::max(d.nl, d.ns)));
   for (size_t i = 0; i < io.size(); ++i) io[i] = (int32_t)i;
   return dupload(h, &h->iota_idx, io);
@@ -443,12 +462,14 @@
   Dev& d = h->d;
   const size_t Bp = d.Bp;
   const size_t sb_off = fb_rows * Bp * 16;
-  const size_t vout_off = sb_off + 2 * nblk * Bp * 16;
+  const size_t n_sb = h->lazy_commit ? 3 : 2;
+  const size_t vout_off = sb_off + n_sb * nblk * Bp * 16;
   const size_t bytes = vout_off + (size_t)VOF * (P.n + 1) * Bp * sizeof(double);
   if (bytes >= (size_t)0xFFFFFFFFu) { h->err = "env batch too large: NR scratch exceeds the 4 GiB one buffer resource addresses; use fewer envs per handle"; return MAPDN_E_INVALID; }
   if (const int rc = dalloc(h, &d.nrbuf, bytes / sizeof(double))) return rc;
   d.nrbuf_bytes = (uint32_t)bytes;
   d.sb_off = (uint32_t)sb_off; d.sb_off_alt = (uint32_t)(sb_off + nblk * Bp * 16);
+  d.sb_off_prev = (uint32_t)(sb_off + (n_sb - 1) * nblk * Bp * 16);
   d.r_vout = (uint32_t)(vout_off / (Bp * sizeof(double)));
   std::vector<double> row(Bp, d.vroot);
   double* rootv = d.nrbuf + ((size_t)d.r_vout + (size_t)VOF * P.n) * Bp;
@@ -536,6 +557,7 @@
   if (rc) return rc;
   h->nr_var = (cfg->nr_init == 2 ? NR_VAR_DC : 0) | (h->plan.zip ? NR_VAR_ZIP : 0);
   h->fuse_inject = h->solver == 0 && !cfg->auto_reset && !h->knobs.inject_full && h->knobs.fuse_inject != 2;
+  h->lazy_commit = h->solver == 0 && !h->plan.zip && h->plan.fused_obus.empty() && h->knobs.lazy_commit != 2;
   h->device = device;
   std::memset(&h->d, 0, sizeof(h->d));
   h->d.B = B; h->d.Bp = (B + 63) / 64 * 64;
@@ -664,12 +686,37 @@
   } else launch_inject_sgen(d, mode, actions, dtype, add_noise, st);
 }
 
+static int commit_behind(mapdn_handle* h, hipStream_t st) {
+  if (!h->lazy_commit || !h->res_behind) return MAPDN_OK;
+  launch_advance(h->d, 0, 0, COMMIT_BEHIND, 0, st);
+  HIPCHK(h, hipMemsetAsync(h->d.lazy, 0, (size_t)h->d.Bp, st));
+  h->res_behind = false;
+  return MAPDN_OK;
+}
+
+static void gather_gbuf(mapdn_handle* h, bool obs, void* out, int dtype, hipStream_t st) {
+  const int C = obs ? h->plan.n_agents * h->plan.obs_size : h->plan.state_size;
+  const int32_t* rows = obs ? h->obs_rows : h->state_rows;
+  const double* scale = obs ? h->obs_scale : h->state_scale;
+  const int32_t *xp = obs ? h->obs_xptr : nullptr, *xr = obs ? h->obs_xrow : nullptr;
+  if (h->lazy_commit) launch_gather_bus(h->d, rows, obs ? h->obs_kpos : h->state_kpos, scale, xp, xr, out, dtype, C, st);
+  else launch_gather(h->d, h->d.gbuf, rows, scale, 1.0, xp, xr, out, dtype, C, st);
+}
+
 static void step_launches(mapdn_handle* h, const void* actions, int32_t actions_dtype, int32_t add_noise, double* reward,
                           uint8_t* terminated, double* info, hipStream_t st) {
   const Dev& d = h->d;
   const bool fused = h->fuse_inject && !h->sbus_stale;
   if (!fused) inject_launch(h, MODE_STEP, actions, actions_dtype, add_noise, st);
   nr_launch(h, MODE_STEP, reward, terminated, info, st, fused ? actions : nullptr, actions_dtype);
+  if (h->lazy_commit) {
+    launch_advance(d, add_noise, 1, COMMIT_LOSING, d.sb_off_alt, st);
+    const uint32_t read = h->d.sb_off;
+    h->d.sb_off = h->d.sb_off_alt; h->d.sb_off_alt = h->d.sb_off_prev; h->d.sb_off_prev = read;
+    std::swap(h->d.lazy, h->d.lazy_next);
+    h->res_behind = true;
+    return;
+  }
   if (d.zip) {
     launch_advance(d, 0, 0, 1, d.sb_off_alt, st);
     launch_advance(d, add_noise, 1, 0, d.sb_off_alt, st);
@@ -688,6 +735,7 @@
   HIPCHK(h, hipSetDevice(h->device));
   hipStream_t st = (hipStream_t)stream;
   const Dev& d = h->d;
+  if (const int rc = commit_behind(h, st)) return rc;
   for (int t = 0; t < max_tries; ++t) {
     launch_reset_begin(d, start_rows, t == 0, st);
     launch_advance(d, add_noise, 1, 0, d.sb_off, st);
@@ -725,10 +773,8 @@
   NEEDDEV(h);
   HIPCHK(h, hipSetDevice(h->device));
   hipStream_t st = (hipStream_t)stream;
-  const Dev& d = h->d;
-  const int C = h->plan.n_agents * h->plan.obs_size;
   step_launches(h, actions, actions_dtype, add_noise, reward, terminated, info, st);
-  launch_gather(d, d.gbuf, h->obs_rows, h->obs_scale, 1.0, h->obs_xptr, h->obs_xrow, obs, obs_dtype, C, st);
+  gather_gbuf(h, true, obs, obs_dtype, st);
   HIPCHK(h, hipGetLastError());
   return MAPDN_OK;
 } MAPDN_CATCH(h)
@@ -739,8 +785,7 @@
   NEEDDEV(h);
   HIPCHK(h, hipSetDevice(h->device));
   hipStream_t st = (hipStream_t)stream;
-  launch_gather(h->d, h->d.gbuf, h->obs_rows, h->obs_scale, 1.0, h->obs_xptr, h->obs_xrow, obs, dtype,
-                h->plan.n_agents * h->plan.obs_size, st);
+  gather_gbuf(h, true, obs, dtype, st);
   HIPCHK(h, hipGetLastError());
   return MAPDN_OK;
 } MAPDN_CATCH(h)
@@ -751,7 +796,7 @@
   NEEDDEV(h);
   HIPCHK(h, hipSetDevice(h->device));
   hipStream_t st = (hipStream_t)stream;
-  launch_gather(h->d, h->d.gbuf, h->state_rows, h->state_scale, 1.0, nullptr, nullptr, state, dtype, h->plan.state_size, st);
+  gather_gbuf(h, false, state, dtype, st);
   HIPCHK(h, hipGetLastError());
   return MAPDN_OK;
 } MAPDN_CATCH(h)
@@ -768,6 +813,7 @@
   HIPCHK(h, hipSetDevice(h->device));
   hipStream_t st = (hipStream_t)stream;
   const Dev& d = h->d;
+  if (vm_pu || va_degree || p_mw || q_mvar) { if (const int rc = commit_behind(h, st)) return rc; }
   if (vm_pu) transpose_out(h, d.vm, 1.0, h->iota_idx, vm_pu, d.nbo, st);
   if (va_degree) transpose_out(h, d.va, 180.0 / M_PI, h->iota_idx, va_degree, d.nbo, st);
   if (p_mw) transpose_out(h, d.res_p, 1.0, h->iota_idx, p_mw, d.nbo, st);
@@ -822,6 +868,7 @@
   HIPCHK(h, hipSetDevice(h->device));
   hipStream_t st = (hipStream_t)stream;
   const Dev& d = h->d;
+  if (const int rc = commit_behind(h, st)) return rc;
   launch_to_envminor(d, p_load, h->t_pl, d.nl, st);
   launch_to_envminor(d, q_load, h->t_ql, d.nl, st);
   launch_to_envminor(d, p_sgen, h->t_pv, d.ns, st);
@@ -869,6 +916,12 @@
                          h->fuse_inject ? 1 : 0, (int32_t)h->plan.fused_obus.size(), h->plan.nb, h->cfg.nr_init};
   std::memcpy(out, v, sizeof(v));
   if (h->solver == 1) out[2] = h->sp_lanes;
+  return MAPDN_OK;
+} MAPDN_CATCH(h)
+
+int mapdn_get_lazy_commit(const mapdn_handle* h, int32_t* out) try {
+  if (!h || !out) return MAPDN_E_INVALID;
+  *out = h->lazy_commit ? 1 : 0;
   return MAPDN_OK;
 } MAPDN_CATCH(h)
 
@@ -1075,6 +1128,7 @@
                      uint8_t* status, hipStream_t st) {
   constexpr int DROOP_POLL = 4;
   if (const int rc = droop_prepare(h)) return rc;
+  if (const int rc = commit_behind(h, st)) return rc;
   const Dev& d = h->d;
   DroopState s = h->droop;
   s.va = c.va; s.vb = c.vb; s.vc = c.vc; s.vd = c.vd; s.damping = c.damping; s.v_tol = c.v_tol; s.ratio = c.reactive_ratio;
diff --git a/mapdn_amd/csrc/kernels.hip b/mapdn_amd/csrc/kernels.hip
--- a/mapdn_amd/csrc/kernels.hip
+++ b/mapdn_amd/csrc/kernels.hip
@@ -234,17 +234,10 @@
   sincos(2.0 * M_PI * u2, &sn_, &cs_);
   n0 = fabs(r * cs_); n1 = fabs(r * sn_);
 }
-template <bool WANT>
-__device__ __forceinline__ void commit_bus(const Dev& d, int b_, int e, size_t S, double& v, double& va, double& P, double& Q) {
-  const size_t o = (size_t)b_ * S + e;
-  if (!d.commit[e]) {
-    if (WANT) { v = d.vm[o]; va = d.va[o]; P = d.res_p[o]; Q = d.res_q[o]; }
-    return;
-  }
-  const int k = d.pos_of_obus[b_];
+__device__ __forceinline__ void bus_results(const Dev& d, int k, int e, size_t S, uint32_t sb_read, double& v, double& va, double& P, double& Q) {
   if (k < d.n) {
     const double* vo = d.nrbuf + ((size_t)d.r_vout + (size_t)VOF * k) * S + e;
-    const double2 sb = ((const double2*)((const char*)d.nrbuf + d.sb_off))[(size_t)k * S + e];
+    const double2 sb = ((const double2*)((const char*)d.nrbuf + sb_read))[(size_t)k * S + e];
     const double ek = vo[(size_t)VO_E * S], fk = vo[(size_t)VO_F * S];
     v = sqrt(ek * ek + fk * fk);
     va = atan2(fk, ek);
@@ -271,6 +264,12 @@
     }
     P = -(d.vroot * ir) * d.sn; Q = (d.vroot * ii) * d.sn;
   }
+}
+template <bool WANT>
+__device__ __forceinline__ void commit_bus(const Dev& d, int b_, int e, size_t S, uint32_t sb_read, double& v, double& va, double& P, double& Q) {
+  const size_t o = (size_t)b_ * S + e;
+  const int k = d.pos_of_obus[b_];
+  bus_results(d, k, e, S, sb_read, v, va, P, Q);
   d.va[o] = va;
   d.vm[o] = v;
   if (d.cm_kind[b_] == 0) { P = P + d.shunt_p[k] * v * v; Q = Q + d.shunt_q[k] * v * v; d.res_p[o] = P; d.res_q[o] = Q; }
@@ -333,9 +332,17 @@
   const size_t S = (size_t)d.Bp;
   if ((int)blk_y >= npairs) {
     double v, va, P, Q;
-    commit_bus<false>(d, (int)blk_y - npairs, e, S, v, va, P, Q);
+    if (do_commit == COMMIT_ACCEPTED) {
+      if (d.commit[e]) commit_bus<false>(d, (int)blk_y - npairs, e, S, d.sb_off, v, va, P, Q);
+      return;
+    }
+    const bool need = d.lazy[e] != 0 && (do_commit == COMMIT_BEHIND || !d.commit[e]);
+    if (!need) return;
+    const int b0 = ((int)blk_y - npairs) * LAZY_BUSES, b1 = min(b0 + LAZY_BUSES, d.nbo);
+    for (int b_ = b0; b_ < b1; ++b_) commit_bus<false>(d, b_, e, S, d.sb_off_prev, v, va, P, Q);
     return;
   }
+  if (do_commit == COMMIT_LOSING && blk_y == 0) d.lazy_next[e] = d.commit[e];
   if ((int)blk_y < npv) { double v0, v1; advance_pv_pair<false>(d, e, (int)blk_y, add_noise, S, v0, v1); }
   else advance_load_pair(d, e, (int)blk_y - npv, add_noise, S, sb_write_off);
 }
@@ -384,7 +391,9 @@
   d.res_p[(size_t)b_ * S + e] = P; d.res_q[(size_t)b_ * S + e] = Q;
 }
 
-#define GATHER_HAS_EXTRA 0x40000000
+#ifndef GATHER_BUS_GROUP
+#define GATHER_BUS_GROUP 8
+#endif
 template <typename T>
 __device__ __forceinline__ void gather_body(const double* __restrict__ base, const int32_t* rows_g, const double* scales_g,
                                             double scale_all, const int32_t* x_ptr_g, const int32_t* x_row_g,
@@ -445,6 +454,92 @@
          double scale_all, const int32_t* x_ptr_g, const int32_t* x_row_g,
          T* __restrict__ out, int C, int B, int Bp) {
   gather_body<T>(base, rows_g, scales_g, scale_all, x_ptr_g, x_row_g, out, C, B, Bp, blockIdx.x, blockIdx.y, gridDim.x, gridDim.y);
+}
+
+template <typename T>
+__global__ void __launch_bounds__(256)
+k_gather_bus(Dev d, const int32_t* rows_g, const int32_t* kpos_g, const double* scales_g, const int32_t* x_ptr_g, const int32_t* x_row_g,
+             T* __restrict__ out, int C) {
+  __shared__ T tile[64][65];
+  typedef const __attribute__((address_space(4))) int32_t* c_i32;
+  typedef const __attribute__((address_space(4))) double* c_f64;
+  const c_i32 rows = (c_i32)(unsigned long long)rows_g, kpos = (c_i32)(unsigned long long)kpos_g;
+  const c_i32 x_ptr = (c_i32)(unsigned long long)x_ptr_g, x_row = (c_i32)(unsigned long long)x_row_g;
+  const c_f64 scales = (c_f64)(unsigned long long)scales_g;
+  const int B = d.B, Bp = d.Bp;
+  const double* __restrict__ base = d.gbuf;
+  unsigned bx = blockIdx.x, by = blockIdx.y;
+  if ((gridDim.y & 7u) == 0u) {
+    const unsigned lin = blockIdx.y * gridDim.x + blockIdx.x, xcd = lin & 7u, slot = lin >> 3;
+    by = (slot / gridDim.x) * 8u + xcd; bx = slot % gridDim.x;
+  }
+  const int c0 = (int)bx * 64, e0 = (int)by * 64;
+  const int tx = threadIdx.x & 63, ty = __builtin_amdgcn_readfirstlane(threadIdx.x >> 6);
+  const int etx = e0 + tx;
+  const bool lz = d.lazy[etx] != 0;
+  const size_t S = (size_t)Bp;
+  const double* const vout = d.nrbuf + (size_t)d.r_vout * S + etx;
+  const double* const sbp = (const double*)((const char*)d.nrbuf + d.sb_off_prev) + 2 * (size_t)etx;
+  constexpr int G = GATHER_BUS_GROUP;
+#pragma unroll 1
+  for (int g = 0; g < 16; g += G) {
+    int rw[G], kp[G]; double sc[G], a[G], b[G];
+#pragma unroll
+    for (int i = 0; i < G; ++i) {
+      const int c = c0 + ty + 4 * (g + i);
+      rw[i] = (c < C) ? rows[c] : -1;
+      kp[i] = (c < C) ? kpos[c] : 0;
+      sc[i] = (c < C) ? scales[c] : 1.0;
+    }
+#pragma unroll
+    for (int i = 0; i < G; ++i) {
+      a[i] = 0.0; b[i] = 0.0;
+      if (rw[i] < 0) continue;
+      if ((rw[i] & GATHER_BUS) && lz) {
+        const int q = (rw[i] >> GATHER_Q_SHIFT) & 3, k = kp[i];
+        if (q < 2) { if (k < d.n) { a[i] = vout[((size_t)VOF * k + VO_E) * S]; b[i] = vout[((size_t)VOF * k + VO_F) * S]; } }
+        else if (!(rw[i] & GATHER_SLOW)) a[i] = sbp[(size_t)k * 2 * S + (q - 2)];
+      } else a[i] = base[(size_t)(rw[i] & GATHER_ROW_MASK) * S + etx];
+    }
+#pragma unroll
+    for (int i = 0; i < G; ++i) {
+      double v = a[i];
+      if (rw[i] >= 0 && (rw[i] & GATHER_BUS) && lz) {
+        const int q = (rw[i] >> GATHER_Q_SHIFT) & 3, k = kp[i];
+        if (q == 0) v = (k < d.n) ? sqrt(a[i] * a[i] + b[i] * b[i]) : d.vroot;
+        else if (q == 1) v = (k < d.n) ? atan2(b[i], a[i]) : 0.0;
+        else if (!(rw[i] & GATHER_SLOW)) { v = -a[i] * d.sn; v = v + 0.0; }
+        else {
+          double vm_, va_, P, Q;
+          bus_results(d, k, etx, S, d.sb_off_prev, vm_, va_, P, Q);
+          P = P + d.shunt_p[k] * vm_ * vm_; Q = Q + d.shunt_q[k] * vm_ * vm_;
+          v = q == 2 ? P : Q;
+        }
+      }
+      v = (rw[i] >= 0) ? v * sc[i] : 0.0;
+      if (rw[i] >= 0 && (rw[i] & GATHER_HAS_EXTRA)) {
+        const int c = c0 + ty + 4 * (g + i);
+        for (int q = x_ptr[c]; q < x_ptr[c + 1]; ++q) v += base[(size_t)x_row[q] * S + etx];
+      }
+      tile[ty + 4 * (g + i)][tx] = (T)v;
+    }
+  }
+  __syncthreads();
+  const int q4 = (threadIdx.x & 15) * 4, er = threadIdx.x >> 4;
+  const bool vec = (C % 4) == 0 && ((unsigned long long)out % (sizeof(T) * 4)) == 0;
+#pragma unroll
+  for (int pass = 0; pass < 4; ++pass) {
+    const int r = er + 16 * pass, e = e0 + r, c = c0 + q4;
+    if (e >= B || c >= C) continue;
+    T* o = out + (size_t)e * C + c;
+    if (vec) {
+      struct alignas(sizeof(T) * 4) V4 { T a, b, c, d; };
+      *reinterpret_cast<V4*>(o) = V4{tile[q4][r], tile[q4 + 1][r], tile[q4 + 2][r], tile[q4 + 3][r]};
+    } else {
+#pragma unroll
+      for (int u = 0; u < 4; ++u) if (c + u < C) o[u] = tile[q4 + u][r];
+    }
+  }
 }
 
 __global__ void __launch_bounds__(256)
@@ -585,7 +680,8 @@
   hipLaunchKernelGGL(k_reset_begin, dim3((d.B + 255) / 256), dim3(256), 0, st, d, start_rows, first_try);
 }
 void launch_advance(const Dev& d, int add_noise, int do_profiles, int do_commit, uint32_t sb_write_off, hipStream_t st) {
-  const int rows = (do_profiles ? ((d.ns + 1) >> 1) + ((d.nl + 1) >> 1) : 0) + (do_commit ? d.nbo : 0);
+  const int rows = (do_profiles ? ((d.ns + 1) >> 1) + ((d.nl + 1) >> 1) : 0) +
+                   (do_commit == COMMIT_ACCEPTED ? d.nbo : do_commit ? (d.nbo + LAZY_BUSES - 1) / LAZY_BUSES : 0);
   if (rows == 0) return;
   hipLaunchKernelGGL(k_advance, dim3((d.B + 255) / 256, rows), dim3(256), 0, st, d, add_noise, do_profiles, do_commit, sb_write_off);
 }
@@ -603,6 +699,12 @@
   if (dtype == MAPDN_F32) hipLaunchKernelGGL(k_gather<float>, grid, dim3(256), 0, st, base, rows, scales, scale_all, x_ptr, x_row, (float*)out, C, d.B, d.Bp);
   else hipLaunchKernelGGL(k_gather<double>, grid, dim3(256), 0, st, base, rows, scales, scale_all, x_ptr, x_row, (double*)out, C, d.B, d.Bp);
 }
+void launch_gather_bus(const Dev& d, const int32_t* rows, const int32_t* kpos, const double* scales, const int32_t* x_ptr,
+                       const int32_t* x_row, void* out, int dtype, int C, hipStream_t st) {
+  const dim3 grid((C + 63) / 64, d.Bp / 64);
+  if (dtype == MAPDN_F32) hipLaunchKernelGGL(k_gather_bus<float>, grid, dim3(256), 0, st, d, rows, kpos, scales, x_ptr, x_row, (float*)out, C);
+  else hipLaunchKernelGGL(k_gather_bus<double>, grid, dim3(256), 0, st, d, rows, kpos, scales, x_ptr, x_row, (double*)out, C);
+}
 void launch_to_envminor(const Dev& d, const double* src, double* dst, int n, hipStream_t st) {
   hipLaunchKernelGGL(k_to_envminor, dim3((n + 63) / 64, d.Bp / 64), dim3(256), 0, st, src, dst, n, d.B, d.Bp);
 }
diff --git a/mapdn_amd/csrc/kernels.hpp b/mapdn_amd/csrc/kernels.hpp
--- a/mapdn_amd/csrc/kernels.hpp
+++ b/mapdn_amd/csrc/kernels.hpp
@@ -63,6 +63,17 @@
   const double* dc_pc;
   int32_t zip;
   const double* zip_c; uint32_t zip_c_bytes;
+  uint8_t *lazy, *lazy_next;
+  uint32_t sb_off_prev;
+};
+enum { COMMIT_NONE = 0, COMMIT_ACCEPTED = 1, COMMIT_LOSING = 2, COMMIT_BEHIND = 3 };
+constexpr int LAZY_BUSES = 8;
+enum : int32_t {
+  GATHER_HAS_EXTRA = 0x40000000,
+  GATHER_BUS = 0x20000000,
+  GATHER_Q_SHIFT = 26,
+  GATHER_SLOW = 0x02000000,
+  GATHER_ROW_MASK = 0x01ffffff,
 };
 
 void launch_inject(const Dev& d, int mode, const void* actions, int dtype, const double* pl, const double* ql,
@@ -98,6 +109,8 @@
 void launch_commit_fused(const Dev& d, hipStream_t st);
 void launch_gather(const Dev& d, const double* base, const int32_t* rows, const double* scales, double scale_all,
                    const int32_t* x_ptr, const int32_t* x_row, void* out, int dtype, int C, hipStream_t st);
+void launch_gather_bus(const Dev& d, const int32_t* rows, const int32_t* kpos, const double* scales, const int32_t* x_ptr,
+                       const int32_t* x_row, void* out, int dtype, int C, hipStream_t st);
 void launch_to_envminor(const Dev& d, const double* src, double* dst, int n, hipStream_t st);
 void launch_copy_i32(const int32_t* s, int32_t* dd, int B, hipStream_t st);
 void launch_copy_u8(const uint8_t* s, uint8_t* dd, int B, hipStream_t st);
diff --git a/mapdn_amd/csrc/nr_common.hpp b/mapdn_amd/csrc/nr_common.hpp
--- a/mapdn_amd/csrc/nr_common.hpp
+++ b/mapdn_amd/csrc/nr_common.hpp
@@ -150,8 +150,14 @@
   }
   if (mode == MODE_STEP && __any(act && !conv)) {
     double a_lo = 0, a_hi = 0, a_dev = 0, a_sum = 0, a_drop = 0, a_rise = 0, a_bar = 0, a_ll = 0, a_ql = 0;
+    const bool behind = valid && d.lazy && d.lazy[e];
     for (unsigned k = t; k < (unsigned)d.nbo; k += Wt) {
-      const double v = valid ? d.vm[(size_t)k * SB + e] : 1.0;
+      double v = 1.0;
+      if (behind) {
+        const unsigned p = (unsigned)d.pos_of_obus[k];
+        v = vroot;
+        if (p < n) { const double ek = gV[((size_t)VOF * p + VO_E) * SB], fk = gV[((size_t)VOF * p + VO_F) * SB]; v = sqrt(ek * ek + fk * fk); }
+      } else if (valid) v = d.vm[(size_t)k * SB + e];
       a_lo += (v < vlo) ? 1.0 : 0.0; a_hi += (v > vhi) ? 1.0 : 0.0;
       a_dev += fabs(v - vref); a_sum += v;
       a_drop = fmax(a_drop, (v < vlo) ? (vlo - v) : 0.0);
diff --git a/mapdn_amd/env.py b/mapdn_amd/env.py
--- a/mapdn_amd/env.py
+++ b/mapdn_amd/env.py
@@ -327,6 +327,9 @@
     def geometry(self):
         return _lib.nr_geometry(self._h)
 
+    def lazy_commit(self):
+        return _lib.lazy_commit(self._h)
+
     def nr_kernel(self):
         return _lib.nr_kernel(self._h)
 
```

New measurement: 36.24 million. 0.906x the previous value.
